# Zain-Jiang/Speech-Editing-Toolkit

Hardware: AMD Instinct MI355X
Metric: diffusion mel-frames/s (100-step p_sample, B=32/GPU, T=800) (higher is better)
Workload: dtype f32 (operands carried as 2 fp16 pieces, 3 MFMA products per term, fp32 accumulate: fp32-equivalent, see roofline.note)

## Files before the change

### include/set_amd.h

```cpp
#ifndef SET_AMD_H
#define SET_AMD_H

#include <stdint.h>

#ifdef __cplusplus
extern "C" {
#endif

#define SET_AMD_ABI_VERSION 2

#define SET_OK 0
#define SET_E_INVALID (-1)
#define SET_E_UNSUPPORTED (-2)
#define SET_E_LAUNCH (-3)

#define SET_ACT_NONE 0
#define SET_ACT_RELU 1
#define SET_ACT_GELU 2
#define SET_ACT_TANH 3
#define SET_ACT_SOFTPLUS 4
#define SET_ACT_MISH 5
#define SET_ACT_LRELU 6

#define SET_PRO_NONE 0
#define SET_PRO_LRELU 1
#define SET_PRO_DIV 2

#define SET_IMPL_NAIVE 1
#define SET_IMPL_MFMA 2
#define SET_IMPL_MFMA2 3

#define SET_IMPL_BF16 4
#define SET_IMPL_F16X2 5

#define SET_IMPL_FEWOUT 6

#define SET_DTYPE_F32 0
#define SET_DTYPE_BF16 1
#define SET_DTYPE_BF16_G16 2
#define SET_DTYPE_BF16_G16_X16 3

int set_abi_version(void);
const char *set_last_error(void);

typedef struct SetConv1dArgs {
    const float *in;
    const float *w;
    const float *bias;
    const float *res;
    const float *mask;
    const float *in_chan_add;
    float *out;
    int64_t in_bs, in_cs, out_bs, out_cs, res_bs, res_cs;
    int64_t w_base, w_sco, w_sci, w_stap;
    int32_t B, Cin, Cout, K, dil, pad;
    int32_t T_in, T_iter, T_out, out_stride, out_off;
    int32_t pro, act, accumulate, impl;
    float pro_param, act_param, alpha;
    float out_div;
} SetConv1dArgs;

int set_conv1d(const SetConv1dArgs *args, void *stream);

int64_t set_packed_conv_weight_size(int32_t Cout, int32_t Cin, int32_t K);
int set_pack_conv_weight(const float *w, float *wp, int32_t Cout, int32_t Cin, int32_t K,
                         int64_t w_base, int64_t w_sco, int64_t w_sci, int64_t w_stap, void *stream);

int64_t set_packed_conv_weight_x2_size(int32_t Cout, int32_t Cin, int32_t K);
int set_pack_conv_weight_x2(const float *w, void *wp, int32_t Cout, int32_t Cin, int32_t K, int64_t w_base, int64_t w_sco,
                            int64_t w_sci, int64_t w_stap, int32_t scale_exp, void *stream);
int64_t set_packed_conv_transpose_x2_size(int32_t Cout, int32_t Cin, int32_t k, int32_t u);
int set_pack_conv_transpose_x2(const float *w, void *wp, int32_t Cout, int32_t Cin, int32_t k, int32_t u, int32_t scale_exp,
                               void *stream);
int set_conv_transpose1d_x2(const float *in, const void *wp, const float *bias, float *out, int32_t B, int32_t Cin, int32_t Cout,
                            int32_t k, int32_t u, int32_t P, int32_t T_in, int32_t pro, float pro_param, void *stream);
int set_conv_x2_range_flag(int32_t *flag, int32_t reset);

typedef struct SetResblockPairArgs {
    const float *x;
    const void *w1;
    const float *b1;
    const void *w2;
    const float *b2;
    float *out;
    int64_t x_bs, x_cs, out_bs, out_cs;
    int32_t B, C, K, dil, T;
    int32_t accumulate;
    float slope, out_div;
} SetResblockPairArgs;
int64_t set_sizeof_resblock_pair_args(void);
int set_resblock_pair_x2_supported(int32_t C, int32_t K, int32_t dil, int32_t T);
int set_resblock_pair_x2(const SetResblockPairArgs *args, void *stream);

int64_t set_packed_conv_weight_v2_size(int32_t Cout, int32_t Cin, int32_t K);
int set_pack_conv_weight_v2(const float *w, float *wp, int32_t Cout, int32_t Cin, int32_t K, int32_t dil,
                            int64_t w_base, int64_t w_sco, int64_t w_sci, int64_t w_stap, void *stream);

int set_weight_norm_fold(const float *g, const float *v, float *w, int32_t n0, int64_t inner, void *stream);

int set_layernorm_ch(const float *x, const float *gamma, const float *beta, const float *mask, float *out,
                     int32_t B, int32_t C, int32_t T, float eps, void *stream);
int set_embedding_bct(const int64_t *idx, const float *table, float *out, int32_t B, int32_t T, int32_t C,
                      int32_t n_rows, float scale, int32_t accumulate, void *stream);
int set_embedding_bct_dev_scale(const int64_t *idx, const float *table, float *out, int32_t B, int32_t T, int32_t C,
                                int32_t n_rows, const float *scale_dev, int32_t accumulate, void *stream);
int set_abs_sum_mask(const float *x, float *mask, int32_t B, int32_t C, int32_t T, void *stream);
int set_index_mask(const int64_t *idx, float *mask, int64_t n, void *stream);
int set_expand_states(const float *enc, const int64_t *mel2ph, float *out, int32_t B, int32_t C,
                      int32_t T_txt, int32_t T, void *stream);
int set_add_chan_mask(const float *x, const float *add, const float *mask, float *out, int32_t B, int32_t C,
                      int32_t T, void *stream);
int set_masked_dur(const int64_t *mel2ph, const float *tmask, const int64_t *txt, int64_t *out, int32_t B,
                   int32_t T, int32_t T_txt, void *stream);
int set_pitch_coarse(const float *f0_in, const float *uv_in, const float *tmask, const int64_t *mel2ph_pad,
                     int32_t uv_from_logit, float *f0_denorm, int64_t *coarse, int64_t n, void *stream);
int set_transpose_btc_to_bct(const float *in, float *out, int32_t B, int32_t T, int32_t C, void *stream);
int set_transpose_bct_to_btc(const float *in, float *out, int32_t B, int32_t C, int32_t T, void *stream);
int set_sum_scale(const float *a, const float *b, const float *c, float *out, float div, int64_t n, void *stream);
int set_blend_mask(const float *a, const float *b, const float *m, float *out, int64_t n, int64_t inner, void *stream);
int set_mul_one_minus_mask(const float *x, const float *m, float *out, int64_t n, int64_t inner, void *stream);
int set_dur_total(const float *dur, const int64_t *txt, int64_t *total, int32_t B, int32_t T_txt, void *stream);
int set_length_regulate(const float *dur, const int64_t *txt, int64_t *mel2ph, int32_t B, int32_t T_txt,
                        int32_t T_out, void *stream);

int set_sinusoid_embed(const float *t, float *out, int32_t dim, int32_t n, void *stream);

int set_gate(const float *y, float *z, int32_t B, int32_t C, int32_t T, void *stream);
int set_res_skip(const float *x_in, const float *o, float *x_out, float *skip, int32_t B, int32_t C, int32_t T,
                 int32_t first, void *stream);

typedef struct SetDiffnetLayerArgs {
    const float *x_in;
    const float *condproj;
    const float *dstep;
    const float *w1p;
    const float *b_dil;
    const float *w2p;
    const float *b_out;
    float *x_out;
    float *skip;
    int64_t cp_bs, d_bs, d_cs;
    int32_t B, T, dil, first;
    uint64_t *dbg_clock;
} SetDiffnetLayerArgs;
int set_diffnet_layer(const SetDiffnetLayerArgs *args, void *stream);
int64_t set_diffnet_w1p_size(void);
int64_t set_diffnet_w2p_size(void);
int set_pack_diffnet_layer(const float *w_dil, const float *w_out, float *w1p, float *w2p, void *stream);
int set_pack_diffnet_layers(const float *w_dil, const float *w_out, int64_t wd_ls, int64_t wo_ls, float *w1p, float *w2p,
                            float *w1w, float *w2w, int32_t L, void *stream);

typedef struct SetDiffnetStackArgs {
    float *xa, *xb, *skip;
    const float *condproj;
    const float *dstep;
    const float *w1p_all;
    const float *w2p_all;
    const float *b_dil_all;
    const float *b_out_all;
    int32_t *sync_ws;
    int64_t cp_bs, cp_ls, d_bs, d_cs, d_ls;
    int32_t B, T, L, dilation_cycle_length;
    const float *w1w_all;
    const float *w2w_all;
    float *x_all;
    float *save_y;
    float *save_z;
    int32_t *err_flag;
    const float *w1s_all;
    const float *w2s_all;
    float *z_ws;
    const void *wx3_all;
    int32_t x3_mode;
} SetDiffnetStackArgs;
int set_diffnet_stack(const SetDiffnetStackArgs *args, void *stream);
int64_t set_sizeof_diffnet_stack_args(void);

int64_t set_diffnet_layer_x3_image_size(int32_t mode);
int set_pack_diffnet_layer_x3(const float *w_dil , const float *w_out , void *img, int32_t mode,
                              int32_t k1, int32_t k2, void *stream);
int set_diffnet_stack_variant(int B, int T, int dilation_cycle_length, int images);
int set_diffnet_stack_x3_winograd(int B, int T, int dilation_cycle_length, int images);
int64_t set_diffnet_w1w_size(void);
int set_pack_diffnet_layer_wino(const float *w_dil, const float *w_out, float *w1w, float *w2w, void *stream);

int set_posterior_step(const float *x0, const float *x_t, const float *eps, const float *coef4, int64_t coef_bs,
                       float *x_prev, int32_t B, int64_t per_batch, uint64_t seed, uint64_t offset, void *stream);
int set_q_sample(const float *x_start, const float *eps, const float *ab2, const float *nonpad, float *x_t,
                 int32_t B, int32_t M, int32_t T, void *stream);
int set_randn(float *out, int64_t n, uint64_t seed, uint64_t offset, void *stream);
int set_rng_seed_delta(const uint64_t *dev_word);
int set_stream_order(void *first, void *after, int32_t slot);
int set_stream_mark(void *stream, int32_t slot, int32_t dev);
int set_stream_mark_done(int32_t slot);
int set_stream_create_low_priority(void **out);

typedef struct SetDiffLoopArgs {
    int32_t B, T, M, L, steps, dilation_cycle_length;
    float *x;
    const float *noise;
    uint64_t seed;
    const float *condproj;
    const float *dstep;
    const float *coef4;
    const float *w_in_p;
    const float *b_in;
    const float *w1p_all;
    const float *w2p_all;
    const float *b_dil_all;
    const float *b_out_all;
    const float *w1w_all;
    const float *w2w_all;
    const float *w1s_all;
    const float *w2s_all;
    float *z_ws;
    const void *wx3_all;
    int32_t x3_mode;
    const void *w_skip_x2, *w_outp_x2, *w_in_x2;
    const float *w_skip_p;
    const float *b_skip;
    const float *w_outp_p;
    const float *b_outp;
    float *ws_x0, *ws_x1, *ws_skip, *ws_h;
    float *ws_x0pred;
    float *layer_span_ms;
    float *loop_ms;
    int32_t n_groups;
    int32_t persistent;
    int32_t *sync_ws;
    int32_t *err_flag;
    const float *cond;
    const void *img16_all;
    const float *b_cond_all;
    float *bf16_ws;
    int64_t bf16_ws_floats;
} SetDiffLoopArgs;
int set_diffusion_loop(const SetDiffLoopArgs *args, void *stream);

int set_conv1d_wgrad(const float *g, const float *x, const float *chan_add, float *dw, int32_t B, int32_t Cin,
                     int32_t Cout, int32_t K, int32_t dil, int32_t pad, int32_t T, int32_t T_in, int32_t pro,
                     float pro_param, int32_t impl, void *stream);

int64_t set_conv1d_wgrad_scratch_floats(int32_t B, int32_t Cin, int32_t Cout, int32_t K, int32_t T, int32_t dtype);
int set_conv1d_wgrad_det(const void *g, const void *x, const float *chan_add, float *dw, int32_t B, int32_t Cin,
                         int32_t Cout, int32_t K, int32_t dil, int32_t pad, int32_t T, int32_t T_in, int32_t pro,
                         float pro_param, int32_t dtype, float *scratch, int64_t scratch_floats, void *stream);
int64_t set_conv1d_wgrad_grouped_scratch_floats(int32_t groups, int32_t B, int32_t Cin, int32_t Cout, int32_t K, int32_t T);
int set_conv1d_wgrad_det_grouped(const void *g, const void *x, const float *chan_add, float *dw, int32_t groups, int64_t g_gs,
                                 int64_t x_gs, int64_t add_gs, int64_t dw_gs, int32_t B, int32_t Cin, int32_t Cout, int32_t K,
                                 int32_t dil, int32_t pad, int32_t T, int32_t T_in, int32_t dtype, float *scratch,
                                 int64_t scratch_floats, void *stream);

typedef struct SetDiffnetLayerBf16Args {
    const float *x_in;
    float *x_out;
    float *skip;
    const float *cond;
    const float *dstep;
    const void *img;
    const float *b_dil, *b_cond, *b_out;
    uint16_t *y16;
    uint16_t *z16;
    int64_t d_bs, d_cs;
    int32_t B, T, dil, first;
} SetDiffnetLayerBf16Args;
int64_t set_sizeof_diffnet_layer_bf16_args(void);
int64_t set_diffnet_layer_bf16_image_size(void);
int set_pack_diffnet_layer_bf16(const float *wdil , const float *wcond ,
                                const float *wout , void *img, void *stream);
int set_pack_diffnet_layers_bf16(const float *wdil, const float *wcond, const float *wout, int64_t sdil, int64_t scond, int64_t sout,
                                 void *img, int32_t L, void *stream);
int set_diffnet_layer_fwd_bf16(const SetDiffnetLayerBf16Args *args, void *stream);
typedef struct SetDiffnetLayersBf16Args {
    const float *x_in;
    float *x_out;
    float *skip;
    const float *cond;
    const float *dstep;
    const void *img;
    const float *b_dil, *b_cond, *b_out;
    float *scratch;
    int64_t scratch_floats;
    int64_t d_bs, d_cs, d_ls;
    int32_t B, T, l0, nl, dilation_cycle_length, first;
} SetDiffnetLayersBf16Args;
int64_t set_sizeof_diffnet_layers_bf16_args(void);
int64_t set_diffnet_layers_bf16_scratch_floats(int32_t B, int32_t T, int32_t l0, int32_t nl, int32_t dilation_cycle_length);
int32_t set_diffnet_layers_bf16_plan(int32_t B, int32_t T, int32_t L, int32_t dilation_cycle_length);
int set_diffnet_layers_fwd_bf16(const SetDiffnetLayersBf16Args *args, void *stream);
int set_debug_bf16_phase_buffer(uint64_t *buf);
int set_debug_split_phase_buffer(uint64_t *buf);
int set_debug_x3_phase_buffer(uint64_t *buf);
int set_debug_resblock_phase_buffer(uint64_t *buf);

typedef struct SetDiffnetLayerBf16BwdArgs {
    const float *dx_out;
    const float *dskip;
    const uint16_t *y16;
    const void *img;
    float *dx;
    uint16_t *dy16;
    uint16_t *do16;
    float *dcond;
    float *part_dbo;
    float *part_dby;
    float *part_dd;
    int32_t B, T, dil, dcond_first;
} SetDiffnetLayerBf16BwdArgs;
int64_t set_sizeof_diffnet_layer_bf16_bwd_args(void);
int32_t set_diffnet_layer_bwd_bf16_tiles(int32_t T, int32_t dil);
int set_diffnet_layer_bwd_bf16(const SetDiffnetLayerBf16BwdArgs *args, void *stream);
int set_diffnet_layer_bwd_reduce(const float *part_dbo, const float *part_dby, const float *part_dd, int32_t B, int32_t tiles,
                                 float *db_out, float *db_dil, float *db_cond, float *dd, int64_t dd_bs, void *stream);
int set_diffnet_layers_bwd_reduce(const float *part_dbo, const float *part_dby, const float *part_dd, int32_t B, int32_t tiles, int32_t L,
                                  float *db_out, int64_t s_out, float *db_dil, int64_t s_dil, float *db_cond, int64_t s_cond, float *dd,
                                  int64_t dd_bs, int64_t dd_ls, void *stream);
int set_partial_rows_sum(const float *part, float *out, int32_t groups, int32_t rows, int32_t cols, int32_t accumulate,
                         float scale, void *stream);

int set_step_proj_fwd(const float *h, const float *w, int64_t w_ls, const float *b, int64_t b_ls, float *out, int32_t L, int32_t C,
                      int32_t N, void *stream);
int64_t set_step_proj_bwd_scratch_floats(int32_t L, int32_t C, int32_t N);
int set_step_proj_bwd(const float *h, const float *g, const float *w, int64_t w_ls, float *dh, float *dw, int64_t dw_ls, float *db,
                      int64_t db_ls, float *scratch, int32_t L, int32_t C, int32_t N, void *stream);
int set_step_proj_bwd_dh(const float *g, const float *w, int64_t w_ls, float *dh, float *scratch, int32_t L, int32_t C, int32_t N,
                         void *stream);
// ... 144 lines not shown
```

### speech-editing-toolkit_amd/_lib.py

```python
import ctypes as C
import os
import shutil
import subprocess

_PKG = os.path.dirname(os.path.abspath(__file__))
_ROOT = os.path.dirname(_PKG)
CSRC = os.path.join(_PKG, "csrc")
INCLUDE = os.path.join(_ROOT, "include")
LIB_PATH = os.path.join(_PKG, "libset_amd.so")
_LIB_OVERRIDE = os.environ.get("SET_AMD_LIB")
SOURCES = ["conv1d.hip", "conv_x2.hip", "resblock_x2.hip", "glue.hip", "diffnet.hip", "diffnet_x3.hip", "train.hip", "attention.hip", "attention_fused.hip", "bf16.hip", "diffnet_bf16.hip", "stutter.hip"]
HIPCC_FLAGS = ["--offload-arch=gfx950", "-O3", "-std=c++17", "-fPIC", "-shared", "-ffp-contract=off"]

OK, E_INVALID, E_UNSUPPORTED, E_LAUNCH = 0, -1, -2, -3
ACT = dict(none=0, relu=1, gelu=2, tanh=3, softplus=4, mish=5, lrelu=6)
PRO = dict(none=0, lrelu=1, div=2)
IMPL_NAIVE, IMPL_MFMA, IMPL_MFMA2, IMPL_BF16, IMPL_F16X2, IMPL_FEWOUT = 1, 2, 3, 4, 5, 6
DTYPE_F32, DTYPE_BF16, DTYPE_BF16_G16, DTYPE_BF16_G16_X16 = 0, 1, 2, 3

c_f32p = C.POINTER(C.c_float)
c_i64p = C.POINTER(C.c_int64)


class SetConv1dArgs(C.Structure):
    _fields_ = [
        ("inp", C.c_void_p), ("w", C.c_void_p), ("bias", C.c_void_p), ("res", C.c_void_p),
        ("mask", C.c_void_p), ("in_chan_add", C.c_void_p), ("out", C.c_void_p),
        ("in_bs", C.c_int64), ("in_cs", C.c_int64), ("out_bs", C.c_int64), ("out_cs", C.c_int64),
        ("res_bs", C.c_int64), ("res_cs", C.c_int64),
        ("w_base", C.c_int64), ("w_sco", C.c_int64), ("w_sci", C.c_int64), ("w_stap", C.c_int64),
        ("B", C.c_int32), ("Cin", C.c_int32), ("Cout", C.c_int32), ("K", C.c_int32), ("dil", C.c_int32),
        ("pad", C.c_int32),
        ("T_in", C.c_int32), ("T_iter", C.c_int32), ("T_out", C.c_int32), ("out_stride", C.c_int32),
        ("out_off", C.c_int32),
        ("pro", C.c_int32), ("act", C.c_int32), ("accumulate", C.c_int32), ("impl", C.c_int32),
        ("pro_param", C.c_float), ("act_param", C.c_float), ("alpha", C.c_float), ("out_div", C.c_float),
    ]


class SetDiffnetLayerArgs(C.Structure):
    _fields_ = [
        ("x_in", C.c_void_p), ("condproj", C.c_void_p), ("dstep", C.c_void_p), ("w1p", C.c_void_p),
        ("b_dil", C.c_void_p), ("w2p", C.c_void_p), ("b_out", C.c_void_p), ("x_out", C.c_void_p),
        ("skip", C.c_void_p),
        ("cp_bs", C.c_int64), ("d_bs", C.c_int64), ("d_cs", C.c_int64),
        ("B", C.c_int32), ("T", C.c_int32), ("dil", C.c_int32), ("first", C.c_int32),
        ("dbg_clock", C.c_void_p),
    ]


class SetDiffLoopArgs(C.Structure):
    _fields_ = [
        ("B", C.c_int32), ("T", C.c_int32), ("M", C.c_int32), ("L", C.c_int32), ("steps", C.c_int32),
        ("dilation_cycle_length", C.c_int32),
        ("x", C.c_void_p), ("noise", C.c_void_p), ("seed", C.c_uint64),
        ("condproj", C.c_void_p), ("dstep", C.c_void_p), ("coef4", C.c_void_p),
        ("w_in_p", C.c_void_p), ("b_in", C.c_void_p),
        ("w1p_all", C.c_void_p), ("w2p_all", C.c_void_p), ("b_dil_all", C.c_void_p), ("b_out_all", C.c_void_p),
        ("w1w_all", C.c_void_p), ("w2w_all", C.c_void_p),
        ("w1s_all", C.c_void_p), ("w2s_all", C.c_void_p), ("z_ws", C.c_void_p), ("wx3_all", C.c_void_p),
        ("x3_mode", C.c_int32),
        ("w_skip_x2", C.c_void_p), ("w_outp_x2", C.c_void_p), ("w_in_x2", C.c_void_p),
        ("w_skip_p", C.c_void_p), ("b_skip", C.c_void_p), ("w_outp_p", C.c_void_p), ("b_outp", C.c_void_p),
        ("ws_x0", C.c_void_p), ("ws_x1", C.c_void_p), ("ws_skip", C.c_void_p), ("ws_h", C.c_void_p),
        ("ws_x0pred", C.c_void_p),
        ("layer_span_ms", C.POINTER(C.c_float)),
        ("loop_ms", C.POINTER(C.c_float)),
        ("n_groups", C.c_int32),
        ("persistent", C.c_int32),
        ("sync_ws", C.c_void_p),
        ("err_flag", C.c_void_p),
        ("cond", C.c_void_p), ("img16_all", C.c_void_p), ("b_cond_all", C.c_void_p),
        ("bf16_ws", C.c_void_p), ("bf16_ws_floats", C.c_int64),
    ]


class SetDiffnetStackArgs(C.Structure):
    _fields_ = [
        ("xa", C.c_void_p), ("xb", C.c_void_p), ("skip", C.c_void_p), ("condproj", C.c_void_p), ("dstep", C.c_void_p),
        ("w1p_all", C.c_void_p), ("w2p_all", C.c_void_p), ("b_dil_all", C.c_void_p), ("b_out_all", C.c_void_p),
        ("sync_ws", C.c_void_p),
        ("cp_bs", C.c_int64), ("cp_ls", C.c_int64), ("d_bs", C.c_int64), ("d_cs", C.c_int64), ("d_ls", C.c_int64),
        ("B", C.c_int32), ("T", C.c_int32), ("L", C.c_int32), ("dilation_cycle_length", C.c_int32),
        ("w1w_all", C.c_void_p), ("w2w_all", C.c_void_p),
        ("x_all", C.c_void_p), ("save_y", C.c_void_p), ("save_z", C.c_void_p),
        ("err_flag", C.c_void_p),
        ("w1s_all", C.c_void_p), ("w2s_all", C.c_void_p), ("z_ws", C.c_void_p), ("wx3_all", C.c_void_p),
        ("x3_mode", C.c_int32),
    ]


class SetDiffnetLayerBf16Args(C.Structure):
    _fields_ = [
        ("x_in", C.c_void_p), ("x_out", C.c_void_p), ("skip", C.c_void_p), ("cond", C.c_void_p), ("dstep", C.c_void_p),
        ("img", C.c_void_p), ("b_dil", C.c_void_p), ("b_cond", C.c_void_p), ("b_out", C.c_void_p),
        ("y16", C.c_void_p), ("z16", C.c_void_p),
        ("d_bs", C.c_int64), ("d_cs", C.c_int64),
        ("B", C.c_int32), ("T", C.c_int32), ("dil", C.c_int32), ("first", C.c_int32),
    ]


class SetDiffnetLayersBf16Args(C.Structure):
    _fields_ = [
        ("x_in", C.c_void_p), ("x_out", C.c_void_p), ("skip", C.c_void_p), ("cond", C.c_void_p), ("dstep", C.c_void_p),
        ("img", C.c_void_p), ("b_dil", C.c_void_p), ("b_cond", C.c_void_p), ("b_out", C.c_void_p),
        ("scratch", C.c_void_p), ("scratch_floats", C.c_int64),
        ("d_bs", C.c_int64), ("d_cs", C.c_int64), ("d_ls", C.c_int64),
        ("B", C.c_int32), ("T", C.c_int32), ("l0", C.c_int32), ("nl", C.c_int32), ("dilation_cycle_length", C.c_int32),
        ("first", C.c_int32),
    ]


class SetDiffnetLayerBf16BwdArgs(C.Structure):
    _fields_ = [
        ("dx_out", C.c_void_p), ("dskip", C.c_void_p), ("y16", C.c_void_p), ("img", C.c_void_p),
        ("dx", C.c_void_p), ("dy16", C.c_void_p), ("do16", C.c_void_p), ("dcond", C.c_void_p),
        ("part_dbo", C.c_void_p), ("part_dby", C.c_void_p), ("part_dd", C.c_void_p),
        ("B", C.c_int32), ("T", C.c_int32), ("dil", C.c_int32), ("dcond_first", C.c_int32),
    ]


class SetResblockPairArgs(C.Structure):
    _fields_ = [
        ("x", C.c_void_p), ("w1", C.c_void_p), ("b1", C.c_void_p), ("w2", C.c_void_p), ("b2", C.c_void_p), ("out", C.c_void_p),
        ("x_bs", C.c_int64), ("x_cs", C.c_int64), ("out_bs", C.c_int64), ("out_cs", C.c_int64),
        ("B", C.c_int32), ("C", C.c_int32), ("K", C.c_int32), ("dil", C.c_int32), ("T", C.c_int32),
        ("accumulate", C.c_int32),
        ("slope", C.c_float), ("out_div", C.c_float),
    ]


class SetPackBf16Desc(C.Structure):
    _fields_ = [
        ("w", C.c_void_p), ("wp", C.c_void_p),
        ("w_base", C.c_int64), ("w_sco", C.c_int64), ("w_sci", C.c_int64), ("w_stap", C.c_int64), ("start", C.c_int64),
        ("Cout", C.c_int32), ("Cin", C.c_int32), ("K", C.c_int32), ("CoutP", C.c_int32), ("CinP", C.c_int32), ("pad_", C.c_int32),
    ]


class SetPackF32Desc(C.Structure):
    _fields_ = [
        ("w", C.c_void_p), ("wp", C.c_void_p),
        ("w_base", C.c_int64), ("w_sco", C.c_int64), ("w_sci", C.c_int64), ("w_stap", C.c_int64), ("start", C.c_int64),
        ("Cout", C.c_int32), ("Cin", C.c_int32), ("K", C.c_int32), ("CinP", C.c_int32), ("kind", C.c_int32), ("RB", C.c_int32),
        ("ch_max", C.c_int32), ("pad_", C.c_int32),
    ]


class SetBmmArgs(C.Structure):
    _fields_ = [
        ("A", C.c_void_p), ("B", C.c_void_p), ("C", C.c_void_p),
        ("a_bo", C.c_int64), ("a_bi", C.c_int64), ("a_ms", C.c_int64), ("a_ks", C.c_int64),
        ("b_bo", C.c_int64), ("b_bi", C.c_int64), ("b_ks", C.c_int64), ("b_ns", C.c_int64),
        ("c_bo", C.c_int64), ("c_bi", C.c_int64), ("c_ms", C.c_int64), ("c_ns", C.c_int64),
        ("n_outer", C.c_int32), ("n_inner", C.c_int32), ("M", C.c_int32), ("N", C.c_int32), ("K", C.c_int32),
        ("alpha", C.c_float), ("accumulate", C.c_int32),
    ]


class SetAttnArgs(C.Structure):
    _fields_ = [
        ("q", C.c_void_p), ("k", C.c_void_p), ("v", C.c_void_p), ("o", C.c_void_p), ("lse", C.c_void_p), ("p", C.c_void_p),
        ("kpm", C.c_void_p),
        ("q_bs", C.c_int64), ("k_bs", C.c_int64), ("v_bs", C.c_int64), ("o_bs", C.c_int64),
        ("q_cs", C.c_int32), ("k_cs", C.c_int32), ("v_cs", C.c_int32), ("o_cs", C.c_int32),
        ("B", C.c_int32), ("heads", C.c_int32), ("head_dim", C.c_int32), ("Tq", C.c_int32), ("Tk", C.c_int32),
        ("scale", C.c_float), ("fill", C.c_float),
        ("bf16", C.c_int32),
    ]


class SetAttnBwdArgs(C.Structure):
    _fields_ = [
        ("fwd", SetAttnArgs),
        ("d_o", C.c_void_p), ("delta", C.c_void_p), ("dq", C.c_void_p), ("dk", C.c_void_p), ("dv", C.c_void_p),
        ("dq_bs", C.c_int64), ("dk_bs", C.c_int64), ("dv_bs", C.c_int64),
        ("dq_cs", C.c_int32), ("dk_cs", C.c_int32), ("dv_cs", C.c_int32),
    ]


_V, _I32, _I64, _U64, _F = C.c_void_p, C.c_int32, C.c_int64, C.c_uint64, C.c_float

SIGNATURES = {
    "set_abi_version": (C.c_int, []),
    "set_last_error": (C.c_char_p, []),
    "set_conv1d": (C.c_int, [C.POINTER(SetConv1dArgs), _V]),
    "set_packed_conv_weight_size": (_I64, [_I32, _I32, _I32]),
    "set_pack_conv_weight": (C.c_int, [_V, _V, _I32, _I32, _I32, _I64, _I64, _I64, _I64, _V]),
    "set_packed_conv_weight_v2_size": (_I64, [_I32, _I32, _I32]),
    "set_pack_conv_weight_v2": (C.c_int, [_V, _V, _I32, _I32, _I32, _I32, _I64, _I64, _I64, _I64, _V]),
    "set_weight_norm_fold": (C.c_int, [_V, _V, _V, _I32, _I64, _V]),
    "set_layernorm_ch": (C.c_int, [_V, _V, _V, _V, _V, _I32, _I32, _I32, _F, _V]),
    "set_embedding_bct": (C.c_int, [_V, _V, _V, _I32, _I32, _I32, _I32, _F, _I32, _V]),
    "set_embedding_bct_dev_scale": (C.c_int, [_V, _V, _V, _I32, _I32, _I32, _I32, _V, _I32, _V]),
    "set_abs_sum_mask": (C.c_int, [_V, _V, _I32, _I32, _I32, _V]),
    "set_index_mask": (C.c_int, [_V, _V, _I64, _V]),
    "set_expand_states": (C.c_int, [_V, _V, _V, _I32, _I32, _I32, _I32, _V]),
    "set_add_chan_mask": (C.c_int, [_V, _V, _V, _V, _I32, _I32, _I32, _V]),
    "set_masked_dur": (C.c_int, [_V, _V, _V, _V, _I32, _I32, _I32, _V]),
    "set_pitch_coarse": (C.c_int, [_V, _V, _V, _V, _I32, _V, _V, _I64, _V]),
    "set_transpose_btc_to_bct": (C.c_int, [_V, _V, _I32, _I32, _I32, _V]),
    "set_transpose_bct_to_btc": (C.c_int, [_V, _V, _I32, _I32, _I32, _V]),
    "set_sum_scale": (C.c_int, [_V, _V, _V, _V, _F, _I64, _V]),
    "set_blend_mask": (C.c_int, [_V, _V, _V, _V, _I64, _I64, _V]),
    "set_mul_one_minus_mask": (C.c_int, [_V, _V, _V, _I64, _I64, _V]),
    "set_dur_total": (C.c_int, [_V, _V, _V, _I32, _I32, _V]),
    "set_length_regulate": (C.c_int, [_V, _V, _V, _I32, _I32, _I32, _V]),
    "set_sinusoid_embed": (C.c_int, [_V, _V, _I32, _I32, _V]),
    "set_gate": (C.c_int, [_V, _V, _I32, _I32, _I32, _V]),
    "set_res_skip": (C.c_int, [_V, _V, _V, _V, _I32, _I32, _I32, _I32, _V]),
    "set_diffnet_layer": (C.c_int, [C.POINTER(SetDiffnetLayerArgs), _V]),
    "set_diffnet_w1p_size": (_I64, []),
    "set_diffnet_w2p_size": (_I64, []),
    "set_pack_diffnet_layer": (C.c_int, [_V, _V, _V, _V, _V]),
    "set_pack_diffnet_layers": (C.c_int, [_V, _V, _I64, _I64, _V, _V, _V, _V, _I32, _V]),
    "set_diffnet_stack_variant": (C.c_int, [C.c_int, C.c_int, C.c_int, C.c_int]),
    "set_diffnet_stack_x3_winograd": (C.c_int, [C.c_int, C.c_int, C.c_int, C.c_int]),
    "set_packed_conv_weight_x2_size": (C.c_int64, [_I32, _I32, _I32]),
    "set_pack_conv_weight_x2": (C.c_int, [_V, _V, _I32, _I32, _I32, _I64, _I64, _I64, _I64, _I32, _V]),
    "set_conv_x2_range_flag": (C.c_int, [C.POINTER(C.c_int32), _I32]),
    "set_sizeof_resblock_pair_args": (_I64, []),
    "set_resblock_pair_x2_supported": (C.c_int, [_I32, _I32, _I32, _I32]),
    "set_resblock_pair_x2": (C.c_int, [C.POINTER(SetResblockPairArgs), _V]),
    "set_packed_conv_transpose_x2_size": (C.c_int64, [_I32, _I32, _I32, _I32]),
    "set_pack_conv_transpose_x2": (C.c_int, [_V, _V, _I32, _I32, _I32, _I32, _I32, _V]),
    "set_conv_transpose1d_x2": (C.c_int, [_V, _V, _V, _V, _I32, _I32, _I32, _I32, _I32, _I32, _I32, _I32, _F, _V]),
    "set_diffnet_layer_x3_image_size": (C.c_int64, [_I32]),
    "set_pack_diffnet_layer_x3": (C.c_int, [_V, _V, _V, _I32, _I32, _I32, _V]),
    "set_diffnet_w1w_size": (_I64, []),
    "set_pack_diffnet_layer_wino": (C.c_int, [_V, _V, _V, _V, _V]),
    "set_diffnet_stack": (C.c_int, [C.POINTER(SetDiffnetStackArgs), _V]),
    "set_sizeof_diffnet_stack_args": (_I64, []),
    "set_posterior_step": (C.c_int, [_V, _V, _V, _V, _I64, _V, _I32, _I64, _U64, _U64, _V]),
    "set_q_sample": (C.c_int, [_V, _V, _V, _V, _V, _I32, _I32, _I32, _V]),
    "set_randn": (C.c_int, [_V, _I64, _U64, _U64, _V]),
    "set_rng_seed_delta": (C.c_int, [_V]),
    "set_stream_order": (C.c_int, [_V, _V, _I32]),
    "set_stream_mark": (C.c_int, [_V, _I32, _I32]),
    "set_stream_mark_done": (C.c_int, [_I32]),
    "set_stream_create_low_priority": (C.c_int, [C.POINTER(C.c_void_p)]),
    "set_diffusion_loop": (C.c_int, [C.POINTER(SetDiffLoopArgs), _V]),
# ... 193 lines not shown
```

### speech-editing-toolkit_amd/csrc/diffnet.hip

```cpp
#include <stdlib.h>

#include "common.h"
#include "boundary_x2.h"

namespace {

constexpr int DC = 256;
constexpr int NT = 64;
constexpr int KS1 = 3 * DC / 2;
constexpr int KS2 = DC / 2;

__device__ __forceinline__ int urow16(int r) { return (r & 3) + 8 * (r >> 2); }

__device__ __forceinline__ int layer_row(int w, int rb, int i) {
    return (rb < 2 ? 64 * w + 32 * rb : DC + 64 * w + 32 * (rb - 2)) + i;
}

__device__ __forceinline__ float fast_sigmoid(float x) { return __builtin_amdgcn_rcpf(1.0f + __expf(-x)); }
__device__ __forceinline__ float fast_tanh(float x) { return 1.0f - 2.0f * __builtin_amdgcn_rcpf(1.0f + __expf(2.0f * x)); }

struct LayerTile {
    const float *xin;
    float *xout;
    float *skp;
// ... 812 lines not shown
#ifdef SET_WINO_PHASES
    if (tid == 0)
        for (int k = 0; k < 9; ++k) atomicAdd(a.sync_ws + 4 + ntiles + k, (int)(ph[k] >> 10));
#endif
    if (tid == 0) {
        atomicAdd(a.sync_ws + 2, (int)(wait_ticks >> 10));
        atomicAdd(a.sync_ws + 3, (int)(fence_ticks >> 10));
    }
}

__global__ void __launch_bounds__(256) pack_diffnet_layer_kernel(const float *w_dil, const float *w_out, float *w1p,
                                                                 float *w2p, int64_t wd_ls = 0, int64_t wo_ls = 0) {
    const int64_t idx = (int64_t)blockIdx.x * 256 + threadIdx.x;
    const int64_t n1 = (int64_t)4 * KS1 * 64 * 4, n2 = (int64_t)4 * KS2 * 64 * 4;
    w_dil += (int64_t)blockIdx.y * wd_ls;
    w_out += (int64_t)blockIdx.y * wo_ls;
    w1p += (int64_t)blockIdx.y * n1;
    w2p += (int64_t)blockIdx.y * n2;
    if (idx < n1) {
        const int rb = (int)(idx & 3), lane = (int)((idx >> 2) & 63);
        const int ks = (int)((idx >> 8) % KS1), w = (int)((idx >> 8) / KS1);
        const int tap = ks >> 7, cp = ks & 127;
        const int row = layer_row(w, rb, lane & 31), c = 2 * cp + (lane >> 5);
        w1p[idx] = w_dil[((int64_t)row * DC + c) * 3 + tap];
    } else if (idx < n1 + n2) {
        const int64_t j = idx - n1;
        const int rb = (int)(j & 3), lane = (int)((j >> 2) & 63);
        const int ks = (int)((j >> 8) % KS2), w = (int)((j >> 8) / KS2);
        const int row = layer_row(w, rb, lane & 31), c = 2 * ks + (lane >> 5);
        w2p[j] = w_out[(int64_t)row * DC + c];
    }
}

__global__ void __launch_bounds__(256) pack_diffnet_wino_kernel(const float *w_dil, const float *w_out, float *w1w,
                                                                float *w2w, int64_t wd_ls = 0, int64_t wo_ls = 0) {
    const int64_t idx = (int64_t)blockIdx.x * 256 + threadIdx.x;
    const int64_t n1 = (int64_t)8 * WN_KS * 64 * 8, n2 = (int64_t)8 * WN_KS * 64 * 2;
    w_dil += (int64_t)blockIdx.y * wd_ls;
    w_out += (int64_t)blockIdx.y * wo_ls;
    w1w += (int64_t)blockIdx.y * n1;
    w2w += (int64_t)blockIdx.y * n2;
    if (idx < n1) {
        const int e = (int)(idx & 7), lane = (int)((idx >> 3) & 63);
        const int ks = (int)((idx >> 9) % WN_KS), w = (int)((idx >> 9) / WN_KS);
        const int rf = e >> 2, p = e & 3;
        const int row = rf * DC + 32 * w + (lane & 31), c = 2 * ks + (lane >> 5);
        const float *g = w_dil + ((int64_t)row * DC + c) * 3;
        const double g0 = g[0], g1 = g[1], g2 = g[2];
        const double v = p == 0 ? g0 : (p == 1 ? 0.5 * (g0 + g1 + g2) : (p == 2 ? 0.5 * (g0 - g1 + g2) : g2));
        w1w[idx] = (float)v;
    } else if (idx < n1 + n2) {
        const int64_t j = idx - n1;
        const int rb = (int)(j & 1), lane = (int)((j >> 1) & 63);
        const int ks = (int)((j >> 7) % WN_KS), w = (int)((j >> 7) / WN_KS);
        const int row = rb * DC + 32 * w + (lane & 31), c = 2 * ks + (lane >> 5);
        w2w[j] = w_out[(int64_t)row * DC + c];
    }
}

}

extern "C" int64_t set_diffnet_w1w_size(void) { return (int64_t)512 * 256 * 4; }
extern "C" int set_pack_diffnet_layer_wino(const float *w_dil, const float *w_out, float *w1w, float *w2w, void *stream) {
    SET_REQUIRE(w_dil && w_out && w1w && w2w, "set_pack_diffnet_layer_wino");
    const int64_t total = set_diffnet_w1w_size() + (int64_t)512 * 256;
    hipLaunchKernelGGL(pack_diffnet_wino_kernel, dim3(set_blocks(total, 256)), dim3(256), 0, (hipStream_t)stream, w_dil,
                       w_out, w1w, w2w);
    return set_check_launch("set_pack_diffnet_layer_wino");
}

extern "C" int64_t set_diffnet_w1p_size(void) { return (int64_t)512 * 768; }
extern "C" int64_t set_diffnet_w2p_size(void) { return (int64_t)512 * 256; }

extern "C" int set_pack_diffnet_layers(const float *w_dil, const float *w_out, int64_t wd_ls, int64_t wo_ls, float *w1p, float *w2p,
                                       float *w1w, float *w2w, int32_t L, void *stream) {
    SET_REQUIRE(w_dil && w_out && w1p && w2p && L > 0 && L <= 65535 && (w1w == nullptr) == (w2w == nullptr), "set_pack_diffnet_layers");
    SET_REQUIRE((int64_t)8 * WN_KS * 64 * 8 == set_diffnet_w1w_size() && (int64_t)8 * WN_KS * 64 * 2 == (int64_t)512 * 256 &&
                    (int64_t)4 * KS1 * 64 * 4 == set_diffnet_w1p_size() && (int64_t)4 * KS2 * 64 * 4 == set_diffnet_w2p_size(),
                "set_pack_diffnet_layers(image sizes)");
    const int64_t total = set_diffnet_w1p_size() + set_diffnet_w2p_size();
    hipLaunchKernelGGL(pack_diffnet_layer_kernel, dim3(set_blocks(total, 256), L), dim3(256), 0, (hipStream_t)stream, w_dil, w_out, w1p,
                       w2p, wd_ls, wo_ls);
    int rc = set_check_launch("set_pack_diffnet_layers");
    if (rc != SET_OK || w1w == nullptr) return rc;
    const int64_t totw = set_diffnet_w1w_size() + (int64_t)512 * 256;
    hipLaunchKernelGGL(pack_diffnet_wino_kernel, dim3(set_blocks(totw, 256), L), dim3(256), 0, (hipStream_t)stream, w_dil, w_out, w1w,
                       w2w, wd_ls, wo_ls);
    return set_check_launch("set_pack_diffnet_layers(wino)");
}
extern "C" int set_pack_diffnet_layer(const float *w_dil, const float *w_out, float *w1p, float *w2p, void *stream) {
    SET_REQUIRE(w_dil && w_out && w1p && w2p, "set_pack_diffnet_layer");
    const int64_t total = set_diffnet_w1p_size() + set_diffnet_w2p_size();
    hipLaunchKernelGGL(pack_diffnet_layer_kernel, dim3(set_blocks(total, 256)), dim3(256), 0, (hipStream_t)stream,
                       w_dil, w_out, w1p, w2p);
    return set_check_launch("set_pack_diffnet_layer");
}

extern "C" int set_diffnet_layer(const SetDiffnetLayerArgs *args, void *stream) {
    SET_REQUIRE(args != nullptr, "set_diffnet_layer");
    const SetDiffnetLayerArgs &a = *args;
    SET_REQUIRE(a.x_in && a.condproj && a.dstep && a.w1p && a.b_dil && a.w2p && a.b_out && a.x_out && a.skip,
                "set_diffnet_layer");
    SET_REQUIRE(a.B > 0 && a.T > 0 && a.dil >= 1, "set_diffnet_layer");
    SET_REQUIRE(a.x_in != a.x_out, "set_diffnet_layer(x_in must not alias x_out)");
    if (a.dil > 8) return set_fail(SET_E_UNSUPPORTED, "set_diffnet_layer", "dilation > 8 (LDS tile > 80 KiB)");
    const size_t lds = (size_t)DC * (NT + 2 * a.dil) * sizeof(float);
    static SetDeviceOnce lds_once;
    if (int rc = set_lds_optin(lds_once, 96 * 1024, "set_diffnet_layer(attr)", diffnet_layer_kernel)) return rc;
    dim3 grid((a.T + NT - 1) / NT, a.B);
    hipLaunchKernelGGL(diffnet_layer_kernel, grid, dim3(256), lds, (hipStream_t)stream, a);
    return set_check_launch("set_diffnet_layer");
}

extern "C" int set_debug_split_phase_buffer(uint64_t *buf) {
    SET_HIP(hipMemcpyToSymbol(HIP_SYMBOL(g_split_phase_buf), &buf, sizeof(buf)), "set_debug_split_phase_buffer");
    return SET_OK;
}

extern "C" int64_t set_sizeof_diffnet_stack_args(void) { return (int64_t)sizeof(SetDiffnetStackArgs); }

static bool split_f32_pinned() {
    const char *e = getenv("SET_AMD_SPLIT_F32");
    return e && atoi(e) != 0;
}
static int x3_mode_of_images(int images) { return (images & 4) ? 3 : ((images & 8) ? 2 : 0); }

static int stack_variant(int B, int T, int dcl, bool have_wino, bool have_split, int x3_mode, int n_cu) {
    const bool have_x3 = x3_mode == 2 || x3_mode == 3;
    const int64_t tiles64 = (int64_t)B * ((T + 63) / 64);
    const int64_t split_blocks = 4 * (int64_t)B * ((T + 31) / 32);
    const bool split_one_per_cu = have_x3 && !split_f32_pinned();
    const bool split_fits = have_split && dcl <= 4 && split_blocks <= (split_one_per_cu ? 1 : 2) * (int64_t)n_cu;
    const bool split_pays = split_blocks <= (int64_t)(have_x3 ? 1 : 2) * n_cu;
    int split_env = 1;
    if (const char *e = getenv("SET_AMD_SPLIT")) split_env = atoi(e);
    if (split_fits && (split_env == 2 || (split_env == 1 && !getenv("SET_AMD_WINO") && split_pays))) return 3;
    int x3_env = 1;
    if (const char *e = getenv("SET_AMD_X3")) x3_env = atoi(e);
    if (have_x3 && dcl <= 4 && (x3_env == 2 || (x3_env == 1 && !getenv("SET_AMD_WINO") && tiles64 >= 8)))
        return x3_mode == 3 ? 4 : 5;
    int ncb = tiles64 < 3 * n_cu ? 1 : 2;
    if (const char *e = getenv("SET_AMD_STACK_NCB")) ncb = atoi(e) == 2 ? 2 : 1;
    const bool wino_ok = have_wino && (1 << (dcl - 1)) <= WN_MAXD;
    bool wino = wino_ok && 25 * tiles64 >= 17 * n_cu;
    if (const char *e = getenv("SET_AMD_WINO")) wino = wino_ok && (atoi(e) == 2 || (wino && atoi(e) != 0));
    return wino ? 2 : (ncb == 1 ? 1 : 0);
}
extern "C" int set_diffnet_stack_variant(int B, int T, int dilation_cycle_length, int images) {
    int n_cu = 256;
    (void)set_cu_count(&n_cu);
    return stack_variant(B, T, dilation_cycle_length, (images & 1) != 0, (images & 2) != 0, x3_mode_of_images(images), n_cu);
}

int set_launch_diffnet_stack_x3(const SetDiffnetStackArgs &a, int n_cu, int fault_tile, hipStream_t s);
int set_x3_winograd_selected(int x3_mode, int B, int T, int dilation_cycle_length, int n_cu);
extern "C" int set_diffnet_stack_x3_winograd(int B, int T, int dilation_cycle_length, int images) {
    int n_cu = 256;
    (void)set_cu_count(&n_cu);
    const int x3_mode = x3_mode_of_images(images);
    if (stack_variant(B, T, dilation_cycle_length, (images & 1) != 0, (images & 2) != 0, x3_mode, n_cu) != 5) return 0;
    return set_x3_winograd_selected(x3_mode, B, T, dilation_cycle_length, n_cu);
}
int set_launch_diffnet_stack_split_x2(const SetDiffnetStackArgs &a, int fault_tile, hipStream_t s);

extern "C" int set_diffnet_stack(const SetDiffnetStackArgs *args, void *stream) {
    SET_REQUIRE(args != nullptr, "set_diffnet_stack");
    const SetDiffnetStackArgs &a = *args;
    SET_REQUIRE(a.xa && a.xb && a.skip && a.condproj && a.dstep && a.w1p_all && a.w2p_all && a.b_dil_all &&
                    a.b_out_all && a.sync_ws,
                "set_diffnet_stack");
    SET_REQUIRE(a.B > 0 && a.T > 0 && a.L > 0 && a.dilation_cycle_length >= 1 && a.dilation_cycle_length <= 4,
                "set_diffnet_stack");
    hipStream_t s = (hipStream_t)stream;
    static SetDeviceOnce lds_once;
    if (int rc = set_lds_optin(lds_once, 150 * 1024, "set_diffnet_stack(attr)", diffnet_stack_kernel<1, 8, 2>, diffnet_stack_kernel<2, 4, 2>,
                               diffnet_stack_wino_kernel<true>, diffnet_stack_wino_kernel<false>, diffnet_stack_split_kernel))
        return rc;
    int n_cu = 0;
    SET_HIP(set_cu_count(&n_cu), "set_diffnet_stack");
    const bool plain = !a.x_all && !a.save_y && !a.save_z;
    const int variant = stack_variant(a.B, a.T, a.dilation_cycle_length, a.w1w_all && a.w2w_all,
                                      a.w1s_all && a.w2s_all && a.z_ws && plain, (a.wx3_all && plain) ? a.x3_mode : 0, n_cu);
    int fault_tile = -1;
    if (const char *e = getenv("SET_AMD_FAULT_TILE")) fault_tile = atoi(e);
    if (variant >= 4) return set_launch_diffnet_stack_x3(a, n_cu, fault_tile, s);
    if (variant == 3 && a.wx3_all && a.x3_mode == 2 && !split_f32_pinned())
        return set_launch_diffnet_stack_split_x2(a, fault_tile, s);
    if (variant == 3) {
        const int tiles = (a.T + 31) / 32, nt = a.B * tiles;
        SET_HIP(set_zero_async(a.sync_ws, (size_t)(4 + 2 * nt) * sizeof(int32_t), s), "set_diffnet_stack(memset)");
        hipLaunchKernelGGL(diffnet_stack_split_kernel, dim3(4 * nt), dim3(256), (size_t)SP_LDS_FLOATS * sizeof(float), s, a,
                           tiles, nt, fault_tile);
        return set_check_launch("set_diffnet_stack");
    }
    const bool wino = variant == 2;
    const int ncb = variant == 1 ? 1 : 2;
    const int ntt = 32 * ncb;
    int tiles_per_utt = (a.T + ntt - 1) / ntt;
    int ntiles = a.B * tiles_per_utt;
    bool concat = wino && a.dilation_cycle_length == 1 && a.T % 2 == 0 && a.T >= WN_NT &&
                  (int64_t)a.cp_bs * 4 < (1ll << 31) && a.d_bs == 0 && !a.save_y && !a.save_z;
    if (concat) {
        ntiles = (int)(((int64_t)a.B * a.T + WN_NT - 1) / WN_NT);
        tiles_per_utt = ntiles;
    }
    const int64_t ntasks64 = (int64_t)ntiles * a.L;
    SET_REQUIRE(ntasks64 < (1ll << 30), "set_diffnet_stack(task count)");
    const int max_dil = 1 << (a.dilation_cycle_length - 1);
    const int task_slot = DC * (ntt + 2 * max_dil);
    const size_t lds = (size_t)(task_slot + 4) * sizeof(float);
    SET_HIP(set_zero_async(a.sync_ws, (size_t)(4 + ntiles + (wino ? 12 : 0)) * sizeof(int32_t), s),
            "set_diffnet_stack(memset)");
    const int wps = wino ? 1 : 2;
    int grid = wps * n_cu;
    if (grid > ntiles * 4 / 5) grid = ntiles * 4 / 5;
    if (grid < n_cu) grid = n_cu < ntiles ? n_cu : ntiles;
    if (const char *e = getenv("SET_AMD_STACK_GRID")) grid = atoi(e) > 0 ? atoi(e) : grid;
    if ((int64_t)grid > ntasks64) grid = (int)ntasks64;
    if (grid < 1) grid = 1;
    if (wino) {
        if (a.dilation_cycle_length == 1)
            hipLaunchKernelGGL(diffnet_stack_wino_kernel<true>, dim3(grid), dim3(512),
                               (size_t)(WN_ZS_OFF + DC * WN_NT + 4) * sizeof(float), s, a, tiles_per_utt, ntiles,
                               (int)ntasks64, concat ? 1 : 0, fault_tile);
        else
            hipLaunchKernelGGL(diffnet_stack_wino_kernel<false>, dim3(grid), dim3(512),
                               (size_t)(WN_ZS_OFF + DC * WN_NT + 4) * sizeof(float), s, a, tiles_per_utt, ntiles,
                               (int)ntasks64, 0, fault_tile);
    } else if (ncb == 1)
        hipLaunchKernelGGL((diffnet_stack_kernel<1, 8, 2>), dim3(grid), dim3(256), lds, s, a, tiles_per_utt, ntiles,
                           (int)ntasks64, task_slot);
    else
        hipLaunchKernelGGL((diffnet_stack_kernel<2, 4, 2>), dim3(grid), dim3(256), lds, s, a, tiles_per_utt, ntiles,
                           (int)ntasks64, task_slot);
    return set_check_launch("set_diffnet_stack");
}

namespace {
__global__ void __launch_bounds__(256) gate_kernel(const float *y, float *z, int B, int C, int T) {
    const int64_t i = (int64_t)blockIdx.x * 256 + threadIdx.x;
    if (i >= (int64_t)B * C * T) return;
    const int64_t ct = i % ((int64_t)C * T);
    const int64_t b = i / ((int64_t)C * T);
    const float *yb = y + b * 2 * C * T;
    z[i] = dev_sigmoid(yb[ct]) * tanhf(yb[(int64_t)C * T + ct]);
}
__global__ void __launch_bounds__(256) res_skip_kernel(const float *x_in, const float *o, float *x_out, float *skip,
                                                       int B, int C, int T, int first) {
    const int64_t i = (int64_t)blockIdx.x * 256 + threadIdx.x;
    if (i >= (int64_t)B * C * T) return;
    const int64_t ct = i % ((int64_t)C * T);
    const int64_t b = i / ((int64_t)C * T);
    const float *ob = o + b * 2 * C * T;
    x_out[i] = (x_in[i] + ob[ct]) / 1.41421356237309504880f;
    const float s = ob[(int64_t)C * T + ct];
    skip[i] = first ? s : skip[i] + s;
}
__global__ void __launch_bounds__(256) sinusoid_kernel(const float *t, float *out, int dim, int n) {
    const int64_t i = (int64_t)blockIdx.x * 256 + threadIdx.x;
    if (i >= (int64_t)dim * n) return;
    const int j = (int)(i / n), k = (int)(i % n);
    const int half = dim / 2;
    const int jj = j < half ? j : j - half;
    const float e = (float)(9.210340371976184 / (double)(half - 1));
    const float freq = expf((float)jj * -e);
    const float ang = t[k] * freq;
    out[i] = j < half ? sinf(ang) : cosf(ang);
}


__global__ void __launch_bounds__(256) randn_kernel(float *out, int64_t n, uint64_t seed, uint64_t offset, const uint64_t *seed_delta) {
    const int64_t q = (int64_t)blockIdx.x * 256 + threadIdx.x;
    if (q * 4 >= n) return;
    if (seed_delta) seed += *seed_delta;
    float z[4];
    randn4(seed, offset + (uint64_t)q, z);
#pragma unroll
    for (int k = 0; k < 4; ++k)
        if (q * 4 + k < n) out[q * 4 + k] = z[k];
}

__global__ void __launch_bounds__(256) posterior_kernel(const float *x0, const float *x_t, const float *eps,
                                                        const float *coef4, int64_t coef_bs, float *x_prev,
                                                        int64_t per_batch, int64_t n, uint64_t seed,
                                                        uint64_t offset, const uint64_t *seed_delta) {
    const int64_t q = (int64_t)blockIdx.x * 256 + threadIdx.x;
    if (q * 4 >= n) return;
    if (seed_delta) seed += *seed_delta;
    float z[4];
    if (!eps) randn4(seed, offset + (uint64_t)q, z);
#pragma unroll
    for (int k = 0; k < 4; ++k) {
        const int64_t i = q * 4 + k;
        if (i >= n) break;
        const float *cf = coef4 + (i / per_batch) * coef_bs;
        const float mean = cf[0] * x0[i] + cf[1] * x_t[i];
        const float e = eps ? eps[i] : z[k];
        x_prev[i] = mean + cf[3] * expf(0.5f * cf[2]) * e;
    }
}

__global__ void __launch_bounds__(256) q_sample_kernel(const float *x_start, const float *eps, const float *ab2,
                                                       const float *nonpad, float *x_t, int B, int M, int T) {
    const int64_t i = (int64_t)blockIdx.x * 256 + threadIdx.x;
    if (i >= (int64_t)B * M * T) return;
    const int t = (int)(i % T);
    const int b = (int)(i / ((int64_t)M * T));
    float v = ab2[2 * b] * x_start[i] + ab2[2 * b + 1] * eps[i];
    if (nonpad) v *= nonpad[(int64_t)b * T + t];
    x_t[i] = v;
}

__global__ void __launch_bounds__(64) selftest_mfma_kernel(float *max_err) {
    constexpr int K = 8;
    const int lane = threadIdx.x;
    auto Af = [](int i, int k) { return 0.25f * (float)((i * 7 + k * 3) % 11) - 1.0f; };
    auto Bf = [](int k, int j) { return 0.125f * (float)((k * 5 + j * 13) % 17) - 0.75f; };
    f32x16 acc = {0};
    for (int k0 = 0; k0 < K; k0 += 2) {
        const int k = k0 + (lane >> 5);
        acc = mfma32(Af(lane & 31, k), Bf(k, lane & 31), acc);
    }
    float err = 0.0f;
    for (int r = 0; r < 16; ++r) {
        const int row = mfma32_row(r, lane), col = lane & 31;
        float ref = 0.0f;
        for (int k = 0; k < K; ++k) ref = fmaf(Af(row, k), Bf(k, col), ref);
        err = fmaxf(err, fabsf(ref - acc[r]));
    }
    for (int off = 32; off > 0; off >>= 1) err = fmaxf(err, __shfl_xor(err, off));
    if (lane == 0) *max_err = err;
}
}

extern "C" int set_gate(const float *y, float *z, int32_t B, int32_t C, int32_t T, void *stream) {
    SET_REQUIRE(y && z && B > 0 && C > 0 && T > 0, "set_gate");
    hipLaunchKernelGGL(gate_kernel, dim3(set_blocks((int64_t)B * C * T, 256)), dim3(256), 0, (hipStream_t)stream, y, z,
                       B, C, T);
    return set_check_launch("set_gate");
}
extern "C" int set_res_skip(const float *x_in, const float *o, float *x_out, float *skip, int32_t B, int32_t C,
                            int32_t T, int32_t first, void *stream) {
    SET_REQUIRE(x_in && o && x_out && skip && B > 0 && C > 0 && T > 0, "set_res_skip");
    hipLaunchKernelGGL(res_skip_kernel, dim3(set_blocks((int64_t)B * C * T, 256)), dim3(256), 0, (hipStream_t)stream,
                       x_in, o, x_out, skip, B, C, T, first);
    return set_check_launch("set_res_skip");
}
extern "C" int set_sinusoid_embed(const float *t, float *out, int32_t dim, int32_t n, void *stream) {
    SET_REQUIRE(t && out && dim >= 4 && (dim % 2) == 0 && n > 0, "set_sinusoid_embed");
    hipLaunchKernelGGL(sinusoid_kernel, dim3(set_blocks((int64_t)dim * n, 256)), dim3(256), 0, (hipStream_t)stream, t,
                       out, dim, n);
    return set_check_launch("set_sinusoid_embed");
}
static const uint64_t *g_seed_delta = nullptr;
const uint64_t *set_seed_delta_ptr() { return g_seed_delta; }
extern "C" int set_rng_seed_delta(const uint64_t *dev_word) {
    g_seed_delta = dev_word;
    return SET_OK;
}

extern "C" int set_randn(float *out, int64_t n, uint64_t seed, uint64_t offset, void *stream) {
    SET_REQUIRE(out && n > 0, "set_randn");
    hipLaunchKernelGGL(randn_kernel, dim3(set_blocks((n + 3) / 4, 256)), dim3(256), 0, (hipStream_t)stream, out, n,
                       seed, offset, g_seed_delta);
    return set_check_launch("set_randn");
}
extern "C" int set_posterior_step(const float *x0, const float *x_t, const float *eps, const float *coef4,
                                  int64_t coef_bs, float *x_prev, int32_t B, int64_t per_batch, uint64_t seed,
                                  uint64_t offset, void *stream) {
    SET_REQUIRE(x0 && x_t && coef4 && x_prev && B > 0 && per_batch > 0, "set_posterior_step");
    const int64_t n = (int64_t)B * per_batch;
    hipLaunchKernelGGL(posterior_kernel, dim3(set_blocks((n + 3) / 4, 256)), dim3(256), 0, (hipStream_t)stream, x0,
                       x_t, eps, coef4, coef_bs, x_prev, per_batch, n, seed, offset, g_seed_delta);
    return set_check_launch("set_posterior_step");
}
extern "C" int set_q_sample(const float *x_start, const float *eps, const float *ab2, const float *nonpad, float *x_t,
                            int32_t B, int32_t M, int32_t T, void *stream) {
    SET_REQUIRE(x_start && eps && ab2 && x_t && B > 0 && M > 0 && T > 0, "set_q_sample");
    hipLaunchKernelGGL(q_sample_kernel, dim3(set_blocks((int64_t)B * M * T, 256)), dim3(256), 0, (hipStream_t)stream,
                       x_start, eps, ab2, nonpad, x_t, B, M, T);
    return set_check_launch("set_q_sample");
}
extern "C" int set_selftest_mfma(float *max_err_host, void *stream) {
    SET_REQUIRE(max_err_host != nullptr, "set_selftest_mfma");
    float *d = nullptr;
    SET_HIP(hipMalloc(&d, sizeof(float)), "set_selftest_mfma");
    hipLaunchKernelGGL(selftest_mfma_kernel, dim3(1), dim3(64), 0, (hipStream_t)stream, d);
    int rc = set_check_launch("set_selftest_mfma");
    if (rc == SET_OK) {
        hipError_t e = hipMemcpyAsync(max_err_host, d, sizeof(float), hipMemcpyDeviceToHost, (hipStream_t)stream);
        if (e == hipSuccess) e = hipStreamSynchronize((hipStream_t)stream);
        if (e != hipSuccess) rc = set_fail(SET_E_LAUNCH, "set_selftest_mfma", hipGetErrorString(e));
    }
    (void)hipFree(d);
    return rc;
}

struct BoundaryArgs {
    const float *skip;
    float *x;
    const float *eps;
    const float *coef4;
    const float *w_skip_p, *b_skip, *w_outp_p, *b_outp, *w_in_p, *b_in;
    float *xin_next;
    float inv_div;
    float div;
    uint64_t seed, quad_offset;
    int T, M, MP;
};
constexpr int BD_LD = 64;

__global__ void __launch_bounds__(256, 2) diffnet_boundary_kernel(BoundaryArgs a) {
    extern __shared__ __attribute__((aligned(16))) float smem[];
    const int tid = threadIdx.x, lane = tid & 63;
    const int w = __builtin_amdgcn_readfirstlane(tid >> 6);
    const int half = lane >> 5, l31 = lane & 31;
    const int b = blockIdx.y, t0 = blockIdx.x * 64, T = a.T, M = a.M;
    {
        const rsrc_t rs = make_rsrc(a.skip + (int64_t)b * DC * T);
        const unsigned vo = 4u * (unsigned)min(t0 + lane, T - 1);
        const bool tv = t0 + lane < T;
        for (int r0 = 0; r0 < 64; r0 += 16) {
            float v[16];
#pragma unroll
            for (int u = 0; u < 16; ++u) v[u] = buf_load(rs, vo, 4u * (unsigned)(64 * w + r0 + u) * (unsigned)T);
#pragma unroll
            for (int u = 0; u < 16; ++u) smem[(64 * w + r0 + u) * BD_LD + lane] = tv ? v[u] / a.div : 0.0f;
        }
    }
    __syncthreads();
    f32x16 acc[2][1][2];
#pragma unroll
    for (int i = 0; i < 2; ++i) {
        acc[i][0][0] = (f32x16){0};
        acc[i][0][1] = (f32x16){0};
        const float *wp = a.w_skip_p + (int64_t)(2 * w + i) * (DC / 2) * 64 + lane;
        const float *bp = smem + half * BD_LD + l31;
        gemm_groups<1, 2, 8>(acc[i], wp, bp, 2 * BD_LD, (DC / 2) / 8, [&](int) {
            wp += 8 * 64;
            bp += 8 * 2 * BD_LD;
        });
    }
    __syncthreads();
#pragma unroll
    for (int i = 0; i < 2; ++i)
#pragma unroll
        for (int r = 0; r < 16; ++r) {
            const int row = 32 * (2 * w + i) + mfma32_row(r, lane);
            const float bias = a.b_skip[row];
#pragma unroll
            for (int cb = 0; cb < 2; ++cb) smem[row * BD_LD + 32 * cb + l31] = fmaxf(acc[i][0][cb][r] + bias, 0.0f);
        }
    __syncthreads();
    const int rbn = (M + 31) / 32;
    f32x16 xo[1][2];
    xo[0][0] = (f32x16){0};
    xo[0][1] = (f32x16){0};
    if (w < rbn) {
        const float *wp = a.w_outp_p + (int64_t)w * (DC / 2) * 64 + lane;
        const float *bp = smem + half * BD_LD + l31;
        gemm_groups<1, 2, 8>(xo, wp, bp, 2 * BD_LD, (DC / 2) / 8, [&](int) {
            wp += 8 * 64;
            bp += 8 * 2 * BD_LD;
        });
    }
    __syncthreads();
    if (w < rbn) {
#pragma unroll
        for (int r = 0; r < 16; ++r) {
            const int row = 32 * w + mfma32_row(r, lane);
            const float bias = a.b_outp[min(row, M - 1)];
#pragma unroll
            for (int cb = 0; cb < 2; ++cb) smem[row * BD_LD + 32 * cb + l31] = row < M ? xo[0][cb][r] + bias : 0.0f;
        }
    }
    __syncthreads();
    {
        const float c1 = a.coef4[0], c2 = a.coef4[1], sig = a.coef4[3] * expf(0.5f * a.coef4[2]);
        float *xb = a.x + (int64_t)b * M * T;
        const float *eb = a.eps ? a.eps + (int64_t)b * M * T : nullptr;
        for (int qi = tid; qi < a.MP * 16; qi += 256) {
            const int m = qi >> 4, tq = qi & 15, t = t0 + 4 * tq;
            float *cell = smem + m * BD_LD + 4 * tq;
            if (m < M && t < T) {
                const int64_t i = (int64_t)m * T + t;
                const f32x4 xt = *reinterpret_cast<const f32x4 *>(xb + i);
                float z[4];
                if (eb) {
                    const f32x4 e4 = *reinterpret_cast<const f32x4 *>(eb + i);
                    z[0] = e4[0]; z[1] = e4[1]; z[2] = e4[2]; z[3] = e4[3];
                } else {
                    randn4(a.seed, a.quad_offset + (uint64_t)(((int64_t)b * M * T + i) >> 2), z);
                }
                f32x4 o;
#pragma unroll
                for (int k = 0; k < 4; ++k) {
                    const float mean = c1 * cell[k] + c2 * xt[k];
                    o[k] = mean + sig * z[k];
                }
                *reinterpret_cast<f32x4 *>(xb + i) = o;
                *reinterpret_cast<f32x4 *>(cell) = o;
            } else {
                *reinterpret_cast<f32x4 *>(cell) = (f32x4){0.0f, 0.0f, 0.0f, 0.0f};
            }
        }
    }
    if (!a.xin_next) return;
    __syncthreads();
#pragma unroll
    for (int i = 0; i < 2; ++i) {
        acc[i][0][0] = (f32x16){0};
        acc[i][0][1] = (f32x16){0};
        const float *wp = a.w_in_p + (int64_t)(2 * w + i) * (a.MP / 2) * 64 + lane;
        const float *bp = smem + half * BD_LD + l31;
        gemm_groups<1, 2, 4>(acc[i], wp, bp, 2 * BD_LD, (a.MP / 2) / 4, [&](int) {
            wp += 4 * 64;
            bp += 4 * 2 * BD_LD;
        });
    }
    const rsrc_t ro = make_rsrc(a.xin_next + (int64_t)b * DC * T);
    float bin[2][16];
#pragma unroll
    for (int i = 0; i < 2; ++i)
#pragma unroll
        for (int r = 0; r < 16; ++r) bin[i][r] = (a.b_in + 32 * (2 * w + i) + urow16(r))[4 * half];
#pragma unroll
    for (int cb = 0; cb < 2; ++cb) {
        if (t0 + 32 * cb + l31 < T) {
            const unsigned so = 4u * (unsigned)(4 * half * T + t0 + 32 * cb + l31);
#pragma unroll
            for (int i = 0; i < 2; ++i)
#pragma unroll
                for (int r = 0; r < 16; ++r) {
                    const int ur = 32 * (2 * w + i) + urow16(r);
                    buf_store(fmaxf(acc[i][0][cb][r] + bin[i][r], 0.0f), ro, so, 4u * (unsigned)ur * (unsigned)T);
                }
        }
    }
}

struct BoundaryX2Args {
    BoundaryArgs g;
    const unsigned short *w_skip_x2, *w_outp_x2, *w_in_x2;
    int32_t *err_flag;
};

__global__ void __launch_bounds__(256, 2) diffnet_boundary_x2_kernel(BoundaryX2Args ax) {
    const BoundaryArgs &a = ax.g;
    extern __shared__ __attribute__((aligned(16))) unsigned char bl[];
    const int tid = threadIdx.x, lane = tid & 63;
    const int w = __builtin_amdgcn_readfirstlane(tid >> 6);
    const int half = lane >> 5, l31 = lane & 31;
    const int b = blockIdx.y, t0 = blockIdx.x * 64, T = a.T, M = a.M;
    const unsigned lane16 = 16u * (unsigned)lane;
    const unsigned T4 = 4u * (unsigned)T;
    float amax = 0.0f;
    {
        const int f = lane, cg = w;
        const rsrc_t rs = make_rsrc(a.skip + (int64_t)b * DC * T);
        const unsigned vo = 4u * (unsigned)min(t0 + f, T - 1);
        const bool tv = t0 + f < T;
        for (int c0 = 0; c0 < 64; c0 += 16) {
            float v[16];
#pragma unroll
            for (int u = 0; u < 16; ++u) v[u] = buf_load(rs, vo, (unsigned)(64 * cg + c0 + u) * T4);
#pragma unroll
            for (int q8 = 0; q8 < 2; ++q8) {
                bx_u32x4 u0, u1;
#pragma unroll
                for (int e = 0; e < 4; ++e) {
                    unsigned short p0[2], p1[2];
#pragma unroll
                    for (int k = 0; k < 2; ++k) {
                        const float sv = v[8 * q8 + 2 * e + k] / a.div;
                        const float x = tv ? sv : 0.0f;
                        amax = fmaxf(amax, fabsf(x));
                        bx_split(x, p0[k], p1[k]);
                    }
                    u0[e] = (unsigned)p0[0] | ((unsigned)p0[1] << 16);
                    u1[e] = (unsigned)p1[0] | ((unsigned)p1[1] << 16);
                }
                *reinterpret_cast<bx_u32x4 *>(bl + f * BX_XR + (64 * cg + c0 + 8 * q8) * 2) = u0;
                *reinterpret_cast<bx_u32x4 *>(bl + BX_PIECE + f * BX_XR + (64 * cg + c0 + 8 * q8) * 2) = u1;
            }
        }
    }
    __syncthreads();
    auto bfrag256 = [&](int ks, int cb) { return (unsigned)((cb * 32 + l31) * BX_XR + (ks * 16 + half * 8) * 2); };
    {
        const rsrc_t rw = make_rsrc(ax.w_skip_x2);
        const float inv = reinterpret_cast<const float *>(ax.w_skip_x2 + (DC / 32) * (DC / 16) * 1024)[1];
        f32x16 acc[2][2];
#pragma unroll
        for (int i = 0; i < 2; ++i)
#pragma unroll
            for (int cb = 0; cb < 2; ++cb) acc[i][cb] = (f32x16){0};
        bx_gemm<2>(acc, rw, lane16, 2 * w, DC / 16, DC / 16, bl, BX_PIECE, bfrag256);
        __syncthreads();
#pragma unroll
        for (int i = 0; i < 2; ++i)
#pragma unroll
            for (int cb = 0; cb < 2; ++cb)
#pragma unroll
                for (int g = 0; g < 4; ++g) {
                    unsigned short p0[4], p1[4];
#pragma unroll
                    for (int e = 0; e < 4; ++e) {
                        const int row = 32 * (2 * w + i) + 8 * g + 4 * half + e;
                        const float h = fmaxf(acc[i][cb][4 * g + e] * inv + a.b_skip[row], 0.0f);
                        amax = fmaxf(amax, h);
                        bx_split(h, p0[e], p1[e]);
                    }
                    const unsigned off = (unsigned)((cb * 32 + l31) * BX_XR + (32 * (2 * w + i) + 8 * g + 4 * half) * 2);
                    bx_u32x2 u;
                    u[0] = (unsigned)p0[0] | ((unsigned)p0[1] << 16); u[1] = (unsigned)p0[2] | ((unsigned)p0[3] << 16);
                    *reinterpret_cast<bx_u32x2 *>(bl + off) = u;
                    u[0] = (unsigned)p1[0] | ((unsigned)p1[1] << 16); u[1] = (unsigned)p1[2] | ((unsigned)p1[3] << 16);
                    *reinterpret_cast<bx_u32x2 *>(bl + BX_PIECE + off) = u;
                }
    }
    __syncthreads();
    float *xs = reinterpret_cast<float *>(bl);
    {
        const int rbn = (M + 31) / 32;
        f32x16 xo[1][2];
        xo[0][0] = (f32x16){0};
        xo[0][1] = (f32x16){0};
        const float inv = reinterpret_cast<const float *>(ax.w_outp_x2 + ((M + 31) / 32) * (DC / 16) * 1024)[1];
        if (w < rbn) bx_gemm<1>(xo, make_rsrc(ax.w_outp_x2), lane16, w, DC / 16, DC / 16, bl, BX_PIECE, bfrag256);
        __syncthreads();
        if (w < 3) {
#pragma unroll
            for (int r = 0; r < 16; ++r) {
                const int row = 32 * w + mfma32_row(r, lane);
                const float bias = a.b_outp[min(row, M - 1)];
#pragma unroll
                for (int cb = 0; cb < 2; ++cb) xs[row * 64 + 32 * cb + l31] = (w < rbn && row < M) ? xo[0][cb][r] * inv + bias : 0.0f;
            }
        }
    }
    __syncthreads();
    {
        const float c1 = a.coef4[0], c2 = a.coef4[1], sig = a.coef4[3] * expf(0.5f * a.coef4[2]);
        float *xb = a.x + (int64_t)b * M * T;
        const float *eb = a.eps ? a.eps + (int64_t)b * M * T : nullptr;
        for (int qi = tid; qi < 96 * 16; qi += 256) {
            const int m = qi >> 4, tq = qi & 15, t = t0 + 4 * tq;
            float *cell = xs + m * 64 + 4 * tq;
            if (m < M && t < T) {
                const int64_t i = (int64_t)m * T + t;
                const f32x4 xt = *reinterpret_cast<const f32x4 *>(xb + i);
                float z[4];
                if (eb) {
                    const f32x4 e4 = *reinterpret_cast<const f32x4 *>(eb + i);
                    z[0] = e4[0]; z[1] = e4[1]; z[2] = e4[2]; z[3] = e4[3];
                } else {
                    randn4(a.seed, a.quad_offset + (uint64_t)(((int64_t)b * M * T + i) >> 2), z);
                }
                f32x4 o;
#pragma unroll
                for (int k = 0; k < 4; ++k) {
                    const float mean = c1 * cell[k] + c2 * xt[k];
                    o[k] = mean + sig * z[k];
                }
                *reinterpret_cast<f32x4 *>(xb + i) = o;
                *reinterpret_cast<f32x4 *>(cell) = o;
            } else {
                *reinterpret_cast<f32x4 *>(cell) = (f32x4){0.0f, 0.0f, 0.0f, 0.0f};
            }
        }
    }
    if (!a.xin_next) {
        if (!(amax < 32768.0f) && ax.err_flag) __hip_atomic_store(ax.err_flag, 2, __ATOMIC_RELAXED, __HIP_MEMORY_SCOPE_AGENT);
        return;
    }
    __syncthreads();
    unsigned char *xp = bl + BX_PIECE;
    constexpr unsigned XP_PIECE = 64 * BX_PR;
    {
        const int f = lane, cg = w;
#pragma unroll
        for (int q8 = 0; q8 < 3; ++q8) {
            bx_u32x4 u0, u1;
#pragma unroll
            for (int e = 0; e < 4; ++e) {
                unsigned short p0[2], p1[2];
#pragma unroll
                for (int k = 0; k < 2; ++k) {
                    const float x = xs[(24 * cg + 8 * q8 + 2 * e + k) * 64 + f];
                    amax = fmaxf(amax, fabsf(x));
                    bx_split(x, p0[k], p1[k]);
                }
                u0[e] = (unsigned)p0[0] | ((unsigned)p0[1] << 16);
                u1[e] = (unsigned)p1[0] | ((unsigned)p1[1] << 16);
            }
            *reinterpret_cast<bx_u32x4 *>(xp + f * BX_PR + (24 * cg + 8 * q8) * 2) = u0;
            *reinterpret_cast<bx_u32x4 *>(xp + XP_PIECE + f * BX_PR + (24 * cg + 8 * q8) * 2) = u1;
        }
    }
    if (!(amax < 32768.0f) && ax.err_flag) __hip_atomic_store(ax.err_flag, 2, __ATOMIC_RELAXED, __HIP_MEMORY_SCOPE_AGENT);
    __syncthreads();
    {
        const int ngin = ((M + 31) / 32) * 2;
        const float inv = reinterpret_cast<const float *>(ax.w_in_x2 + (DC / 32) * ngin * 1024)[1];
        f32x16 acc[2][2];
#pragma unroll
        for (int i = 0; i < 2; ++i)
#pragma unroll
            for (int cb = 0; cb < 2; ++cb) acc[i][cb] = (f32x16){0};
        bx_gemm<2>(acc, make_rsrc(ax.w_in_x2), lane16, 2 * w, ngin, ngin, xp, XP_PIECE,
                   [&](int ks, int cb) { return (unsigned)((cb * 32 + l31) * BX_PR + (ks * 16 + half * 8) * 2); });
        const rsrc_t ro = make_rsrc(a.xin_next + (int64_t)b * DC * T);
        float bin[2][16];
#pragma unroll
        for (int i = 0; i < 2; ++i)
#pragma unroll
            for (int r = 0; r < 16; ++r) bin[i][r] = (a.b_in + 32 * (2 * w + i) + urow16(r))[4 * half];
#pragma unroll
        for (int cb = 0; cb < 2; ++cb) {
            if (t0 + 32 * cb + l31 < T) {
                const unsigned so = 4u * (unsigned)(4 * half * T + t0 + 32 * cb + l31);
#pragma unroll
                for (int i = 0; i < 2; ++i)
#pragma unroll
                    for (int r = 0; r < 16; ++r) {
                        const int ur = 32 * (2 * w + i) + urow16(r);
                        buf_store(fmaxf(acc[i][cb][r] * inv + bin[i][r], 0.0f), ro, so, 4u * (unsigned)ur * (unsigned)T);
                    }
            }
        }
    }
}

static bool boundary_fusable(const SetDiffLoopArgs &a) {
    if (const char *e = getenv("SET_AMD_FUSED_BOUNDARY"))
        if (atoi(e) == 0) return false;
    return a.T % 4 == 0 && a.M <= 96 && a.M >= 2 && ((a.M + 15) / 16 * 16 / 2) % 8 == 0;
}

static int launch_boundary(const SetDiffLoopArgs &a, int Bg, const float *skip, float *x, const float *eps, int sid,
                           uint64_t quad_offset, float *xin_next, bool x2, hipStream_t s) {
    static SetDeviceOnce lds_once;
    if (int rc = set_lds_optin(lds_once, 80 * 1024, "boundary(attr)", diffnet_boundary_kernel, diffnet_boundary_x2_kernel)) return rc;
    BoundaryArgs g = {};
    g.skip = skip; g.x = x; g.eps = eps; g.coef4 = a.coef4 + 4 * sid;
    g.w_skip_p = a.w_skip_p; g.b_skip = a.b_skip; g.w_outp_p = a.w_outp_p; g.b_outp = a.b_outp;
    g.w_in_p = a.w_in_p; g.b_in = a.b_in; g.xin_next = xin_next;
    g.div = sqrtf((float)a.L); g.seed = a.seed; g.quad_offset = quad_offset;
    g.T = a.T; g.M = a.M; g.MP = (a.M + 15) / 16 * 16;
    if (x2) {
        BoundaryX2Args gx = {};
        gx.g = g;
        gx.w_skip_x2 = reinterpret_cast<const unsigned short *>(a.w_skip_x2);
        gx.w_outp_x2 = reinterpret_cast<const unsigned short *>(a.w_outp_x2);
        gx.w_in_x2 = reinterpret_cast<const unsigned short *>(a.w_in_x2);
        gx.err_flag = a.err_flag;
        hipLaunchKernelGGL(diffnet_boundary_x2_kernel, dim3((a.T + 63) / 64, Bg), dim3(256), (size_t)2 * BX_PIECE, s, gx);
    } else {
        hipLaunchKernelGGL(diffnet_boundary_kernel, dim3((a.T + 63) / 64, Bg), dim3(256), (size_t)DC * BD_LD * sizeof(float), s, g);
    }
    return set_check_launch("set_diffusion_loop(boundary)");
}

static SetConv1dArgs conv1x1_args(const float *in, const float *wp, const float *bias, float *out, int B, int Cin,
                                  int Cout, int T) {
    SetConv1dArgs c = {};
    c.in = in; c.w = wp; c.bias = bias; c.out = out;
    c.in_bs = (int64_t)Cin * T; c.in_cs = T; c.out_bs = (int64_t)Cout * T; c.out_cs = T;
    c.B = B; c.Cin = Cin; c.Cout = Cout; c.K = 1; c.dil = 1; c.pad = 0;
    c.T_in = T; c.T_iter = T; c.T_out = T; c.out_stride = 1; c.out_off = 0;
    c.alpha = 1.0f; c.impl = SET_IMPL_MFMA;
    return c;
}

static hipStream_t g_aux_streams[8] = {nullptr};
static int aux_stream(int i, hipStream_t *out) {
    if (!g_aux_streams[i]) SET_HIP(hipStreamCreateWithFlags(&g_aux_streams[i], hipStreamNonBlocking), "aux stream");
    *out = g_aux_streams[i];
    return SET_OK;
}

static int diffusion_chain(const SetDiffLoopArgs &a, int g, int b0, int Bg, hipStream_t s, hipEvent_t *ev) {
    const int T = a.T, M = a.M, L = a.L;
    const int64_t per_batch = (int64_t)M * T;
    float *x = a.x + (int64_t)b0 * per_batch;
    float *ws_x0 = a.ws_x0 + (int64_t)b0 * DC * T, *ws_x1 = a.ws_x1 + (int64_t)b0 * DC * T;
    float *ws_skip = a.ws_skip + (int64_t)b0 * DC * T, *ws_h = a.ws_h + (int64_t)b0 * DC * T;
    float *ws_x0pred = a.ws_x0pred + (int64_t)b0 * per_batch;
    const float *condproj = a.condproj ? a.condproj + (int64_t)b0 * L * 512 * T : nullptr;
    const int tiles_per_utt = (T + NT - 1) / NT;
    int32_t *sync_ws = a.sync_ws ? a.sync_ws + 16 * (int64_t)g + 2 * (int64_t)b0 * ((T + 31) / 32) : nullptr;
    const uint64_t quads_before = (uint64_t)((int64_t)b0 * per_batch / 4);
    const uint64_t quads_total = (uint64_t)(((int64_t)a.B * per_batch + 3) / 4);
    int rc = SET_OK;
    const bool fused_boundary = boundary_fusable(a);
    const bool bf16_loop = a.img16_all != nullptr;
    int n_cu = 0;
    SET_HIP(set_cu_count(&n_cu), "set_diffusion_loop");
    bool boundary_x2 = false;
    if (a.persistent && !bf16_loop && fused_boundary && a.w_skip_x2 && a.w_outp_x2 && a.w_in_x2 && a.wx3_all && a.x3_mode == 2 &&
        a.M <= 96) {
        const int v = stack_variant(Bg, T, a.dilation_cycle_length, a.w1w_all && a.w2w_all, a.w1s_all && a.w2s_all && a.z_ws,
                                    a.x3_mode, n_cu);
        boundary_x2 = v == 5 || (v == 3 && !split_f32_pinned());
    }
    if (bf16_loop && fused_boundary && a.w_skip_x2 && a.w_outp_x2 && a.w_in_x2 && a.M <= 96) boundary_x2 = true;
    if (const char *e = getenv("SET_AMD_BOUNDARY_X2")) boundary_x2 = boundary_x2 && atoi(e) != 0;
    for (int k = 0; k < a.steps && rc == SET_OK; ++k) {
        const int sid = a.steps - 1 - k;
        if (!fused_boundary || k == 0) {
            SetConv1dArgs cin = conv1x1_args(x, a.w_in_p, a.b_in, ws_x0, Bg, M, DC, T);
            cin.act = SET_ACT_RELU;
            rc = set_conv1d(&cin, s);
            if (rc != SET_OK) break;
        }
        float *cur = ws_x0, *nxt = ws_x1;
        if (ev) (void)hipEventRecord(ev[2 * k], s);
        if (a.persistent && !bf16_loop) {
            SetDiffnetStackArgs sa = {};
            sa.xa = ws_x0; sa.xb = ws_x1; sa.skip = ws_skip;
            sa.condproj = condproj; sa.cp_bs = (int64_t)L * 512 * T; sa.cp_ls = (int64_t)512 * T;
            sa.dstep = a.dstep + sid; sa.d_bs = 0; sa.d_cs = a.steps; sa.d_ls = (int64_t)DC * a.steps;
            sa.w1p_all = a.w1p_all; sa.w2p_all = a.w2p_all; sa.b_dil_all = a.b_dil_all; sa.b_out_all = a.b_out_all;
            sa.w1w_all = a.w1w_all; sa.w2w_all = a.w2w_all;
            sa.w1s_all = a.w1s_all; sa.w2s_all = a.w2s_all; sa.wx3_all = a.wx3_all; sa.x3_mode = a.x3_mode;
            sa.z_ws = a.z_ws ? a.z_ws + (int64_t)b0 * DC * 32 * ((T + 31) / 32) : nullptr;
            sa.err_flag = a.err_flag;
            sa.sync_ws = sync_ws;
            sa.B = Bg; sa.T = T; sa.L = L; sa.dilation_cycle_length = a.dilation_cycle_length;
            rc = set_diffnet_stack(&sa, s);
        }
        int fuse = 1;
        if (bf16_loop && a.bf16_ws && a.dilation_cycle_length <= 2) {
            fuse = set_diffnet_layers_bf16_plan(Bg, T, L, a.dilation_cycle_length);
            if (const char *e = getenv("SET_AMD_BF16_FUSE")) fuse = atoi(e) < 1 ? 1 : (atoi(e) > 16 ? 16 : atoi(e));
            if (fuse > 1 && a.bf16_ws_floats < set_diffnet_layers_bf16_scratch_floats(a.B, T, 0, fuse, a.dilation_cycle_length)) fuse = 1;
        }
        for (int l = 0; l < L && rc == SET_OK && bf16_loop && fuse > 1; l += fuse) {
            SetDiffnetLayersBf16Args fa = {};
            fa.x_in = cur; fa.x_out = nxt; fa.skip = ws_skip;
            fa.cond = a.cond + (int64_t)b0 * 192 * T;
            fa.dstep = a.dstep + sid; fa.d_bs = 0; fa.d_cs = a.steps; fa.d_ls = (int64_t)DC * a.steps;
            fa.img = reinterpret_cast<const uint16_t *>(a.img16_all) + (int64_t)l * set_diffnet_layer_bf16_image_size();
            fa.b_dil = a.b_dil_all + (int64_t)l * 512; fa.b_cond = a.b_cond_all + (int64_t)l * 512; fa.b_out = a.b_out_all + (int64_t)l * 512;
            const int64_t per_utt = set_diffnet_layers_bf16_scratch_floats(1, T, 0, fuse, a.dilation_cycle_length);
            fa.scratch = a.bf16_ws + (int64_t)b0 * per_utt; fa.scratch_floats = (int64_t)Bg * per_utt;
            fa.B = Bg; fa.T = T; fa.l0 = l; fa.nl = L - l < fuse ? L - l : fuse; fa.dilation_cycle_length = a.dilation_cycle_length;
            fa.first = (l == 0);
            rc = set_diffnet_layers_fwd_bf16(&fa, s);
            float *tmp = cur; cur = nxt; nxt = tmp;
        }
        for (int l = 0; l < L && rc == SET_OK && bf16_loop && fuse == 1; ++l) {
            SetDiffnetLayerBf16Args la = {};
            la.x_in = cur; la.x_out = nxt; la.skip = ws_skip;
            la.cond = a.cond + (int64_t)b0 * 192 * T;
            la.dstep = a.dstep + (int64_t)l * DC * a.steps + sid;
            la.d_bs = 0; la.d_cs = a.steps;
            la.img = reinterpret_cast<const uint16_t *>(a.img16_all) + (int64_t)l * set_diffnet_layer_bf16_image_size();
            la.b_dil = a.b_dil_all + (int64_t)l * 512; la.b_cond = a.b_cond_all + (int64_t)l * 512;
            la.b_out = a.b_out_all + (int64_t)l * 512;
            la.B = Bg; la.T = T; la.dil = 1 << (l % a.dilation_cycle_length); la.first = (l == 0);
            rc = set_diffnet_layer_fwd_bf16(&la, s);
            float *tmp = cur; cur = nxt; nxt = tmp;
        }
        for (int l = 0; l < L && rc == SET_OK && !a.persistent && !bf16_loop; ++l) {
            SetDiffnetLayerArgs la = {};
            la.x_in = cur; la.x_out = nxt; la.skip = ws_skip;
            la.condproj = condproj + (int64_t)l * 512 * T;
            la.cp_bs = (int64_t)L * 512 * T;
            la.dstep = a.dstep + (int64_t)l * DC * a.steps + sid;
            la.d_bs = 0; la.d_cs = a.steps;
            la.w1p = a.w1p_all + (int64_t)l * (512 * 768); la.b_dil = a.b_dil_all + (int64_t)l * 512;
            la.w2p = a.w2p_all + (int64_t)l * (512 * 256); la.b_out = a.b_out_all + (int64_t)l * 512;
            la.B = Bg; la.T = T; la.dil = 1 << (l % a.dilation_cycle_length); la.first = (l == 0);
            rc = set_diffnet_layer(&la, s);
            float *tmp = cur; cur = nxt; nxt = tmp;
        }
        if (ev) (void)hipEventRecord(ev[2 * k + 1], s);
        if (rc != SET_OK) break;
        const float *eps = a.noise ? a.noise + (int64_t)k * a.B * per_batch + (int64_t)b0 * per_batch : nullptr;
        if (fused_boundary) {
            rc = launch_boundary(a, Bg, ws_skip, x, eps, sid, (uint64_t)(k + 1) * quads_total + quads_before,
                                 k + 1 < a.steps ? ws_x0 : nullptr, boundary_x2, s);
            continue;
        }
        SetConv1dArgs cs = conv1x1_args(ws_skip, a.w_skip_p, a.b_skip, ws_h, Bg, DC, DC, T);
        cs.pro = SET_PRO_DIV; cs.pro_param = sqrtf((float)L); cs.act = SET_ACT_RELU;
        rc = set_conv1d(&cs, s);
        if (rc != SET_OK) break;
        SetConv1dArgs co = conv1x1_args(ws_h, a.w_outp_p, a.b_outp, ws_x0pred, Bg, DC, M, T);
        rc = set_conv1d(&co, s);
        if (rc != SET_OK) break;
        rc = set_posterior_step(ws_x0pred, x, eps, a.coef4 + 4 * sid, 0, x, Bg, per_batch, a.seed,
                                (uint64_t)(k + 1) * quads_total + quads_before, s);
    }
    return rc;
}

extern "C" int set_diffusion_loop(const SetDiffLoopArgs *args, void *stream) {
    SET_REQUIRE(args != nullptr, "set_diffusion_loop");
    const SetDiffLoopArgs &a = *args;
    SET_REQUIRE(a.B > 0 && a.T > 0 && a.M > 0 && a.L > 0 && a.steps > 0 && a.dilation_cycle_length >= 1,
                "set_diffusion_loop");
    SET_REQUIRE(a.x && a.dstep && a.coef4 && a.w_in_p && a.b_in && a.b_dil_all && a.b_out_all && a.w_skip_p && a.b_skip &&
                    a.w_outp_p && a.b_outp, "set_diffusion_loop");
    if (a.img16_all) {
        SET_REQUIRE(a.cond && a.b_cond_all, "set_diffusion_loop(bf16 loop needs cond and b_cond_all)");
    } else {
        SET_REQUIRE(a.condproj && a.w1p_all && a.w2p_all, "set_diffusion_loop");
        SET_REQUIRE(!a.persistent || a.sync_ws, "set_diffusion_loop(persistent needs sync_ws)");
    }
    SET_REQUIRE(a.ws_x0 && a.ws_x1 && a.ws_skip && a.ws_h && a.ws_x0pred, "set_diffusion_loop");
    hipStream_t s = (hipStream_t)stream;
    const int64_t per_batch = (int64_t)a.M * a.T;
    int G = a.n_groups < 1 ? 1 : (a.n_groups > 8 ? 8 : a.n_groups);
    if (G > a.B) G = a.B;
    if (per_batch % 4 != 0) G = 1;
    const bool timing = a.layer_span_ms != nullptr;
    hipEvent_t *ev = nullptr;
    if (timing) {
        ev = new hipEvent_t[(size_t)2 * a.steps * G];
        for (int i = 0; i < 2 * a.steps * G; ++i) SET_HIP(hipEventCreate(&ev[i]), "set_diffusion_loop(event)");
    }
    hipEvent_t loop_ev[2] = {nullptr, nullptr};
    if (a.loop_ms) {
        SET_HIP(hipEventCreate(&loop_ev[0]), "set_diffusion_loop(event)");
        SET_HIP(hipEventCreate(&loop_ev[1]), "set_diffusion_loop(event)");
        (void)hipEventRecord(loop_ev[0], s);
    }
    int rc = SET_OK;
    if (G == 1) {
        rc = diffusion_chain(a, 0, 0, a.B, s, ev);
    } else {
        hipEvent_t fork = nullptr, join[8] = {nullptr};
        SET_HIP(hipEventCreateWithFlags(&fork, hipEventDisableTiming), "set_diffusion_loop(fork)");
        SET_HIP(hipEventRecord(fork, s), "set_diffusion_loop(fork)");
        for (int g = 0; g < G && rc == SET_OK; ++g) {
            const int b0 = (int)((int64_t)a.B * g / G), b1 = (int)((int64_t)a.B * (g + 1) / G);
            hipStream_t sg;
            rc = aux_stream(g, &sg);
            if (rc != SET_OK) break;
            SET_HIP(hipStreamWaitEvent(sg, fork, 0), "set_diffusion_loop(fork wait)");
            rc = diffusion_chain(a, g, b0, b1 - b0, sg, ev ? ev + (size_t)2 * a.steps * g : nullptr);
            SET_HIP(hipEventCreateWithFlags(&join[g], hipEventDisableTiming), "set_diffusion_loop(join)");
            SET_HIP(hipEventRecord(join[g], sg), "set_diffusion_loop(join)");
            SET_HIP(hipStreamWaitEvent(s, join[g], 0), "set_diffusion_loop(join wait)");
        }
        (void)hipEventDestroy(fork);
        for (int g = 0; g < G; ++g)
            if (join[g]) (void)hipEventDestroy(join[g]);
    }
    if (a.loop_ms) (void)hipEventRecord(loop_ev[1], s);
    if (timing || a.loop_ms) {
        if (rc == SET_OK) {
            hipError_t e = hipStreamSynchronize(s);
            if (e != hipSuccess) rc = set_fail(SET_E_LAUNCH, "set_diffusion_loop(sync)", hipGetErrorString(e));
        }
        if (rc == SET_OK && timing) {
            for (int k = 0; k < a.steps; ++k) {
                float acc_ms = 0.0f;
                for (int g = 0; g < G; ++g) {
                    float ms = 0.0f;
                    (void)hipEventElapsedTime(&ms, ev[(size_t)2 * a.steps * g + 2 * k], ev[(size_t)2 * a.steps * g + 2 * k + 1]);
                    acc_ms += ms;
                }
                a.layer_span_ms[k] = acc_ms / (float)G;
            }
        }
        if (rc == SET_OK && a.loop_ms) (void)hipEventElapsedTime(a.loop_ms, loop_ev[0], loop_ev[1]);
    }
    if (ev) {
        for (int i = 0; i < 2 * a.steps * G; ++i) (void)hipEventDestroy(ev[i]);
        delete[] ev;
    }
    if (loop_ev[0]) { (void)hipEventDestroy(loop_ev[0]); (void)hipEventDestroy(loop_ev[1]); }
    return rc;
}

extern "C" int64_t set_sizeof_conv1d_args(void) { return (int64_t)sizeof(SetConv1dArgs); }
extern "C" int64_t set_sizeof_diffnet_layer_args(void) { return (int64_t)sizeof(SetDiffnetLayerArgs); }
extern "C" int64_t set_sizeof_diff_loop_args(void) { return (int64_t)sizeof(SetDiffLoopArgs); }
```

### speech-editing-toolkit_amd/csrc/diffnet_x3.hip

```cpp
#include <stdio.h>
#include <stdlib.h>

#include "common.h"

typedef __bf16 bf16x8_t __attribute__((ext_vector_type(8)));
typedef unsigned u32x4_t __attribute__((ext_vector_type(4)));
typedef unsigned u32x2_t __attribute__((ext_vector_type(2)));

__device__ uint64_t *g_x3_phase_buf = nullptr;
#ifndef SET_X3_PROBE
#define SET_X3_PROBE 0
#endif

namespace {

constexpr int XC = 256;
constexpr int X_MAXD = 8;
constexpr int XR = XC * 2 + 16;
constexpr int X_KS1 = 48;
constexpr int X_KS2 = 16;
constexpr float RSQRT2 = 0.70710678118654752440f;

__device__ __forceinline__ unsigned short f2bf(float x) { return __builtin_bit_cast(unsigned short, (__bf16)x); }
__device__ __forceinline__ float bf2f(unsigned short u) { return __builtin_bit_cast(float, (unsigned)u << 16); }
__device__ __forceinline__ void split3(float a, unsigned short &p0, unsigned short &p1, unsigned short &p2) {
    p0 = f2bf(a);
    const float r1 = a - bf2f(p0);
    p1 = f2bf(r1);
    p2 = f2bf(r1 - bf2f(p1));
}
typedef _Float16 f16x8_t __attribute__((ext_vector_type(8)));
__device__ __forceinline__ unsigned short f2h(float x) { return __builtin_bit_cast(unsigned short, (_Float16)x); }
__device__ __forceinline__ float h2f(unsigned short u) { return (float)__builtin_bit_cast(_Float16, u); }

struct SplitBf16x3 {
    static constexpr int NP = 3, NPROD = 6, MODE = 3, PF = 2, PF2 = 1;
    static __device__ __forceinline__ constexpr int qa(int t) { return t == 0 ? 2 : (t == 1 || t == 3) ? 1 : 0; }
    static __device__ __forceinline__ constexpr int qb(int t) { return t == 2 ? 2 : (t == 1 || t == 4) ? 1 : 0; }
    static __device__ __forceinline__ void split(float a, unsigned short (&p)[3]) { split3(a, p[0], p[1], p[2]); }
    static __device__ __forceinline__ f32x16 mma(u32x4_t a, u32x4_t b, f32x16 c) {
        return __builtin_amdgcn_mfma_f32_32x32x16_bf16(__builtin_bit_cast(bf16x8_t, a), __builtin_bit_cast(bf16x8_t, b), c, 0, 0, 0);
    }
};
struct SplitF16x2 {
    static constexpr int NP = 2, NPROD = 3, MODE = 2, PF = 4, PF2 = 2;
    static __device__ __forceinline__ constexpr int qa(int t) { return t == 0 ? 1 : 0; }
    static __device__ __forceinline__ constexpr int qb(int t) { return t == 1 ? 1 : 0; }
    static __device__ __forceinline__ void split(float a, unsigned short (&p)[2]) {
        p[0] = f2h(a);
        p[1] = f2h(a - h2f(p[0]));
    }
    static __device__ __forceinline__ void split2(float a, float b, unsigned (&p)[2]) { split2_f16(a, b, p[0], p[1]); }
    static __device__ __forceinline__ f32x16 mma(u32x4_t a, u32x4_t b, f32x16 c) {
        return __builtin_amdgcn_mfma_f32_32x32x16_f16(__builtin_bit_cast(f16x8_t, a), __builtin_bit_cast(f16x8_t, b), c, 0, 0, 0);
    }
};
template <typename S> constexpr int64_t x_n1() { return 8LL * X_KS1 * 2 * S::NP * 512; }
template <typename S> constexpr int64_t x_n2() { return 8LL * X_KS2 * 2 * S::NP * 512; }
constexpr int X_KSV = 32;
template <typename S> constexpr int64_t x_nv() { return S::MODE == 2 ? 8LL * X_KSV * 4 * S::NP * 512 + 8 : 0; }
template <typename S> constexpr int64_t x_nimg() { return x_n1<S>() + x_n2<S>() + 8 + x_nv<S>(); }
__device__ __forceinline__ u32x4_t buf_load_u4(rsrc_t r, unsigned voff, unsigned soff) {
    return __builtin_amdgcn_raw_buffer_load_b128(r, (int)voff, (int)soff, 0);
}
__device__ __forceinline__ float fsig(float x) { return __builtin_amdgcn_rcpf(1.0f + __expf(-x)); }
__device__ __forceinline__ float ftanh(float x) { return 1.0f - 2.0f * __builtin_amdgcn_rcpf(1.0f + __expf(2.0f * x)); }
__device__ __forceinline__ int urow(int r) { return (r & 3) + 8 * (r >> 2); }
constexpr int X_NT = 2;
__device__ __forceinline__ float buf_load_nt(rsrc_t r, unsigned voff, unsigned soff) {
    return __builtin_bit_cast(float, __builtin_amdgcn_raw_buffer_load_b32(r, (int)voff, (int)soff, X_NT));
}

template <typename S>
__global__ void __launch_bounds__(256) pack_layer_x3_kernel(const float *wdil, const float *wout, unsigned short *img, float s1, float s2) {
    const int64_t idx = (int64_t)blockIdx.x * 256 + threadIdx.x;
    constexpr int64_t n1 = x_n1<S>() / S::NP, n2 = x_n2<S>() / S::NP;
    constexpr int64_t nv = x_nv<S>() > 0 ? (x_nv<S>() - 8) / S::NP : 0;
    if (idx == 0) {
        float *tail = reinterpret_cast<float *>(img + x_n1<S>() + x_n2<S>());
        tail[0] = s1; tail[1] = 1.0f / s1; tail[2] = s2; tail[3] = 1.0f / s2;
        if (nv > 0) {
            float *tw = reinterpret_cast<float *>(img + x_nimg<S>() - 8);
            tw[0] = 0.5f * s1; tw[1] = 1.0f / (0.5f * s1); tw[2] = 0.0f; tw[3] = 0.0f;
        }
    }
    if (idx >= n1 + n2 + nv) return;
    if (idx >= n1 + n2) {
        int64_t r = idx - n1 - n2;
        const int e = r & 7; r >>= 3;
        const int l = r & 63; r >>= 6;
        const int mb = r & 3; r >>= 2;
        const int ks = (int)(r % X_KSV), w = (int)(r / X_KSV);
        const int row = (mb >= 2 ? XC : 0) + 32 * w + 16 * (mb & 1) + (l & 15), k = 8 * (l >> 4) + e;
        const int plane = ks >> 3, c = 32 * (ks & 7) + k;
        const float *g = wdil + ((int64_t)row * XC + c) * 3;
        const double g0 = g[0], g1 = g[1], gg2 = g[2];
        const double u = plane == 0 ? 0.5 * (g0 + g1 + gg2) : (plane == 1 ? 0.5 * (g0 - g1 + gg2) : (plane == 2 ? g0 : -gg2));
        unsigned short p[S::NP];
        S::split((0.5f * s1) * (float)u, p);
        unsigned short *base = img + x_n1<S>() + x_n2<S>() + 8 + ((((int64_t)w * X_KSV + ks) * 4 + mb) * S::NP) * 512 + l * 8 + e;
#pragma unroll
        for (int q = 0; q < S::NP; ++q) base[q * 512] = p[q];
        return;
    }
    const bool g2 = idx >= n1;
    int64_t r = g2 ? idx - n1 : idx;
    const int e = r & 7; r >>= 3;
    const int l = r & 63; r >>= 6;
    const int rb = r & 1; r >>= 1;
    const int nks = g2 ? X_KS2 : X_KS1;
    const int ks = (int)(r % nks), w = (int)(r / nks);
    const int row = (rb ? XC : 0) + 32 * w + (l & 31), k = 8 * (l >> 5) + e;
    const float v = g2 ? s2 * wout[(int64_t)row * XC + 16 * ks + k] : s1 * wdil[((int64_t)row * XC + 16 * (ks % 16) + k) * 3 + ks / 16];
    unsigned short p[S::NP];
    S::split(v, p);
    unsigned short *base = img + (g2 ? x_n1<S>() : 0) + ((((int64_t)w * nks + ks) * 2 + rb) * S::NP) * 512 + l * 8 + e;
#pragma unroll
    for (int q = 0; q < S::NP; ++q) base[q * 512] = p[q];
}

template <typename S, int NKS, int NU, int NCB, int PF, typename BF>
__device__ __forceinline__ void gemm_x3(f32x16 (&acc)[NU][2][NCB], rsrc_t img, unsigned lane16, unsigned abase, unsigned ustride,
                                        const unsigned char *lds, unsigned piece_bytes, BF bfrag) {
    constexpr int NP = S::NP;
    static_assert(NKS % PF == 0, "k-steps must be a multiple of the prefetch distance");
    u32x4_t A[PF][NU][2][NP];
#pragma unroll
    for (int p = 0; p < PF; ++p)
#pragma unroll
        for (int u = 0; u < NU; ++u)
#pragma unroll
            for (int rb = 0; rb < 2; ++rb)
#pragma unroll
                for (int q = 0; q < NP; ++q)
                    A[p][u][rb][q] = buf_load_u4(img, lane16, abase + (unsigned)u * ustride + (unsigned)(((p * 2 + rb) * NP + q) * 1024));
    for (int kb = 0; kb < NKS; kb += PF) {
#pragma unroll
        for (int p = 0; p < PF; ++p) {
            const int ks = kb + p;
            u32x4_t Bv[NCB][NP];
#pragma unroll
            for (int cb = 0; cb < NCB; ++cb) {
                const unsigned bo = bfrag(ks, cb);
#pragma unroll
                for (int q = 0; q < NP; ++q) Bv[cb][q] = *reinterpret_cast<const u32x4_t *>(lds + q * piece_bytes + bo);
            }
            __builtin_amdgcn_sched_barrier(0);
            __builtin_amdgcn_s_setprio(1);
#pragma unroll
            for (int t = 0; t < S::NPROD; ++t)
#pragma unroll
                for (int u = 0; u < NU; ++u)
#pragma unroll
                    for (int rb = 0; rb < 2; ++rb)
#pragma unroll
                        for (int cb = 0; cb < NCB; ++cb)
                            acc[u][rb][cb] = S::mma(A[p][u][rb][S::qa(t)], Bv[cb][S::qb(t)], acc[u][rb][cb]);
            __builtin_amdgcn_s_setprio(0);
            const int kn = min(ks + PF, NKS - 1);
#pragma unroll
            for (int u = 0; u < NU; ++u)
#pragma unroll
                for (int rb = 0; rb < 2; ++rb)
#pragma unroll
                    for (int q = 0; q < NP; ++q)
                        A[p][u][rb][q] = buf_load_u4(img, lane16, abase + (unsigned)u * ustride + (unsigned)(((kn * 2 + rb) * NP + q) * 1024));
            __builtin_amdgcn_sched_barrier(0);
        }
    }
}

template <typename S, int NCB>
constexpr size_t x3_lds_bytes(int max_dil) {
    return (size_t)S::NP * (size_t)(NCB * (32 + 2 * max_dil) * XR) + NCB * XC * sizeof(float) + 16;
}

struct X3Tile {
    const float *xin;
    float *xout, *skp;
    const float *cp;
    const float *dstep;
    int64_t cp_bs, d_bs, d_cs;
    const unsigned short *img;
    const float *b_dil, *b_out;
    int32_t *err_flag;
    int T, dil, first;
    int q0, nbu, Q;
};

struct X3Col {
    int b, t0;
    bool ok;
};
__device__ __forceinline__ X3Col x3_col(const X3Tile &a, int cb) {
    const int q = a.q0 + cb, qc = min(q, a.Q - 1);
    X3Col c;
    c.b = qc / a.nbu;
    c.t0 = (qc - c.b * a.nbu) * 32;
    c.ok = q < a.Q;
    return c;
}

template <int NP>
__device__ __forceinline__ void pack8(const unsigned short (&p)[8][NP], u32x4_t (&u)[NP]) {
#pragma unroll
    for (int q = 0; q < NP; ++q)
#pragma unroll
        for (int e = 0; e < 4; ++e) u[q][e] = (unsigned)p[2 * e][q] | ((unsigned)p[2 * e + 1][q] << 16);
}

template <int NU, int NCB>
__device__ __forceinline__ void x3_init(const X3Tile &a, f32x16 (&acc)[NU][2][NCB]) {
    const int lane = threadIdx.x & 63;
    const int w = __builtin_amdgcn_readfirstlane(threadIdx.x >> 6);
    const int half = lane >> 5, l31 = lane & 31;
    const int T = a.T;
    const unsigned T4 = 4u * (unsigned)T;
#pragma unroll
    for (int cb = 0; cb < NCB; ++cb) {
        const X3Col c = x3_col(a, cb);
        const rsrc_t rcp = make_rsrc(a.cp + (int64_t)c.b * a.cp_bs);
        const unsigned vo4 = 4u * (unsigned)(4 * half * T + min(c.t0 + l31, T - 1));
#pragma unroll
        for (int u = 0; u < NU; ++u)
#pragma unroll
            for (int rb = 0; rb < 2; ++rb) {
                const float *bd = a.b_dil + (rb ? XC : 0) + 32 * (NU * w + u);
#pragma unroll
                for (int r = 0; r < 16; ++r) {
                    const unsigned ur = (unsigned)((rb ? XC : 0) + 32 * (NU * w + u) + urow(r));
                    const float blo = bd[urow(r)], bhi = bd[urow(r) + 4];
                    acc[u][rb][cb][r] = (half ? bhi : blo) + buf_load_nt(rcp, vo4, ur * T4);
                }
            }
    }
}

template <typename S, int NU, int NCB>
__device__ __forceinline__ void x3_main(const X3Tile &a, f32x16 (&acc)[NU][2][NCB], unsigned char *lds, unsigned piece_bytes, uint64_t *dbg,
                                        uint64_t &tprev) {
#define X3_PHASE(p)                                           \
    if (dbg) {                                                \
        const uint64_t tn = __builtin_amdgcn_s_memtime();     \
        dbg[p] += tn - tprev;                                 \
        tprev = tn;                                           \
    }
    X3_PHASE(0)
    constexpr int NP = S::NP;
    constexpr int NW = 8 / NU, NT = 64 * NW;
    const int tid = threadIdx.x, lane = tid & 63;
    const int w = __builtin_amdgcn_readfirstlane(tid >> 6);
    const int half = lane >> 5, l31 = lane & 31;
    const int T = a.T, d = a.dil;
    const int RB = 32 + 2 * d;
    float *dsh = reinterpret_cast<float *>(lds + NP * piece_bytes);
    const unsigned T4 = 4u * (unsigned)T;
    const rsrc_t rw = make_rsrc(a.img);
    const unsigned lane16 = 16u * (unsigned)lane;
    auto row0 = [&](int u, int rb) { return (rb ? XC : 0) + 32 * (NU * w + u); };
    const float *sc = reinterpret_cast<const float *>(a.img + x_n1<S>() + x_n2<S>());
    const float s1 = sc[0], is1 = sc[1], s2 = sc[2], is2 = sc[3];
    bool tv[NCB];
    unsigned vo4[NCB];
    int64_t ub[NCB];
#pragma unroll
    for (int cb = 0; cb < NCB; ++cb) {
        const X3Col c = x3_col(a, cb);
        const int t = c.t0 + l31;
        tv[cb] = c.ok && t < T;
        vo4[cb] = 4u * (unsigned)(4 * half * T + min(t, T - 1));
        ub[cb] = (int64_t)c.b * XC * T;
    }

    {
        constexpr int NCG = (NW / NCB) * 2, CHG = XC / NCG, CPT = CHG < 32 ? CHG : 32, NPASS = CHG / CPT;
        const int cbs = w % NCB, fr = lane & 31, cg = (w / NCB) * 2 + (lane >> 5);
        const X3Col c = x3_col(a, cbs);
        const rsrc_t rx = make_rsrc(a.xin + (int64_t)c.b * XC * T);
#pragma unroll
        for (int i0 = 0; i0 < XC * NCB; i0 += NT) {
            const int idx = i0 + tid;
            if (NT <= XC * NCB || idx < XC * NCB) {
                const X3Col cd = x3_col(a, idx >> 8);
                dsh[idx] = a.dstep[(int64_t)cd.b * a.d_bs + (int64_t)(idx & 255) * a.d_cs];
            }
        }
        float amax = 0.0f;
        auto put = [&](int jj, int ch0, const float (&v)[CPT], bool valid) {
#pragma unroll
            for (int q8 = 0; q8 < CPT / 8; ++q8) {
                unsigned short p[8][NP];
                const f32x4 d0 = *reinterpret_cast<const f32x4 *>(dsh + XC * cbs + ch0 + 8 * q8);
                const f32x4 d1 = *reinterpret_cast<const f32x4 *>(dsh + XC * cbs + ch0 + 8 * q8 + 4);
#pragma unroll
                for (int e = 0; e < 8; ++e) {
                    const int ch = 8 * q8 + e;
                    const float xs = v[ch] + (e < 4 ? d0[e & 3] : d1[e & 3]);
                    const float xv = valid ? xs : 0.0f;
                    if constexpr (S::MODE == 2) amax = fmaxf(amax, fabsf(xv));
                    S::split(xv, p[e]);
                }
                u32x4_t u[NP];
                pack8<NP>(p, u);
#pragma unroll
                for (int q = 0; q < NP; ++q)
                    *reinterpret_cast<u32x4_t *>(lds + q * piece_bytes + (cbs * RB + jj) * XR + (ch0 + 8 * q8) * 2) = u[q];
            }
        };
        const int t = c.t0 - d + fr, th = c.t0 - d + 32 + fr;
        const bool tvx = c.ok && t >= 0 && t < T, has_h = fr < 2 * d, tvh = c.ok && th >= 0 && th < T;
#pragma unroll
        for (int ps = 0; ps < NPASS; ++ps) {
            const int ch0 = CHG * cg + CPT * ps;
            const unsigned cgo = (unsigned)ch0 * T4;
            const unsigned vox = 4u * (unsigned)min(max(t, 0), T - 1) + cgo, voh = 4u * (unsigned)min(max(th, 0), T - 1) + cgo;
            float vx[CPT], vh[CPT];
#pragma unroll
            for (int k = 0; k < CPT; ++k) vx[k] = buf_load(rx, vox, (unsigned)k * T4);
            if (has_h) {
#pragma unroll
                for (int k = 0; k < CPT; ++k) vh[k] = buf_load(rx, voh, (unsigned)k * T4);
            }
            if (ps == 0) __syncthreads();
            put(fr, ch0, vx, tvx);
            if (has_h) put(32 + fr, ch0, vh, tvh);
        }
        if constexpr (S::MODE == 2) {
            if (!(amax < 32768.0f) && a.err_flag) __hip_atomic_store(a.err_flag, 2, __ATOMIC_RELAXED, __HIP_MEMORY_SCOPE_AGENT);
        }
    }
    if constexpr (NU != 1) x3_init<NU, NCB>(a, acc);
#pragma unroll
    for (int u = 0; u < NU; ++u)
#pragma unroll
        for (int rb = 0; rb < 2; ++rb)
#pragma unroll
            for (int cb = 0; cb < NCB; ++cb)
#pragma unroll
                for (int r = 0; r < 16; ++r) acc[u][rb][cb][r] *= s1;
    __syncthreads();
    X3_PHASE(1)

    gemm_x3<S, X_KS1, NU, NCB, (NU == 1 ? S::PF : S::PF2)>(
        acc, rw, lane16, (unsigned)(NU * w * X_KS1 * 2 * NP * 1024), (unsigned)(X_KS1 * 2 * NP * 1024), lds, piece_bytes, [&](int ks, int cb) {
            return (unsigned)((cb * RB + l31 + (ks >> 4) * d) * XR + ((ks & 15) * 16 + half * 8) * 2);
        });
    X3_PHASE(2)

    float xres[NU][NCB][16];
    auto load_xres = [&]() {
#pragma unroll
        for (int cb = 0; cb < NCB; ++cb) {
            const rsrc_t rx = make_rsrc(a.xin + ub[cb]);
#pragma unroll
            for (int u = 0; u < NU; ++u)
#pragma unroll
                for (int r = 0; r < 16; ++r) xres[u][cb][r] = buf_load(rx, vo4[cb], (unsigned)(row0(u, 0) + urow(r)) * T4);
        }
    };
    if constexpr (NU == 1) load_xres();
    __syncthreads();
    X3_PHASE(8)
#pragma unroll
    for (int u = 0; u < NU; ++u)
#pragma unroll
        for (int cb = 0; cb < NCB; ++cb)
#pragma unroll
            for (int g = 0; g < 4; ++g) {
                unsigned short p[4][NP];
#pragma unroll
                for (int e = 0; e < 4; ++e) {
                    const int r = 4 * g + e;
                    const float zz = fsig(acc[u][0][cb][r] * is1) * ftanh(acc[u][1][cb][r] * is1);
                    const float z = tv[cb] ? zz : 0.0f;
                    S::split(z, p[e]);
                }
                const unsigned off = (unsigned)((cb * 32 + l31) * XR + (32 * (NU * w + u) + 8 * g + 4 * half) * 2);
#pragma unroll
                for (int q = 0; q < NP; ++q) {
                    u32x2_t uu;
                    uu[0] = (unsigned)p[0][q] | ((unsigned)p[1][q] << 16);
                    uu[1] = (unsigned)p[2][q] | ((unsigned)p[3][q] << 16);
                    *reinterpret_cast<u32x2_t *>(lds + q * piece_bytes + off) = uu;
                }
            }
    X3_PHASE(9)
    if constexpr (NU != 1) load_xres();
#pragma unroll
    for (int u = 0; u < NU; ++u)
#pragma unroll
        for (int rb = 0; rb < 2; ++rb) {
            const float *bo = a.b_out + row0(u, rb);
#pragma unroll
            for (int r = 0; r < 16; ++r) {
                const float blo = bo[urow(r)], bhi = bo[urow(r) + 4];
                const float bias = half ? bhi : blo;
#pragma unroll
                for (int cb = 0; cb < NCB; ++cb) acc[u][rb][cb][r] = (rb == 0 ? bias + xres[u][cb][r] : bias) * s2;
            }
        }
    float sk[NU][NCB][16];
    auto load_sk = [&]() {
#pragma unroll
        for (int cb = 0; cb < NCB; ++cb) {
            const rsrc_t rsk = make_rsrc(a.skp + ub[cb]);
#pragma unroll
            for (int u = 0; u < NU; ++u)
#pragma unroll
                for (int r = 0; r < 16; ++r) sk[u][cb][r] = buf_load_nt(rsk, vo4[cb], (unsigned)(32 * (NU * w + u) + urow(r)) * T4);
        }
    };
    if constexpr (NU == 1) load_sk();
    X3_PHASE(10)
    __syncthreads();
    X3_PHASE(3)

    gemm_x3<S, X_KS2, NU, NCB, (NU == 1 ? S::PF : S::PF2)>(
        acc, rw, lane16, (unsigned)(x_n1<S>() * 2 + NU * w * X_KS2 * 2 * NP * 1024), (unsigned)(X_KS2 * 2 * NP * 1024), lds, piece_bytes,
        [&](int ks, int cb) { return (unsigned)((cb * 32 + l31) * XR + (ks * 16 + half * 8) * 2); });
    X3_PHASE(4)

#pragma unroll
    for (int cb = 0; cb < NCB; ++cb) {
        if (tv[cb]) {
            const rsrc_t rxo = make_rsrc(a.xout + ub[cb]);
#pragma unroll
            for (int u = 0; u < NU; ++u)
#pragma unroll
                for (int r = 0; r < 16; ++r)
                    buf_store_agent((acc[u][0][cb][r] * is2) * RSQRT2, rxo, vo4[cb], (unsigned)(row0(u, 0) + urow(r)) * T4);
        }
    }
    const bool first = a.first != 0;
    if constexpr (NU != 1) {
        if (!first) load_sk();
    }
#pragma unroll
    for (int cb = 0; cb < NCB; ++cb) {
        if (tv[cb]) {
            const rsrc_t rsk = make_rsrc(a.skp + ub[cb]);
#pragma unroll
            for (int u = 0; u < NU; ++u)
#pragma unroll
                for (int r = 0; r < 16; ++r)
                    buf_store_agent(first ? acc[u][1][cb][r] * is2 : acc[u][1][cb][r] * is2 + sk[u][cb][r], rsk, vo4[cb],
                                    (unsigned)(32 * (NU * w + u) + urow(r)) * T4);
        }
    }
}
#undef X3_PHASE

template <typename S, int NU, int NCB>
__global__ void __launch_bounds__(512 / NU, NU) diffnet_stack_x3_kernel(SetDiffnetStackArgs a, int tiles_per_utt, int ntiles, int ntasks,
                                                                        unsigned piece_bytes, int fault_tile) {
    extern __shared__ __attribute__((aligned(16))) unsigned char lds[];
    int *s_task = reinterpret_cast<int *>(lds + S::NP * piece_bytes + NCB * XC * sizeof(float));
    int *counter = a.sync_ws, *abort_flag = a.sync_ws + 1, *done = a.sync_ws + 4;
    const int tid = threadIdx.x;
    uint64_t *dbg = (SET_X3_PROBE && blockIdx.x == 0 && tid == 0) ? g_x3_phase_buf : nullptr;
    uint64_t tprev = dbg ? __builtin_amdgcn_s_memtime() : 0;
    if (tid == 0) s_task[0] = atomicAdd(counter, 1);
    __syncthreads();
    int n = __builtin_amdgcn_readfirstlane(s_task[0]);
    int i_done = -1, l_done = 0;
    while (n < ntasks) {
        const int l = n / ntiles, i = n - l * ntiles, j = i;
        X3Tile lt;
        lt.xin = (l & 1) ? a.xb : a.xa;
        lt.xout = (l & 1) ? a.xa : a.xb;
        lt.skp = a.skip;
        lt.cp = a.condproj + (int64_t)l * a.cp_ls; lt.cp_bs = a.cp_bs;
        lt.dstep = a.dstep + (int64_t)l * a.d_ls; lt.d_bs = a.d_bs; lt.d_cs = a.d_cs;
        lt.img = reinterpret_cast<const unsigned short *>(a.wx3_all) + (int64_t)l * x_nimg<S>();
        lt.b_dil = a.b_dil_all + (int64_t)l * 512;
        lt.b_out = a.b_out_all + (int64_t)l * 512;
        lt.err_flag = a.err_flag;
        lt.T = a.T; lt.dil = 1 << (l % a.dilation_cycle_length); lt.first = (l == 0);
        lt.nbu = (a.T + 31) / 32; lt.Q = a.B * lt.nbu; lt.q0 = i * NCB;
        f32x16 acc[NU][2][NCB];
        if constexpr (NU == 1) x3_init<NU, NCB>(lt, acc);
        __builtin_amdgcn_sched_barrier(0);
        const int *f0 = done + i, *fl = done + (j > 0 ? i - 1 : i), *fr = done + (j < tiles_per_utt - 1 ? i + 1 : i);
        int peek = l, claimed = 0;
        if (tid == 0) {
            if (l > 0) peek = min(ld_agent(f0), min(ld_agent(fl), ld_agent(fr)));
            claimed = atomicAdd(counter, 1);
        }
        if (dbg) { const uint64_t tn = __builtin_amdgcn_s_memtime(); dbg[11] += tn - tprev; tprev = tn; }
        asm volatile("s_waitcnt vmcnt(0)" ::: "memory");
        if (dbg) { const uint64_t tn = __builtin_amdgcn_s_memtime(); dbg[12] += tn - tprev; tprev = tn; }
        if (tid == 0) {
            if (peek >= l) __builtin_amdgcn_fence(__ATOMIC_ACQUIRE, "agent");
            s_task[0] = claimed;
            s_task[1] = peek >= l ? 1 : 2;
        }
        __syncthreads();
        if (tid == 0 && i_done >= 0 && !(l_done == 0 && i_done == fault_tile))
            __hip_atomic_store(done + i_done, l_done + 1, __ATOMIC_RELAXED, __HIP_MEMORY_SCOPE_AGENT);
        i_done = -1;
        if (__builtin_amdgcn_readfirstlane(s_task[1]) == 2) {
            if (tid == 0) {
                int ok = 1;
                unsigned spins = 0;
                for (;;) {
                    const int v0 = ld_agent(f0), v1 = ld_agent(fl), v2 = ld_agent(fr);
                    if (min(v0, min(v1, v2)) >= l) break;
                    __builtin_amdgcn_s_sleep(8);
                    if (++spins > STACK_SPIN_LIMIT || ld_agent(abort_flag) != 0) {
                        __hip_atomic_store(abort_flag, 1, __ATOMIC_RELAXED, __HIP_MEMORY_SCOPE_AGENT);
                        if (a.err_flag) __hip_atomic_store(a.err_flag, 1, __ATOMIC_RELAXED, __HIP_MEMORY_SCOPE_AGENT);
                        ok = 0;
                        break;
                    }
                }
                __builtin_amdgcn_fence(__ATOMIC_ACQUIRE, "agent");
                s_task[2] = ok;
            }
            __syncthreads();
            if (__builtin_amdgcn_readfirstlane(s_task[2]) == 0) break;
        }
        const int n_next = __builtin_amdgcn_readfirstlane(s_task[0]);
        x3_main<S, NU, NCB>(lt, acc, lds, piece_bytes, dbg, tprev);
        i_done = i;
        l_done = l;
        n = n_next;
        if (dbg) {
            const uint64_t tn = __builtin_amdgcn_s_memtime();
            dbg[5] += tn - tprev;
            dbg[7] += 1;
            tprev = tn;
        }
    }
    asm volatile("s_waitcnt vmcnt(0)" ::: "memory");
    __syncthreads();
    if (tid == 0 && i_done >= 0 && !(l_done == 0 && i_done == fault_tile))
        __hip_atomic_store(done + i_done, l_done + 1, __ATOMIC_RELAXED, __HIP_MEMORY_SCOPE_AGENT);
}

template <typename S, int NU, int NCB>
int launch_x3(const SetDiffnetStackArgs &a, int n_cu, int fault_tile, hipStream_t s) {
    static SetDeviceOnce lds_once;
    if (int rc = set_lds_optin(lds_once, 160 * 1024, "set_diffnet_stack(x3 attr)", diffnet_stack_x3_kernel<S, NU, NCB>)) return rc;
    const int Q = a.B * ((a.T + 31) / 32);
    const int ntiles = (Q + NCB - 1) / NCB, tiles_per_utt = ntiles;
    const int64_t ntasks64 = (int64_t)ntiles * a.L;
    SET_REQUIRE(ntasks64 < (1ll << 30), "set_diffnet_stack(task count)");
    SET_REQUIRE((int64_t)2 * XC * a.T * 4 < ((int64_t)1 << 31), "set_diffnet_stack(split-operand kernel: T too large)");
    const int max_dil = 1 << (a.dilation_cycle_length - 1);
    const unsigned piece_bytes = (unsigned)(NCB * (32 + 2 * max_dil) * XR);
    const size_t ldsz = x3_lds_bytes<S, NCB>(max_dil);
    SET_HIP(set_zero_async(a.sync_ws, (size_t)(4 + ntiles) * sizeof(int32_t), s), "set_diffnet_stack(memset)");
    int grid = NU * n_cu;
    if (grid > ntiles * 4 / 5) grid = ntiles * 4 / 5;
    if (const char *e = getenv("SET_AMD_STACK_GRID")) grid = atoi(e) > 0 ? atoi(e) : grid;
    if ((int64_t)grid > ntasks64) grid = (int)ntasks64;
    if (grid < 1) grid = 1;
    hipLaunchKernelGGL((diffnet_stack_x3_kernel<S, NU, NCB>), dim3(grid), dim3(512 / NU), ldsz, s, a, tiles_per_utt, ntiles, (int)ntasks64,
                       piece_bytes, fault_tile);
    return set_check_launch("set_diffnet_stack");
}

typedef unsigned u32x2w_t __attribute__((ext_vector_type(2)));
typedef float f32x2 __attribute__((ext_vector_type(2)));
__device__ __forceinline__ f32x2 buf_load2(rsrc_t r, unsigned voff, unsigned soff) {
    return __builtin_bit_cast(f32x2, __builtin_amdgcn_raw_buffer_load_b64(r, (int)voff, (int)soff, 0));
}
__device__ __forceinline__ f32x2 buf_load2_nt(rsrc_t r, unsigned voff, unsigned soff) {
    return __builtin_bit_cast(f32x2, __builtin_amdgcn_raw_buffer_load_b64(r, (int)voff, (int)soff, X_NT));
}

constexpr int XRV = XC * 2 + 32;
template <int NB> constexpr unsigned xv_piece() { return 16 * NB * XRV; }
template <int NB> constexpr unsigned xv_plane() { return 2 * xv_piece<NB>(); }
template <int NB> constexpr unsigned xv_zpiece() { return 32 * NB * XR; }
template <int NB> constexpr unsigned xv_tile() { return 2 * xv_plane<NB>() > 2 * xv_zpiece<NB>() ? 2 * xv_plane<NB>() : 2 * xv_zpiece<NB>(); }
constexpr int XV_PF = 2;
constexpr int XV_PF2 = 2;
constexpr int X3V_FLAG_UNIT = 8;

__device__ __forceinline__ f32x4 mma16(u32x4_t a, u32x4_t b, f32x4 c) {
    return __builtin_amdgcn_mfma_f32_16x16x32_f16(__builtin_bit_cast(f16x8_t, a), __builtin_bit_cast(f16x8_t, b), c, 0, 0, 0);
}
__device__ __forceinline__ float row_prev(float v) {
    return __builtin_bit_cast(float, __builtin_amdgcn_update_dpp(0, __builtin_bit_cast(int, v), 0x111, 0xf, 0xf, false));
}
__device__ __forceinline__ float row_next(float v) {
    return __builtin_bit_cast(float, __builtin_amdgcn_update_dpp(0, __builtin_bit_cast(int, v), 0x101, 0xf, 0xf, false));
}

template <int NB>
__device__ __forceinline__ void x3v_init(const X3Tile &a, f32x4 (&PQ)[2][4][NB]) {
    typedef SplitF16x2 S;
    int tid = threadIdx.x;
    asm volatile("" : "+v"(tid));
    const int lane = tid & 63;
    const int w = __builtin_amdgcn_readfirstlane(tid >> 6);
    const int l15 = lane & 15, kg = lane >> 4;
    const int T = a.T;
    const unsigned T4 = 4u * (unsigned)T;
    const float hs = 0.5f * reinterpret_cast<const float *>(a.img + x_nimg<S>() - 8)[0];
    f32x4 bias[4];
#pragma unroll
    for (int mb = 0; mb < 4; ++mb) bias[mb] = *reinterpret_cast<const f32x4 *>(a.b_dil + (mb >= 2 ? XC : 0) + 32 * w + 16 * (mb & 1) + 4 * kg);
#pragma unroll
    for (int nb = 0; nb < NB; ++nb) {
        const X3Col c = x3_col(a, nb);
        const rsrc_t rcp = make_rsrc(a.cp + (int64_t)c.b * a.cp_bs);
        const unsigned vo = 4u * (unsigned)(4 * kg * T + min(c.t0 + 2 * l15, T - 2));
#pragma unroll
        for (int mb = 0; mb < 4; ++mb) {
            const unsigned row0 = (unsigned)((mb >= 2 ? XC : 0) + 32 * w + 16 * (mb & 1));
#pragma unroll
            for (int i = 0; i < 4; ++i) {
                const f32x2 v = buf_load2_nt(rcp, vo, (row0 + (unsigned)i) * T4);
                const float e = bias[mb][i] + v[0], o = bias[mb][i] + v[1];
                PQ[0][mb][nb][i] = hs * (e + o);
                PQ[1][mb][nb][i] = hs * (e - o);
            }
        }
    }
}

template <int NB, int PH>
__device__ __forceinline__ void x3v_stage_load(const X3Tile &a, int w, int lane, f32x2 (&x12)[NB][8], float (&xh)[NB][8]) {
    const int l15 = lane & 15, cs = lane >> 4;
    const int ch0 = 32 * w + 8 * cs;
    const int T = a.T;
    const unsigned T4 = 4u * (unsigned)T;
    const bool edge = l15 == 0 || l15 == 15;
#pragma unroll
    for (int nb = 0; nb < NB; ++nb) {
        const X3Col c = x3_col(a, nb);
        const rsrc_t rx = make_rsrc(a.xin + (int64_t)c.b * XC * T);
        const int t = c.t0 + 2 * l15;
        const unsigned vox = 4u * (unsigned)min(t, T - 2) + (unsigned)ch0 * T4;
#pragma unroll
        for (int k = 0; k < 8; ++k) x12[nb][k] = buf_load2(rx, vox, (unsigned)k * T4);
        if (PH == 1) {
            const int th = l15 == 0 ? c.t0 - 1 : c.t0 + 32;
            const unsigned voh = 4u * (unsigned)min(max(th, 0), T - 1) + (unsigned)ch0 * T4;
            if (edge) {
#pragma unroll
                for (int k = 0; k < 8; ++k) xh[nb][k] = buf_load(rx, voh, (unsigned)k * T4);
            }
        }
    }
}
template <int NB, int PH>
__device__ __forceinline__ float x3v_stage_store(const X3Tile &a, unsigned char *lds, const float *dsh, int w, int lane, const f32x2 (&x12)[NB][8],
                                                 const float (&xh)[NB][8]) {
    typedef SplitF16x2 S;
    const int l15 = lane & 15, cs = lane >> 4;
    const int ch0 = 32 * w + 8 * cs;
    const int T = a.T;
    const bool edge = l15 == 0 || l15 == 15;
    float amax = 0.0f;
#pragma unroll
    for (int nb = 0; nb < NB; ++nb) {
        const X3Col c = x3_col(a, nb);
        const int t = c.t0 + 2 * l15, th = l15 == 0 ? c.t0 - 1 : c.t0 + 32;
        const bool v12 = c.ok && t < T, vh = c.ok && edge && th >= 0 && th < T;
        const f32x4 dA = *reinterpret_cast<const f32x4 *>(dsh + nb * XC + ch0);
        const f32x4 dB = *reinterpret_cast<const f32x4 *>(dsh + nb * XC + ch0 + 4);
        u32x4_t u[2][2];
#pragma unroll
        for (int e2 = 0; e2 < 4; ++e2) {
            float V[2][2];
#pragma unroll
            for (int h = 0; h < 2; ++h) {
                const int e = 2 * e2 + h;
                const float ds = e < 4 ? dA[e & 3] : dB[e & 3];
                const float d1 = v12 ? x12[nb][e][0] + ds : 0.0f, d2 = v12 ? x12[nb][e][1] + ds : 0.0f;
                if (PH == 0) {
                    V[0][h] = d1 + d2;
                    V[1][h] = d2 - d1;
                } else {
                    float d0 = row_prev(d2), d3 = row_next(d1);
                    const float hv = vh ? xh[nb][e] + ds : 0.0f;
                    d0 = l15 == 0 ? hv : d0;
                    d3 = l15 == 15 ? hv : d3;
                    V[0][h] = d0 - d2;
                    V[1][h] = d1 - d3;
                }
            }
#pragma unroll
            for (int j = 0; j < 2; ++j) {
                amax = fmaxf(fmaxf(amax, fabsf(V[j][0])), fabsf(V[j][1]));
                unsigned pw[2];
                S::split2(V[j][0], V[j][1], pw);
                u[j][0][e2] = pw[0];
                u[j][1][e2] = pw[1];
            }
        }
#pragma unroll
        for (int j = 0; j < 2; ++j)
#pragma unroll
            for (int q = 0; q < 2; ++q) *reinterpret_cast<u32x4_t *>(lds + j * xv_plane<NB>() + q * xv_piece<NB>() + (16 * nb + l15) * XRV + ch0 * 2) = u[j][q];
    }
    return amax;
}

template <int NB, int PFV>
__device__ __forceinline__ void x3v_plane(f32x4 (&acc)[4][NB], u32x4_t (&A)[PFV][4][2], rsrc_t img, unsigned lane16, unsigned abase, int seg,
                                          const unsigned char *bplane, unsigned boff) {
    typedef SplitF16x2 S;
    const int ks_last = 16 * (seg >> 1) + 15;
    for (int kb = 0; kb < 8; kb += PFV) {
#pragma unroll
        for (int p = 0; p < PFV; ++p) {
            const int kc = kb + p, ks = 8 * seg + kc;
            u32x4_t Bv[NB][2];
#pragma unroll
            for (int nb = 0; nb < NB; ++nb)
#pragma unroll
                for (int q = 0; q < 2; ++q) Bv[nb][q] = *reinterpret_cast<const u32x4_t *>(bplane + q * xv_piece<NB>() + boff + (unsigned)(nb * 16 * XRV) + (unsigned)kc * 64u);
            __builtin_amdgcn_sched_barrier(0);
            __builtin_amdgcn_s_setprio(1);
#pragma unroll
            for (int t = 0; t < S::NPROD; ++t)
#pragma unroll
                for (int mb = 0; mb < 4; ++mb)
#pragma unroll
                    for (int nb = 0; nb < NB; ++nb) acc[mb][nb] = mma16(A[p][mb][S::qa(t)], Bv[nb][S::qb(t)], acc[mb][nb]);
            __builtin_amdgcn_s_setprio(0);
            const int kn = min(ks + PFV, ks_last);
#pragma unroll
            for (int mb = 0; mb < 4; ++mb)
#pragma unroll
                for (int q = 0; q < 2; ++q) A[p][mb][q] = buf_load_u4(img, lane16, abase + (unsigned)(((kn * 4 + mb) * 2 + q) * 1024));
            __builtin_amdgcn_sched_barrier(0);
        }
    }
}

template <int NB>
__device__ __forceinline__ void x3v_main(const X3Tile &a, f32x4 (&PQ)[2][4][NB], unsigned char *lds, uint64_t *dbg, uint64_t &tprev, uint64_t (&ts)[32]) {
#if SET_X3_PROBE == 2
#define X3V_PHASE(p)                                  \
    {                                                 \
        __builtin_amdgcn_sched_barrier(0);            \
        ts[8 + (p)] = __builtin_amdgcn_s_memtime();   \
        __builtin_amdgcn_sched_barrier(0);            \
    }
#else
#define X3V_PHASE(p)                                          \
    if (dbg) {                                                \
        const uint64_t tn = __builtin_amdgcn_s_memtime();     \
        dbg[p] += tn - tprev;                                 \
        tprev = tn;                                           \
    }
#endif
#if SET_X3_PROBE == 2
#define X3V_TS(p) X3V_PHASE(p)
#else
#define X3V_TS(p)
#endif
    X3V_PHASE(0)
    typedef SplitF16x2 S;
    constexpr int PFV = XV_PF;
    int tid = threadIdx.x;
    asm volatile("" : "+v"(tid));
    const int lane = tid & 63;
    const int w = __builtin_amdgcn_readfirstlane(tid >> 6);
    const int l15 = lane & 15, kg = lane >> 4;
    const int half = lane >> 5, l31 = lane & 31;
    const int T = a.T;
    const unsigned T4 = 4u * (unsigned)T;
    const unsigned lane16 = 16u * (unsigned)lane;
    float *dsh = reinterpret_cast<float *>(lds + xv_tile<NB>());
    const rsrc_t rw = make_rsrc(a.img);
    const float *sc = reinterpret_cast<const float *>(a.img + x_n1<S>() + x_n2<S>());
    const float s2 = sc[2], is2 = sc[3];
    const float is1w = reinterpret_cast<const float *>(a.img + x_nimg<S>() - 8)[1];
    const float cg2 = is1w * -1.4426950408889634f, cf2 = is1w * 2.8853900817779268f;
    const unsigned abase = (unsigned)((x_n1<S>() + x_n2<S>() + 8) * 2) + (unsigned)(w * X_KSV * 4 * 2 * 1024);
    const unsigned boff = (unsigned)(l15 * XRV + kg * 16);
    u32x4_t A[PFV][4][2];
    f32x2 x12[NB][8];
    float xh[NB][8];
    x3v_stage_load<NB, 0>(a, w, lane, x12, xh);
    float amax = x3v_stage_store<NB, 0>(a, lds, dsh, w, lane, x12, xh);
#pragma unroll
    for (int p = 0; p < PFV; ++p)
#pragma unroll
        for (int mb = 0; mb < 4; ++mb)
#pragma unroll
            for (int q = 0; q < 2; ++q) A[p][mb][q] = buf_load_u4(rw, lane16, abase + (unsigned)(((p * 4 + mb) * 2 + q) * 1024));
    X3V_TS(12)
    __syncthreads();
    X3V_PHASE(1)
    x3v_plane<NB, PFV>(PQ[0], A, rw, lane16, abase, 0, lds, boff);
    x3v_plane<NB, PFV>(PQ[1], A, rw, lane16, abase, 1, lds + xv_plane<NB>(), boff);
    X3V_PHASE(2)
    x3v_stage_load<NB, 1>(a, w, lane, x12, xh);
    __builtin_amdgcn_sched_barrier(0);
#pragma unroll
    for (int mb = 0; mb < 4; ++mb)
#pragma unroll
        for (int nb = 0; nb < NB; ++nb)
#pragma unroll
            for (int i = 0; i < 4; ++i) {
                const float pp = PQ[0][mb][nb][i], qq = PQ[1][mb][nb][i];
                PQ[0][mb][nb][i] = pp + qq;
                PQ[1][mb][nb][i] = pp - qq;
            }
    __syncthreads();
    X3V_TS(13)
    amax = fmaxf(amax, x3v_stage_store<NB, 1>(a, lds, dsh, w, lane, x12, xh));
    if (!(amax < 32768.0f) && a.err_flag) __hip_atomic_store(a.err_flag, 2, __ATOMIC_RELAXED, __HIP_MEMORY_SCOPE_AGENT);
#pragma unroll
    for (int p = 0; p < PFV; ++p)
#pragma unroll
        for (int mb = 0; mb < 4; ++mb)
#pragma unroll
            for (int q = 0; q < 2; ++q) A[p][mb][q] = buf_load_u4(rw, lane16, abase + (unsigned)((((16 + p) * 4 + mb) * 2 + q) * 1024));
    X3V_TS(14)
    __syncthreads();
    X3V_PHASE(3)
    x3v_plane<NB, PFV>(PQ[0], A, rw, lane16, abase, 2, lds, boff);
    x3v_plane<NB, PFV>(PQ[1], A, rw, lane16, abase, 3, lds + xv_plane<NB>(), boff);
    X3V_PHASE(4)
    bool tv[NB];
    unsigned vo4[NB];
    int64_t ub[NB];
#pragma unroll
    for (int cb = 0; cb < NB; ++cb) {
        const X3Col c = x3_col(a, cb);
        const int t = c.t0 + l31;
        tv[cb] = c.ok && t < T;
        vo4[cb] = 4u * (unsigned)(4 * half * T + min(t, T - 1));
        ub[cb] = (int64_t)c.b * XC * T;
    }
    float xres[NB][16];
#pragma unroll
    for (int cb = 0; cb < NB; ++cb) {
        const rsrc_t rx = make_rsrc(a.xin + ub[cb]);
#pragma unroll
        for (int r = 0; r < 16; ++r) xres[cb][r] = buf_load(rx, vo4[cb], (unsigned)(32 * w + urow(r)) * T4);
    }
    __syncthreads();
    X3V_TS(15)
#pragma unroll
    for (int nb = 0; nb < NB; ++nb) {
        const X3Col c = x3_col(a, nb);
        const bool tvp = c.ok && c.t0 + 2 * l15 < T;
#pragma unroll
        for (int eo = 0; eo < 2; ++eo)
#pragma unroll
            for (int m = 0; m < 2; ++m) {
                float zz[4];
#pragma unroll
                for (int i = 0; i < 4; ++i) {
                    const float u = __builtin_amdgcn_exp2f(PQ[eo][m][nb][i] * cg2);
                    const float v = __builtin_amdgcn_exp2f(fminf(PQ[eo][m + 2][nb][i] * cf2, 64.0f));
                    const float g = (v - 1.0f) * __builtin_amdgcn_rcpf((1.0f + u) * (1.0f + v));
                    zz[i] = tvp ? g : 0.0f;
                }
                unsigned plo[2], phi[2];
                S::split2(zz[0], zz[1], plo);
                S::split2(zz[2], zz[3], phi);
                const unsigned off = (unsigned)((32 * nb + 2 * l15 + eo) * XR + (32 * w + 16 * m + 4 * kg) * 2);
#pragma unroll
                for (int q = 0; q < 2; ++q) {
                    u32x2w_t uu;
                    uu[0] = plo[q];
                    uu[1] = phi[q];
                    *reinterpret_cast<u32x2w_t *>(lds + q * xv_zpiece<NB>() + off) = uu;
                }
            }
    }
    f32x16 acc[1][2][NB];
#pragma unroll
    for (int rb = 0; rb < 2; ++rb) {
        const float *bo = a.b_out + (rb ? XC : 0) + 32 * w;
#pragma unroll
        for (int r = 0; r < 16; ++r) {
            const float blo = bo[urow(r)], bhi = bo[urow(r) + 4];
            const float bias = half ? bhi : blo;
#pragma unroll
            for (int cb = 0; cb < NB; ++cb) acc[0][rb][cb][r] = (rb == 0 ? bias + xres[cb][r] : bias) * s2;
        }
    }
    X3V_TS(16)
    __syncthreads();
    X3V_PHASE(8)
    gemm_x3<S, X_KS2, 1, NB, XV_PF2>(acc, rw, lane16, (unsigned)(x_n1<S>() * 2 + w * X_KS2 * 2 * 2 * 1024), (unsigned)(X_KS2 * 2 * 2 * 1024), lds,
                                     xv_zpiece<NB>(), [&](int ks, int cb) { return (unsigned)((cb * 32 + l31) * XR + (ks * 16 + half * 8) * 2); });
    X3V_PHASE(9)
    const bool first = a.first != 0;
    float sk[NB][16];
    if (!first) {
#pragma unroll
        for (int cb = 0; cb < NB; ++cb) {
            const rsrc_t rsk = make_rsrc(a.skp + ub[cb]);
#pragma unroll
            for (int r = 0; r < 16; ++r) sk[cb][r] = buf_load_nt(rsk, vo4[cb], (unsigned)(32 * w + urow(r)) * T4);
        }
    }
#pragma unroll
    for (int cb = 0; cb < NB; ++cb) {
        if (tv[cb]) {
            const rsrc_t rxo = make_rsrc(a.xout + ub[cb]);
#pragma unroll
            for (int r = 0; r < 16; ++r) buf_store_agent((acc[0][0][cb][r] * is2) * RSQRT2, rxo, vo4[cb], (unsigned)(32 * w + urow(r)) * T4);
        }
    }
    X3V_TS(17)
#pragma unroll
    for (int cb = 0; cb < NB; ++cb) {
        if (tv[cb]) {
            const rsrc_t rsk = make_rsrc(a.skp + ub[cb]);
#pragma unroll
            for (int r = 0; r < 16; ++r)
                buf_store_agent(first ? acc[0][1][cb][r] * is2 : acc[0][1][cb][r] * is2 + sk[cb][r], rsk, vo4[cb], (unsigned)(32 * w + urow(r)) * T4);
        }
    }
    X3V_PHASE(10)
}
#undef X3V_PHASE
#undef X3V_TS

#if SET_X3_PROBE == 2
#ifndef X3V_TL_TASK
#define X3V_TL_TASK 10
#endif
#define X3V_KTS(p)                                \
    {                                             \
        __builtin_amdgcn_sched_barrier(0);        \
        ts[p] = __builtin_amdgcn_s_memtime();     \
        __builtin_amdgcn_sched_barrier(0);        \
    }
#else
#define X3V_KTS(p)
#endif
template <int NB>
__global__ void __launch_bounds__(512, 1) diffnet_stack_x3v_kernel(SetDiffnetStackArgs a, int ntiles, int ntasks, int fault_tile) {
    typedef SplitF16x2 S;
    extern __shared__ __attribute__((aligned(16))) unsigned char lds[];
    int *s_task = reinterpret_cast<int *>(lds + xv_tile<NB>() + NB * XC * sizeof(float));
    int *counter = a.sync_ws, *abort_flag = a.sync_ws + 1, *done = a.sync_ws + 4;
    const int tid = threadIdx.x;
    uint64_t *dbg = (SET_X3_PROBE == 1 && blockIdx.x == 0 && tid == 0) ? g_x3_phase_buf : nullptr;
    uint64_t tprev = dbg ? __builtin_amdgcn_s_memtime() : 0;
    if (tid == 0) s_task[0] = atomicAdd(counter, 1);
    __syncthreads();
    int n = __builtin_amdgcn_readfirstlane(s_task[0]);
    int i_done = -1, l_done = 0;
    uint64_t ts[32] = {};
    int n_mine = 0;
    (void)n_mine;
    while (n < ntasks) {
        const int l = n / ntiles, i = n - l * ntiles;
        X3Tile lt;
        lt.xin = (l & 1) ? a.xb : a.xa;
        lt.xout = (l & 1) ? a.xa : a.xb;
        lt.skp = a.skip;
        lt.cp = a.condproj + (int64_t)l * a.cp_ls; lt.cp_bs = a.cp_bs;
        lt.dstep = a.dstep + (int64_t)l * a.d_ls; lt.d_bs = a.d_bs; lt.d_cs = a.d_cs;
        lt.img = reinterpret_cast<const unsigned short *>(a.wx3_all) + (int64_t)l * x_nimg<S>();
        lt.b_dil = a.b_dil_all + (int64_t)l * 512;
        lt.b_out = a.b_out_all + (int64_t)l * 512;
        lt.err_flag = a.err_flag;
        lt.T = a.T; lt.dil = 1; lt.first = (l == 0);
        lt.nbu = (a.T + 31) / 32; lt.Q = a.B * lt.nbu; lt.q0 = i * NB;
        f32x4 PQ[2][4][NB];
        X3V_KTS(0)
        if (i_done >= 0) {
            asm volatile("s_waitcnt vmcnt(0)" ::: "memory");
            if ((tid & 63) == 0 && !(l_done == 0 && i_done == fault_tile))
                (void)__hip_atomic_fetch_add(done + i_done, 1, __ATOMIC_RELAXED, __HIP_MEMORY_SCOPE_AGENT);
            i_done = -1;
        }
        __builtin_amdgcn_sched_barrier(0);
        float dsv[(NB * XC + 511) / 512];
#pragma unroll
        for (int j = 0; j < (NB * XC + 511) / 512; ++j) {
            const int idx = min(tid + 512 * j, NB * XC - 1);
            dsv[j] = lt.dstep[(int64_t)x3_col(lt, idx >> 8).b * lt.d_bs + (int64_t)(idx & (XC - 1)) * lt.d_cs];
        }
        x3v_init<NB>(lt, PQ);
        __builtin_amdgcn_sched_barrier(0);
        const int *f0 = done + i, *fl = done + (i > 0 ? i - 1 : i), *fr = done + (i < ntiles - 1 ? i + 1 : i);
        int peek = l, claimed = 0;
        if (tid == 0) {
            if (l > 0) peek = min(ld_agent(f0), min(ld_agent(fl), ld_agent(fr))) / X3V_FLAG_UNIT;
            claimed = atomicAdd(counter, 1);
        }
        X3V_KTS(1)
        asm volatile("s_waitcnt vmcnt(0)" ::: "memory");
        X3V_KTS(2)
        {
            float *dsh = reinterpret_cast<float *>(lds + xv_tile<NB>());
#pragma unroll
            for (int j = 0; j < (NB * XC + 511) / 512; ++j)
                if (tid + 512 * j < NB * XC) dsh[tid + 512 * j] = dsv[j];
        }
        if (tid == 0) {
            if (peek >= l) __builtin_amdgcn_fence(__ATOMIC_ACQUIRE, "agent");
            s_task[0] = claimed;
            s_task[1] = peek >= l ? 1 : 2;
        }
        __syncthreads();
        X3V_KTS(3)
        if (__builtin_amdgcn_readfirstlane(s_task[1]) == 2) {
            if (tid == 0) {
                int ok = 1;
                unsigned spins = 0;
                for (;;) {
                    const int v0 = ld_agent(f0), v1 = ld_agent(fl), v2 = ld_agent(fr);
                    if (min(v0, min(v1, v2)) >= l * X3V_FLAG_UNIT) break;
                    __builtin_amdgcn_s_sleep(8);
                    if (++spins > STACK_SPIN_LIMIT || ld_agent(abort_flag) != 0) {
                        __hip_atomic_store(abort_flag, 1, __ATOMIC_RELAXED, __HIP_MEMORY_SCOPE_AGENT);
                        if (a.err_flag) __hip_atomic_store(a.err_flag, 1, __ATOMIC_RELAXED, __HIP_MEMORY_SCOPE_AGENT);
                        ok = 0;
                        break;
                    }
                }
                __builtin_amdgcn_fence(__ATOMIC_ACQUIRE, "agent");
                s_task[2] = ok;
            }
            __syncthreads();
            if (__builtin_amdgcn_readfirstlane(s_task[2]) == 0) break;
        }
        const int n_next = __builtin_amdgcn_readfirstlane(s_task[0]);
        X3V_KTS(4)
        x3v_main<NB>(lt, PQ, lds, dbg, tprev, ts);
#if SET_X3_PROBE == 2
        if (++n_mine == X3V_TL_TASK && (tid == 0 || tid == 448) && g_x3_phase_buf) {
            const rsrc_t rt = make_rsrc(g_x3_phase_buf);
            const unsigned row = (unsigned)(2 * blockIdx.x + (tid ? 1 : 0)) * 128u;
#pragma unroll
            for (int k = 0; k < 32; ++k) __builtin_amdgcn_raw_buffer_store_b32((unsigned)(ts[k] - ts[0]), rt, (int)(row + 4 * k), 0, 0);
            __builtin_amdgcn_raw_buffer_store_b32((unsigned)n, rt, (int)(row + 20), 0, 0);
            __builtin_amdgcn_raw_buffer_store_b32((unsigned)s_task[1], rt, (int)(row + 24), 0, 0);
            __builtin_amdgcn_raw_buffer_store_b32((unsigned)ts[0], rt, (int)(row + 28), 0, 0);
        } else if (n_mine == X3V_TL_TASK + 1 && (tid == 0 || tid == 448) && g_x3_phase_buf) {
            __builtin_amdgcn_raw_buffer_store_b32((unsigned)ts[0], make_rsrc(g_x3_phase_buf), (int)((unsigned)(2 * blockIdx.x + (tid ? 1 : 0)) * 128u + 124u), 0, 0);
        }
#endif
        i_done = i;
        l_done = l;
        n = n_next;
        if (dbg) {
            const uint64_t tn = __builtin_amdgcn_s_memtime();
            dbg[5] += tn - tprev;
            dbg[7] += 1;
            tprev = tn;
        }
    }
    asm volatile("s_waitcnt vmcnt(0)" ::: "memory");
    if ((tid & 63) == 0 && i_done >= 0 && !(l_done == 0 && i_done == fault_tile))
        (void)__hip_atomic_fetch_add(done + i_done, 1, __ATOMIC_RELAXED, __HIP_MEMORY_SCOPE_AGENT);
}

template <int NB>
int launch_x3v(const SetDiffnetStackArgs &a, int n_cu, int fault_tile, hipStream_t s) {
    static SetDeviceOnce lds_once;
    if (int rc = set_lds_optin(lds_once, 160 * 1024, "set_diffnet_stack(x3v attr)", diffnet_stack_x3v_kernel<NB>)) return rc;
    const int Q = a.B * ((a.T + 31) / 32);
    const int ntiles = (Q + NB - 1) / NB;
    const int64_t ntasks64 = (int64_t)ntiles * a.L;
    SET_REQUIRE(ntasks64 < (1ll << 30), "set_diffnet_stack(task count)");
    SET_REQUIRE((int64_t)2 * XC * a.T * 4 < ((int64_t)1 << 31), "set_diffnet_stack(split-operand kernel: T too large)");
    SET_REQUIRE(a.dilation_cycle_length == 1 && a.T % 2 == 0, "set_diffnet_stack(x3v: dilation 1 and even T only)");
    const size_t ldsz = (size_t)xv_tile<NB>() + NB * XC * sizeof(float) + 16;
    SET_HIP(set_zero_async(a.sync_ws, (size_t)(4 + ntiles) * sizeof(int32_t), s), "set_diffnet_stack(memset)");
    int grid = n_cu;
    if (NB == 2 && grid > ntiles * 4 / 5) grid = ntiles * 4 / 5;
    if (const char *e = getenv("SET_AMD_STACK_GRID")) grid = atoi(e) > 0 ? atoi(e) : grid;
    if ((int64_t)grid > ntasks64) grid = (int)ntasks64;
    if (grid < 1) grid = 1;
    hipLaunchKernelGGL(diffnet_stack_x3v_kernel<NB>, dim3(grid), dim3(512), ldsz, s, a, ntiles, (int)ntasks64, fault_tile);
    return set_check_launch("set_diffnet_stack");
}


constexpr int SX_PF = 8;

__device__ __forceinline__ float buf_load_sc1(rsrc_t r, unsigned voff, unsigned soff) {
    return __builtin_bit_cast(float, __builtin_amdgcn_raw_buffer_load_b32(r, (int)voff, (int)soff, 16));
}
__device__ __forceinline__ u32x4_t buf_load_u4_sc1(rsrc_t r, unsigned voff, unsigned soff) {
    return __builtin_amdgcn_raw_buffer_load_b128(r, (int)voff, (int)soff, 16);
}

__device__ __forceinline__ bool sx_wait(const int *f0, const int *f1, const int *f2, int want, int *abort_flag, int *err_flag, bool fence = true) {
    unsigned spins = 0;
    for (;;) {
        const int v0 = ld_agent(f0), v1 = ld_agent(f1), v2 = ld_agent(f2);
        if (min(v0, min(v1, v2)) >= want) break;
        __builtin_amdgcn_s_sleep(1);
        if (++spins > SPLIT_SPIN_LIMIT || ld_agent(abort_flag) != 0) {
            __hip_atomic_store(abort_flag, 1, __ATOMIC_RELAXED, __HIP_MEMORY_SCOPE_AGENT);
            if (err_flag) __hip_atomic_store(err_flag, 1, __ATOMIC_RELAXED, __HIP_MEMORY_SCOPE_AGENT);
            return false;
        }
    }
    if (fence) __builtin_amdgcn_fence(__ATOMIC_ACQUIRE, "agent");
    return true;
}

template <int NKS, typename BF>
__device__ __forceinline__ void sx_gemm(f32x16 &acc, u32x4_t (&A)[SX_PF][2], rsrc_t img, unsigned lane16, unsigned abase,
                                        const unsigned char *lds, unsigned piece_bytes, BF bfrag) {
    unsigned bo = bfrag(0);
    u32x4_t b0 = *reinterpret_cast<const u32x4_t *>(lds + bo);
    u32x4_t b1 = *reinterpret_cast<const u32x4_t *>(lds + piece_bytes + bo);
#pragma unroll 1
    for (int kb = 0; kb < NKS; kb += SX_PF) {
#pragma unroll
        for (int p = 0; p < SX_PF; ++p) {
            const int ks = kb + p;
            const unsigned bn = bfrag(min(ks + 1, NKS - 1));
            const u32x4_t nb0 = *reinterpret_cast<const u32x4_t *>(lds + bn);
            const u32x4_t nb1 = *reinterpret_cast<const u32x4_t *>(lds + piece_bytes + bn);
            acc = SplitF16x2::mma(A[p][1], b0, acc);
            acc = SplitF16x2::mma(A[p][0], b1, acc);
            acc = SplitF16x2::mma(A[p][0], b0, acc);
            const int kn = min(ks + SX_PF, NKS - 1);
            A[p][0] = buf_load_u4(img, lane16, abase + (unsigned)(kn * 4 * 1024));
            A[p][1] = buf_load_u4(img, lane16, abase + (unsigned)((kn * 4 + 1) * 1024));
            b0 = nb0;
            b1 = nb1;
            __builtin_amdgcn_sched_barrier(0);
        }
    }
}
__device__ __forceinline__ void sx_preload(u32x4_t (&A)[SX_PF][2], rsrc_t img, unsigned lane16, unsigned abase) {
#pragma unroll
    for (int p = 0; p < SX_PF; ++p) {
        A[p][0] = buf_load_u4(img, lane16, abase + (unsigned)(p * 4 * 1024));
        A[p][1] = buf_load_u4(img, lane16, abase + (unsigned)((p * 4 + 1) * 1024));
    }
}

__global__ void __launch_bounds__(256, 1) diffnet_stack_split_x2_kernel(SetDiffnetStackArgs a, int tiles_per_utt, int ntiles,
                                                                         unsigned piece_bytes, int fault_tile, int nofence) {
    typedef SplitF16x2 S;
    extern __shared__ __attribute__((aligned(16))) unsigned char lds[];
    float *gs = reinterpret_cast<float *>(lds + 2 * piece_bytes);
    float *dsh = gs + 64 * 32;
    int *s_ok = reinterpret_cast<int *>(dsh + XC);
    int *abort_flag = a.sync_ws + 1, *ready = a.sync_ws + 4, *zcnt = a.sync_ws + 4 + ntiles;
    const int tid = threadIdx.x, lane = tid & 63, half = lane >> 5, l31 = lane & 31;
    const int j = __builtin_amdgcn_readfirstlane(tid >> 6);
    if ((int)blockIdx.x >= 4 * ntiles) {
        const int hp = blockIdx.x & 3;
        for (int l = 1; l < a.L; ++l) {
            unsigned spins = 0;
            while (l >= 2 && ld_agent(ready) < 4 * (l - 1)) {
                __builtin_amdgcn_s_sleep(8);
                if (++spins > SPLIT_SPIN_LIMIT || ld_agent(abort_flag) != 0) return;
            }
            const unsigned char *img = reinterpret_cast<const unsigned char *>(a.wx3_all) + (int64_t)l * x_nimg<S>() * 2;
            const rsrc_t r1 = make_rsrc(img + (size_t)(2 * hp) * X_KS1 * 4 * 1024);
            const rsrc_t r2 = make_rsrc(img + x_n1<S>() * 2 + (size_t)(2 * hp) * X_KS2 * 4 * 1024);
            for (unsigned off = 16u * tid; off < 2u * X_KS1 * 4 * 1024; off += 8u * 4096u) {
#pragma unroll
                for (unsigned q = 0; q < 8; ++q) {
                    const u32x4_t v = buf_load_u4(r1, off + q * 4096u, 0u);
                    asm volatile("" ::"v"(v));
                }
            }
            for (unsigned off = 16u * tid; off < 2u * X_KS2 * 4 * 1024; off += 8u * 4096u) {
#pragma unroll
                for (unsigned q = 0; q < 8; ++q) {
                    const u32x4_t v = buf_load_u4(r2, off + q * 4096u, 0u);
                    asm volatile("" ::"v"(v));
                }
            }
        }
        return;
    }
    const int i = blockIdx.x >> 2, h = blockIdx.x & 3;
    const int b = i / tiles_per_utt, jt = i - b * tiles_per_utt;
    const int T = a.T, t0 = jt * 32;
    const int il = jt > 0 ? i - 1 : i, ir = jt < tiles_per_utt - 1 ? i + 1 : i;
    const unsigned T4 = 4u * (unsigned)T;
    const int w8 = 2 * h + (j & 1), rb = j >> 1;
    const int ch0 = 32 * w8;
    const int tq = t0 + l31;
    const bool tv = tq < T;
    const unsigned vo4 = 4u * (unsigned)(4 * half * T + min(tq, T - 1));
    const unsigned lane16 = 16u * (unsigned)lane;
    unsigned short *zt = reinterpret_cast<unsigned short *>(a.z_ws) + (int64_t)i * (2 * 32 * XC);
    const rsrc_t rz = make_rsrc(zt);
    const rsrc_t rsk = make_rsrc(a.skip + (int64_t)b * XC * T);
    uint64_t *dbg = (SET_X3_PROBE && blockIdx.x == 5 && tid == 0) ? g_x3_phase_buf : nullptr;
    uint64_t tprev = dbg ? __builtin_amdgcn_s_memtime() : 0;
#define SX_PHASE(p)                                           \
    if (dbg) {                                                \
        const uint64_t tn = __builtin_amdgcn_s_memtime();     \
        dbg[p] += tn - tprev;                                 \
        tprev = tn;                                           \
    }
    for (int l = 0; l < a.L; ++l) {
        const int d = 1 << (l % a.dilation_cycle_length);
        const unsigned short *img = reinterpret_cast<const unsigned short *>(a.wx3_all) + (int64_t)l * x_nimg<S>();
        const rsrc_t rw = make_rsrc(img);
        const float *sc = reinterpret_cast<const float *>(img + x_n1<S>() + x_n2<S>());
        const float s1 = sc[0], is1 = sc[1], s2 = sc[2], is2 = sc[3];
        const rsrc_t rxin = make_rsrc(((l & 1) ? a.xb : a.xa) + (int64_t)b * XC * T);
        const rsrc_t rxout = make_rsrc(((l & 1) ? a.xa : a.xb) + (int64_t)b * XC * T);
        const rsrc_t rcp = make_rsrc(a.condproj + (int64_t)l * a.cp_ls + (int64_t)b * a.cp_bs);
        const float *dstep = a.dstep + (int64_t)l * a.d_ls + (int64_t)b * a.d_bs;
        const float *bd = a.b_dil_all + (int64_t)l * 512 + rb * XC + ch0, *bo = a.b_out_all + (int64_t)l * 512 + rb * XC + ch0;
        u32x4_t A[SX_PF][2];
        const unsigned ab1 = (unsigned)(((w8 * X_KS1) * 2 + rb) * 2 * 1024);
        sx_preload(A, rw, lane16, ab1);
        f32x16 acc;
#pragma unroll
        for (int r = 0; r < 16; ++r) {
            const float blo = bd[urow(r)], bhi = bd[urow(r) + 4];
            acc[r] = (half ? bhi : blo) + buf_load(rcp, vo4, (unsigned)(rb * XC + ch0 + urow(r)) * T4);
        }
        if (tid == 0) *s_ok = (l == 0 || sx_wait(ready + i, ready + il, ready + ir, 4 * l, abort_flag, a.err_flag, !nofence)) ? 1 : 0;
        __syncthreads();
        if (__builtin_amdgcn_readfirstlane(*s_ok) == 0) return;
        SX_PHASE(0)
        {
            const int f = tid & 31, cg = tid >> 5;
            dsh[tid] = dstep[(int64_t)tid * a.d_cs];
            float amax = 0.0f;
            auto put = [&](int row, const float (&v)[32], bool valid) {
#pragma unroll
                for (int q8 = 0; q8 < 4; ++q8) {
                    unsigned short p[8][2];
                    const f32x4 d0 = *reinterpret_cast<const f32x4 *>(dsh + 32 * cg + 8 * q8);
                    const f32x4 d1 = *reinterpret_cast<const f32x4 *>(dsh + 32 * cg + 8 * q8 + 4);
#pragma unroll
                    for (int e = 0; e < 8; ++e) {
                        const float xs = v[8 * q8 + e] + (e < 4 ? d0[e & 3] : d1[e & 3]);
                        const float xv = valid ? xs : 0.0f;
                        amax = fmaxf(amax, fabsf(xv));
                        S::split(xv, p[e]);
                    }
                    u32x4_t u[2];
                    pack8<2>(p, u);
                    *reinterpret_cast<u32x4_t *>(lds + row * XR + (32 * cg + 8 * q8) * 2) = u[0];
                    *reinterpret_cast<u32x4_t *>(lds + piece_bytes + row * XR + (32 * cg + 8 * q8) * 2) = u[1];
                }
            };
            const int t = t0 - d + f, th = t0 - d + 32 + f;
            const bool tvx = t >= 0 && t < T, has_h = f < 2 * d, tvh = th >= 0 && th < T;
            const unsigned vox = 4u * (unsigned)min(max(t, 0), T - 1), voh = 4u * (unsigned)min(max(th, 0), T - 1);
            float vx[32], vh[32];
            if (nofence) {
#pragma unroll
                for (int k = 0; k < 32; ++k) vx[k] = buf_load_sc1(rxin, vox, (unsigned)(32 * cg + k) * T4);
                if (has_h) {
#pragma unroll
                    for (int k = 0; k < 32; ++k) vh[k] = buf_load_sc1(rxin, voh, (unsigned)(32 * cg + k) * T4);
                }
            } else {
#pragma unroll
                for (int k = 0; k < 32; ++k) vx[k] = buf_load(rxin, vox, (unsigned)(32 * cg + k) * T4);
                if (has_h) {
#pragma unroll
                    for (int k = 0; k < 32; ++k) vh[k] = buf_load(rxin, voh, (unsigned)(32 * cg + k) * T4);
                }
            }
            __syncthreads();
            put(f, vx, tvx);
            if (has_h) put(32 + f, vh, tvh);
            if (!(amax < 32768.0f) && a.err_flag) __hip_atomic_store(a.err_flag, 2, __ATOMIC_RELAXED, __HIP_MEMORY_SCOPE_AGENT);
        }
#pragma unroll
        for (int r = 0; r < 16; ++r) acc[r] *= s1;
        __syncthreads();
        SX_PHASE(1)
        sx_gemm<X_KS1>(acc, A, rw, lane16, ab1, lds, piece_bytes, [&](int ks) {
            return (unsigned)((l31 + (ks >> 4) * d) * XR + ((ks & 15) * 16 + half * 8) * 2);
        });
        SX_PHASE(2)
        if (rb == 1) {
#pragma unroll
            for (int r = 0; r < 16; ++r) gs[(32 * (j & 1) + urow(r) + 4 * half) * 32 + l31] = ftanh(acc[r] * is1);
        }
        __syncthreads();
        if (rb == 0) {
#pragma unroll
            for (int g = 0; g < 4; ++g) {
                unsigned short p[4][2];
#pragma unroll
                for (int e = 0; e < 4; ++e) {
                    const int r = 4 * g + e;
                    const float zz = fsig(acc[r] * is1) * gs[(32 * (j & 1) + urow(r) + 4 * half) * 32 + l31];
                    S::split(tv ? zz : 0.0f, p[e]);
                }
                const unsigned off = (unsigned)(l31 * (XC * 2) + (ch0 + 8 * g + 4 * half) * 2);
#pragma unroll
                for (int q = 0; q < 2; ++q) {
                    u32x2_t u;
                    u[0] = (unsigned)p[0][q] | ((unsigned)p[1][q] << 16);
                    u[1] = (unsigned)p[2][q] | ((unsigned)p[3][q] << 16);
                    __builtin_amdgcn_raw_buffer_store_b64(u, rz, (int)(off + (unsigned)q * (32u * XC * 2u)), 0, 16);
                }
            }
        }
        asm volatile("s_waitcnt vmcnt(0)" ::: "memory");
        __syncthreads();
        if (tid == 0) __hip_atomic_fetch_add(zcnt + i, 1, __ATOMIC_RELAXED, __HIP_MEMORY_SCOPE_AGENT);
        SX_PHASE(3)
        const unsigned ab2 = (unsigned)(x_n1<S>() * 2 + ((w8 * X_KS2) * 2 + rb) * 2 * 1024);
        sx_preload(A, rw, lane16, ab2);
        float prev[16];
        {
            const rsrc_t rp = make_rsrc(rb == 0 ? ((l & 1) ? a.xb : a.xa) + (int64_t)b * XC * T : a.skip + (int64_t)b * XC * T);
#pragma unroll
            for (int r = 0; r < 16; ++r) prev[r] = buf_load(rp, vo4, (unsigned)(ch0 + urow(r)) * T4);
        }
#pragma unroll
        for (int r = 0; r < 16; ++r) {
            const float blo = bo[urow(r)], bhi = bo[urow(r) + 4];
            const float bias = half ? bhi : blo;
            acc[r] = (rb == 0 ? bias + prev[r] : bias) * s2;
        }
        if (tid == 0) *s_ok = sx_wait(zcnt + i, zcnt + i, zcnt + i, 4 * (l + 1), abort_flag, a.err_flag, !nofence) ? 1 : 0;
        __syncthreads();
        if (__builtin_amdgcn_readfirstlane(*s_ok) == 0) return;
        SX_PHASE(4)
        {
            u32x4_t zv[8];
#pragma unroll
            for (int k = 0; k < 8; ++k)
                zv[k] = nofence ? buf_load_u4_sc1(rz, 16u * (unsigned)tid, 4096u * (unsigned)k) : buf_load_u4(rz, 16u * (unsigned)tid, 4096u * (unsigned)k);
#pragma unroll
            for (int k = 0; k < 8; ++k) {
                const int unit = tid + 256 * k;
                const int q = unit >> 10, fr = (unit >> 5) & 31, part = unit & 31;
                *reinterpret_cast<u32x4_t *>(lds + q * piece_bytes + fr * XR + part * 16) = zv[k];
            }
        }
        __syncthreads();
        SX_PHASE(5)
        sx_gemm<X_KS2>(acc, A, rw, lane16, ab2, lds, piece_bytes, [&](int ks) {
            return (unsigned)(l31 * XR + (ks * 16 + half * 8) * 2);
        });
        SX_PHASE(6)
        if (tv && rb == 0) {
#pragma unroll
            for (int r = 0; r < 16; ++r) buf_store_agent((acc[r] * is2) * RSQRT2, rxout, vo4, (unsigned)(ch0 + urow(r)) * T4);
        } else if (tv) {
            const bool first = l == 0;
#pragma unroll
            for (int r = 0; r < 16; ++r)
                buf_store(first ? acc[r] * is2 : acc[r] * is2 + prev[r], rsk, vo4, (unsigned)(ch0 + urow(r)) * T4);
        }
        asm volatile("s_waitcnt vmcnt(0)" ::: "memory");
        __syncthreads();
        if (tid == 0 && !(l == 0 && i == fault_tile && h == 0))
            __hip_atomic_fetch_add(ready + i, 1, __ATOMIC_RELAXED, __HIP_MEMORY_SCOPE_AGENT);
        SX_PHASE(7)
    }
#undef SX_PHASE
}

}

int set_launch_diffnet_stack_split_x2(const SetDiffnetStackArgs &a, int fault_tile, hipStream_t s) {
    static SetDeviceOnce lds_once;
    if (int rc = set_lds_optin(lds_once, 80 * 1024, "set_diffnet_stack(split x2 attr)", diffnet_stack_split_x2_kernel)) return rc;
    const int tiles = (a.T + 31) / 32, nt = a.B * tiles;
    const int max_dil = 1 << (a.dilation_cycle_length - 1);
    const unsigned piece_bytes = (unsigned)((32 + 2 * max_dil) * XR);
    const size_t ldsz = (size_t)2 * piece_bytes + (64 * 32 + XC) * sizeof(float) + 16;
    SET_HIP(set_zero_async(a.sync_ws, (size_t)(4 + 2 * nt) * sizeof(int32_t), s), "set_diffnet_stack(memset)");
    int n_cu = 0;
    (void)set_cu_count(&n_cu);
    const int extra = (4 * nt + 8 <= n_cu && a.L > 1) ? 8 : 0;
    const int nofence = 1;
    hipLaunchKernelGGL(diffnet_stack_split_x2_kernel, dim3(4 * nt + extra), dim3(256), ldsz, s, a, tiles, nt, piece_bytes, fault_tile, nofence);
    return set_check_launch("set_diffnet_stack");
}

extern "C" int set_debug_x3_phase_buffer(uint64_t *buf) {
    SET_HIP(hipMemcpyToSymbol(HIP_SYMBOL(g_x3_phase_buf), &buf, sizeof(buf)), "set_debug_x3_phase_buffer");
    return SET_OK;
}

extern "C" int64_t set_diffnet_layer_x3_image_size(int32_t mode) {
    return mode == 2 ? x_nimg<SplitF16x2>() : (mode == 3 ? x_nimg<SplitBf16x3>() : -1);
}

extern "C" int set_pack_diffnet_layer_x3(const float *w_dil, const float *w_out, void *img, int32_t mode, int32_t k1, int32_t k2,
                                         void *stream) {
    SET_REQUIRE(w_dil && w_out && img && (mode == 2 || mode == 3), "set_pack_diffnet_layer_x3");
    SET_REQUIRE(k1 >= -60 && k1 <= 60 && k2 >= -60 && k2 <= 60, "set_pack_diffnet_layer_x3(scale exponents)");
    const float s1 = ldexpf(1.0f, k1), s2 = ldexpf(1.0f, k2);
    unsigned short *im = reinterpret_cast<unsigned short *>(img);
    if (mode == 2)
        hipLaunchKernelGGL(pack_layer_x3_kernel<SplitF16x2>, dim3(set_blocks((x_nimg<SplitF16x2>() - 16) / 2, 256)), dim3(256), 0,
                           (hipStream_t)stream, w_dil, w_out, im, s1, s2);
    else
        hipLaunchKernelGGL(pack_layer_x3_kernel<SplitBf16x3>, dim3(set_blocks((x_nimg<SplitBf16x3>() - 8) / 3, 256)), dim3(256), 0,
                           (hipStream_t)stream, w_dil, w_out, im, s1, s2);
    return set_check_launch("set_pack_diffnet_layer_x3");
}

int set_x3_winograd_selected(int x3_mode, int B, int T, int dilation_cycle_length, int n_cu) {
    if (x3_mode != 2 || dilation_cycle_length != 1 || T % 2 != 0) return 0;
    const int64_t tiles64 = (int64_t)B * ((T + 63) / 64);
    bool narrow = 5 * tiles64 < 3 * (int64_t)n_cu;
    if (const char *e = getenv("SET_AMD_X3_TILE")) narrow = atoi(e) == 32;
    if (narrow) return 0;
    if (const char *e = getenv("SET_AMD_X3_WINO")) {
        const int v = atoi(e);
        if (v <= 0) return 0;
        if (v == 2 || v == 3) return v;
    }
    const int64_t tiles96 = ((int64_t)B * ((T + 31) / 32) + 2) / 3;
    return tiles96 >= (int64_t)n_cu ? 3 : 2;
}

int set_launch_diffnet_stack_x3(const SetDiffnetStackArgs &a, int n_cu, int fault_tile, hipStream_t s) {
    SET_REQUIRE(a.x3_mode == 2 || a.x3_mode == 3, "set_diffnet_stack(x3_mode must be 2 = f16x2 or 3 = bf16x3)");
    const int64_t tiles64 = (int64_t)a.B * ((a.T + 63) / 64);
    bool narrow = 5 * tiles64 < 3 * (int64_t)n_cu;
    if (const char *e = getenv("SET_AMD_X3_TILE")) narrow = atoi(e) == 32;
    const bool al8 = ((reinterpret_cast<uintptr_t>(a.condproj) | reinterpret_cast<uintptr_t>(a.xa) | reinterpret_cast<uintptr_t>(a.xb)) & 7) == 0 &&
                     ((a.cp_bs | a.cp_ls) & 1) == 0;
    const int wino = al8 ? set_x3_winograd_selected(a.x3_mode, a.B, a.T, a.dilation_cycle_length, n_cu) : 0;
    if (wino == 3) return launch_x3v<3>(a, n_cu, fault_tile, s);
    if (wino == 2) return launch_x3v<2>(a, n_cu, fault_tile, s);
    if (a.x3_mode == 2)
        return narrow ? launch_x3<SplitF16x2, 1, 1>(a, n_cu, fault_tile, s) : launch_x3<SplitF16x2, 1, 2>(a, n_cu, fault_tile, s);
    return narrow ? launch_x3<SplitBf16x3, 1, 1>(a, n_cu, fault_tile, s) : launch_x3<SplitBf16x3, 1, 2>(a, n_cu, fault_tile, s);
}
```

### speech-editing-toolkit_amd/ops.py

```python
import collections
import ctypes as C
import math
import os
import typing

import torch

from . import _lib
from ._lib import (ACT, PRO, IMPL_BF16, IMPL_MFMA, IMPL_MFMA2, IMPL_NAIVE, SetConv1dArgs, SetDiffnetLayerArgs,
                   SetDiffLoopArgs, SetDiffnetStackArgs, check)

_DEFAULT_IMPL = os.environ.get("SET_AMD_CONV_IMPL", "auto")
_WEIGHTS_EPOCH = 0


_COMPUTE_DTYPE = os.environ.get("SET_AMD_DTYPE", "f32")


def set_compute_dtype(dtype):
    global _COMPUTE_DTYPE
    if dtype not in ("f32", "bf16"):
        raise ValueError("compute dtype must be 'f32' or 'bf16', got %r" % (dtype,))
    _COMPUTE_DTYPE = dtype

# ... 629 lines not shown
    return z


def res_skip(x_in, o, skip, first):
    _f(x_in), _f(o), _f(skip)
    B, Cc, T = x_in.shape
    x_out = torch.empty_like(x_in)
    check(_lib.lib().set_res_skip(_p(x_in), _p(o), _p(x_out), _p(skip), B, Cc, T, int(bool(first)), _stream()),
          "set_res_skip")
    return x_out


def pack_diffnet_layer(w_dil, w_out, w1p=None, w2p=None):
    _f(w_dil), _f(w_out)
    L = _lib.lib()
    if w1p is None:
        w1p = torch.empty(L.set_diffnet_w1p_size(), dtype=torch.float32, device=w_dil.device)
        w2p = torch.empty(L.set_diffnet_w2p_size(), dtype=torch.float32, device=w_dil.device)
    check(L.set_pack_diffnet_layer(_p(w_dil), _p(w_out), _p(_f(w1p)), _p(_f(w2p)), _stream()), "set_pack_diffnet_layer")
    return w1p, w2p


def pack_diffnet_layer_wino(w_dil, w_out, w1w, w2w):
    _f(w_dil), _f(w_out), _f(w1w), _f(w2w)
    check(_lib.lib().set_pack_diffnet_layer_wino(_p(w_dil), _p(w_out), _p(w1w), _p(w2w), _stream()),
          "set_pack_diffnet_layer_wino")


def sync_ws_size(B, T):
    return 160 + 2 * B * ((T + 31) // 32)


class SplitRangeError(_lib.SetAmdError):
    """An activation left the range of the fp16 operand splitting (the loop's output is not valid)."""


_SPLIT_MODE_OVERRIDE = [None]


def split_operand_mode():
    if _SPLIT_MODE_OVERRIDE[0] is not None:
        return _SPLIT_MODE_OVERRIDE[0]
    v = os.environ.get("SET_AMD_SPLIT_OPERAND", "f16x2").lower()
    if v not in ("f16x2", "bf16x3"):
        raise ValueError("SET_AMD_SPLIT_OPERAND must be f16x2 or bf16x3, not %r" % v)
    return 2 if v == "f16x2" else 3


class split_operand_mode_as:

    def __init__(self, mode):
        self.mode = mode

    def __enter__(self):
        self.prev, _SPLIT_MODE_OVERRIDE[0] = _SPLIT_MODE_OVERRIDE[0], self.mode

    def __exit__(self, *exc):
        _SPLIT_MODE_OVERRIDE[0] = self.prev


def _images_mask(have_wino, have_split, x3_mode):
    m = split_operand_mode() if x3_mode is None else int(x3_mode)
    return int(bool(have_wino)) | (2 if have_split else 0) | (4 if m == 3 else 0) | (8 if m == 2 else 0)


def stack_variant(B, T, dilation_cycle_length, have_wino=True, have_split=True, x3_mode=None):
    return int(_lib.lib().set_diffnet_stack_variant(int(B), int(T), int(dilation_cycle_length), _images_mask(have_wino, have_split, x3_mode)))


def stack_x3_winograd(B, T, dilation_cycle_length, have_wino=True, have_split=True, x3_mode=None):
    return int(_lib.lib().set_diffnet_stack_x3_winograd(int(B), int(T), int(dilation_cycle_length), _images_mask(have_wino, have_split, x3_mode)))


STACK_VARIANT_NAMES = {0: "diffnet_stack_kernel<2,4,2>", 1: "diffnet_stack_kernel<1,8,2>", 2: "diffnet_stack_wino_kernel",
                       3: "diffnet_stack_split_kernel", 4: "diffnet_stack_x3_kernel<SplitBf16x3>",
                       5: "diffnet_stack_x3_kernel<SplitF16x2>"}


class SplitOperandImages:

    def __init__(self, L, mode, device):
        self.mode = int(mode)
        n = int(_lib.lib().set_diffnet_layer_x3_image_size(self.mode))
        self.data = torch.empty(L, n, dtype=torch.int16, device=device)

    def pack(self, i, w_dil, w_out):
        _f(w_dil), _f(w_out)
        k1 = k2 = 0
        if self.mode == 2:
            import math
            m1, m2 = float(w_dil.abs().max()), float(w_out.abs().max())
            k1 = max(-60, min(60, 3 - math.frexp(m1)[1] + 1)) if m1 > 0 and math.isfinite(m1) else 0
            k2 = max(-60, min(60, 3 - math.frexp(m2)[1] + 1)) if m2 > 0 and math.isfinite(m2) else 0
        check(_lib.lib().set_pack_diffnet_layer_x3(_p(w_dil), _p(w_out), self.data[i].data_ptr(), self.mode, k1, k2, _stream()),
              "set_pack_diffnet_layer_x3")


def split_images(w1p_all, w2p_all):
    L = w1p_all.shape[0]
    return tuple(w.view(L, 4, -1, 64, 4).permute(0, 1, 4, 2, 3).contiguous().view(L, -1) for w in (w1p_all, w2p_all))


class StackImages(typing.NamedTuple):
    w1p: torch.Tensor
    w2p: torch.Tensor
    b_dil: torch.Tensor
    b_out: torch.Tensor
    w1w: typing.Optional[torch.Tensor] = None
    w2w: typing.Optional[torch.Tensor] = None
    w1s: typing.Optional[torch.Tensor] = None
    w2s: typing.Optional[torch.Tensor] = None
    wx3: typing.Optional[SplitOperandImages] = None


def _set_images(a, images, B, T, dcl, dev):
    if not isinstance(images, StackImages):
        raise TypeError("the layer stack takes its weight images as an ops.StackImages (fields by name), not %s: a bare tuple in the "
                        "wrong order would launch on the wrong image" % type(images).__name__)
    a.w1p_all, a.w2p_all = images.w1p.data_ptr(), images.w2p.data_ptr()
    a.b_dil_all, a.b_out_all = images.b_dil.data_ptr(), images.b_out.data_ptr()
    if images.w1w is not None:
        a.w1w_all, a.w2w_all = images.w1w.data_ptr(), images.w2w.data_ptr()
    x3 = images.wx3
    if x3 is not None:
        a.wx3_all, a.x3_mode = x3.data.data_ptr(), x3.mode
    if images.w1s is None or stack_variant(B, T, dcl, x3_mode=x3.mode if x3 is not None else 0) != 3:
        return None
    a.w1s_all, a.w2s_all = images.w1s.data_ptr(), images.w2s.data_ptr()
    z_ws = torch.empty(B * ((T + 31) // 32) * 256 * 32, dtype=torch.float32, device=dev)
    a.z_ws = z_ws.data_ptr()
    return z_ws


def diffnet_stack(xa, xb, skip, condproj, dstep_ptr, d_bs, d_cs, d_ls, images, dilation_cycle_length, sync_ws=None,
                  x_all=None, save_y=None, save_z=None, err_flag=None):
    B, Cc, T = xa.shape
    assert Cc == 256
    a = SetDiffnetStackArgs()
    z_ws = _set_images(a, images, B, T, dilation_cycle_length, xa.device)
    _f(xa), _f(xb), _f(skip), _f(condproj)
    L = images.b_dil.shape[0]
    if sync_ws is None:
        sync_ws = torch.empty(sync_ws_size(B, T), dtype=torch.int32, device=xa.device)
    a.xa, a.xb, a.skip = xa.data_ptr(), xb.data_ptr(), skip.data_ptr()
    a.condproj, a.dstep = condproj.data_ptr(), dstep_ptr
    if x_all is not None:
        a.x_all, a.save_y, a.save_z = _f(x_all).data_ptr(), _f(save_y).data_ptr(), _f(save_z).data_ptr()
    if err_flag is not None:
        a.err_flag = err_flag.data_ptr()
    a.sync_ws = sync_ws.data_ptr()
    a.cp_bs, a.cp_ls = condproj.stride(0), 512 * T
    a.d_bs, a.d_cs, a.d_ls = int(d_bs), int(d_cs), int(d_ls)
    a.B, a.T, a.L, a.dilation_cycle_length = B, T, L, int(dilation_cycle_length)
    check(_lib.lib().set_diffnet_stack(C.byref(a), _stream()), "set_diffnet_stack")
    return sync_ws


def diffnet_layer(x_in, condproj, cp_bs, dstep, d_bs, d_cs, w1p, b_dil, w2p, b_out, x_out, skip, dil, first,
                  dbg_clock=None):
    _f(x_in), _f(x_out), _f(skip)
    B, Cc, T = x_in.shape
    assert Cc == 256
    a = SetDiffnetLayerArgs()
    a.x_in, a.condproj, a.dstep = x_in.data_ptr(), condproj, dstep
    a.w1p, a.b_dil, a.w2p, a.b_out = w1p.data_ptr(), b_dil.data_ptr(), w2p.data_ptr(), b_out.data_ptr()
    a.x_out, a.skip = x_out.data_ptr(), skip.data_ptr()
    a.cp_bs, a.d_bs, a.d_cs = int(cp_bs), int(d_bs), int(d_cs)
    a.B, a.T, a.dil, a.first = B, T, int(dil), int(bool(first))
    a.dbg_clock = dbg_clock.data_ptr() if dbg_clock is not None else None
    check(_lib.lib().set_diffnet_layer(C.byref(a), _stream()), "set_diffnet_layer")


def posterior_step(x0, x_t, coef4, eps=None, out=None, seed=0, offset=0):
    _f(x0), _f(x_t), _f(coef4), _f(eps)
    B = x0.shape[0]
    per_batch = x0.numel() // B
    out = x_t if out is None else out
    assert coef4.shape[0] in (1, B) and coef4.shape[-1] == 4
    coef_bs = 0 if coef4.shape[0] == 1 else 4
    check(_lib.lib().set_posterior_step(_p(x0), _p(x_t), _p(eps), _p(coef4), coef_bs, _p(out), B, per_batch, int(seed),
                                        int(offset), _stream()), "set_posterior_step")
    return out


def q_sample(x_start, eps, ab2, nonpad=None):
    _f(x_start), _f(eps), _f(ab2), _f(nonpad)
    B, M, T = x_start.shape[0], x_start.shape[-2], x_start.shape[-1]
    out = torch.empty_like(x_start)
    check(_lib.lib().set_q_sample(_p(x_start), _p(eps), _p(ab2), _p(nonpad), _p(out), B, M, T, _stream()),
          "set_q_sample")
    return out


def randn(shape, device, seed=0, offset=0):
    out = torch.empty(shape, dtype=torch.float32, device=device)
    check(_lib.lib().set_randn(_p(out), out.numel(), int(seed), int(offset), _stream()), "set_randn")
    return out


def fanout(x, n):
    return (x,) * n


def grad_scale(x, s):
    return x


def dropout(x, p, seed, offset=0):
    return x


def res_skip_fn(x, o, skip_in):
    first = skip_in is None
    skip = torch.empty_like(x) if first else skip_in
    return res_skip(x, o, skip, first), skip


def selftest_mfma():
    err = C.c_float(-1.0)
    check(_lib.lib().set_selftest_mfma(C.byref(err), _stream()), "set_selftest_mfma")
    return float(err.value)


def diffusion_loop(*, x, noise, seed, condproj, dstep, coef4, w_in, b_in, packs, w_skip, b_skip,
                   w_outp, b_outp, L, steps, dilation_cycle_length, want_layer_spans=False, n_groups=None,
                   persistent=None, bf16=None):
    _f(x), _f(noise), _f(condproj), _f(dstep), _f(coef4)
    B, M, T = x.shape
    dev = x.device
    ws = [torch.empty(B, 256, T, dtype=torch.float32, device=dev) for _ in range(4)]
    ws_x0pred = torch.empty(B, M, T, dtype=torch.float32, device=dev)
    a = SetDiffLoopArgs()
    a.B, a.T, a.M, a.L, a.steps, a.dilation_cycle_length = B, T, M, L, steps, dilation_cycle_length
    a.x = x.data_ptr()
    a.noise = noise.data_ptr() if noise is not None else None
    a.seed = int(seed)
    a.condproj = condproj.data_ptr() if condproj is not None else None
    a.dstep, a.coef4 = dstep.data_ptr(), coef4.data_ptr()
    if bf16 is not None:
        a.cond, a.img16_all, a.b_cond_all = _f(bf16["cond"]).data_ptr(), bf16["imgs"].data_ptr(), _f(bf16["b_cond"]).data_ptr()
        n_ws = max(_lib.lib().set_diffnet_layers_bf16_scratch_floats(B, T, 0, n, dilation_cycle_length) for n in range(2, 17)) \
            if dilation_cycle_length <= 2 else 0
        if n_ws > 0:
            bf16_ws = torch.empty(n_ws, dtype=torch.float32, device=dev)
            a.bf16_ws, a.bf16_ws_floats = bf16_ws.data_ptr(), n_ws
    a.w_in_p, a.b_in = w_in.packed().data_ptr(), b_in.data_ptr()
    z_ws = _set_images(a, packs, B, T, dilation_cycle_length, dev)
    a.persistent = int(default_persistent() if persistent is None else bool(persistent))
    sync_ws = torch.empty(sync_ws_size(B, T), dtype=torch.int32, device=dev)
    a.sync_ws = sync_ws.data_ptr()
    err = torch.zeros(1, dtype=torch.int32, device=dev)
    a.err_flag = err.data_ptr()
    bf16_bx2 = bf16 is not None and split_operand_mode() == 2
    use_bx2 = ((a.wx3_all and a.x3_mode == 2) or bf16_bx2) and M <= 96 and os.environ.get("SET_AMD_BOUNDARY_X2", "1") != "0"
    if use_bx2:
        a.w_skip_x2, a.w_outp_x2, a.w_in_x2 = (w.packed_x2().data_ptr() for w in (w_skip, w_outp, w_in))
    a.w_skip_p, a.b_skip = w_skip.packed().data_ptr(), b_skip.data_ptr()
    a.w_outp_p, a.b_outp = w_outp.packed().data_ptr(), b_outp.data_ptr()
    a.ws_x0, a.ws_x1, a.ws_skip, a.ws_h = (w.data_ptr() for w in ws)
    a.ws_x0pred = ws_x0pred.data_ptr()
    a.n_groups = default_groups(B, T) if n_groups is None else int(n_groups)
    spans, loop_ms = None, None
    if want_layer_spans:
        spans = (C.c_float * steps)()
        a.layer_span_ms = C.cast(spans, C.POINTER(C.c_float))
        loop_ms = C.c_float(0.0)
        a.loop_ms = C.pointer(loop_ms)
    check(_lib.lib().set_diffusion_loop(C.byref(a), _stream()), "set_diffusion_loop")
    if a.persistent or use_bx2:
        code = int(err.item())
        if code == 2:
            raise SplitRangeError("set_diffusion_loop: an activation of magnitude >= 32768 is outside the range of the fp16 "
                                  "operand splitting; set SET_AMD_SPLIT_OPERAND=bf16x3 (fp32 range) or SET_AMD_X3=0")
        if code != 0:
            raise _lib.SetAmdError("set_diffusion_loop: a tile dependency wait of the persistent layer-stack kernel timed out")
    if spans is None:
        return None
    return {"layer_span_ms": list(spans), "loop_ms": float(loop_ms.value), "n_groups": int(a.n_groups),
            "persistent": int(a.persistent)}


def default_persistent():
    return os.environ.get("SET_AMD_PERSISTENT", "1") != "0"


def default_groups(B, T):
    return 1


class MatView:

    def __init__(self, tensor, n_outer, n_inner, rows, cols, bo_s, bi_s, rs, cs, offset=0):
        self.tensor = _f(tensor)
        self.n_outer, self.n_inner, self.rows, self.cols = int(n_outer), int(n_inner), int(rows), int(cols)
        self.bo_s, self.bi_s, self.rs, self.cs, self.offset = int(bo_s), int(bi_s), int(rs), int(cs), int(offset)

    @property
    def t(self):
        return MatView(self.tensor, self.n_outer, self.n_inner, self.cols, self.rows, self.bo_s, self.bi_s, self.cs,
                       self.rs, self.offset)

    @staticmethod
    def heads(x, heads, chan0=0, width=None):
        B, Ctot, T = x.shape
        H = Ctot - chan0 if width is None else width
        d = H // heads
# ... 167 lines not shown
```

Before: 175,100.

## Skip dead last-layer residual output and fold sync reset into boundary kernel

Result: no change. 176,200 (median of 6 runs) (+0.6%).

```diff
diff --git a/include/set_amd.h b/include/set_amd.h
--- a/include/set_amd.h
+++ b/include/set_amd.h
@@ -172,6 +172,7 @@
     float *z_ws;
     const void *wx3_all;
     int32_t x3_mode;
+    int32_t last_x_dead;
 } SetDiffnetStackArgs;
 int set_diffnet_stack(const SetDiffnetStackArgs *args, void *stream);
 int64_t set_sizeof_diffnet_stack_args(void);
diff --git a/speech-editing-toolkit_amd/_lib.py b/speech-editing-toolkit_amd/_lib.py
--- a/speech-editing-toolkit_amd/_lib.py
+++ b/speech-editing-toolkit_amd/_lib.py
@@ -86,7 +86,7 @@
         ("x_all", C.c_void_p), ("save_y", C.c_void_p), ("save_z", C.c_void_p),
         ("err_flag", C.c_void_p),
         ("w1s_all", C.c_void_p), ("w2s_all", C.c_void_p), ("z_ws", C.c_void_p), ("wx3_all", C.c_void_p),
-        ("x3_mode", C.c_int32),
+        ("x3_mode", C.c_int32), ("last_x_dead", C.c_int32),
     ]
 
 
diff --git a/speech-editing-toolkit_amd/csrc/diffnet.hip b/speech-editing-toolkit_amd/csrc/diffnet.hip
--- a/speech-editing-toolkit_amd/csrc/diffnet.hip
+++ b/speech-editing-toolkit_amd/csrc/diffnet.hip
@@ -988,7 +988,7 @@
     return stack_variant(B, T, dilation_cycle_length, (images & 1) != 0, (images & 2) != 0, x3_mode_of_images(images), n_cu);
 }
 
-int set_launch_diffnet_stack_x3(const SetDiffnetStackArgs &a, int n_cu, int fault_tile, hipStream_t s);
+int set_launch_diffnet_stack_x3(const SetDiffnetStackArgs &a, int n_cu, int fault_tile, bool sync_clean, hipStream_t s);
 int set_x3_winograd_selected(int x3_mode, int B, int T, int dilation_cycle_length, int n_cu);
 extern "C" int set_diffnet_stack_x3_winograd(int B, int T, int dilation_cycle_length, int images) {
     int n_cu = 256;
@@ -997,17 +997,16 @@
     if (stack_variant(B, T, dilation_cycle_length, (images & 1) != 0, (images & 2) != 0, x3_mode, n_cu) != 5) return 0;
     return set_x3_winograd_selected(x3_mode, B, T, dilation_cycle_length, n_cu);
 }
-int set_launch_diffnet_stack_split_x2(const SetDiffnetStackArgs &a, int fault_tile, hipStream_t s);
-
-extern "C" int set_diffnet_stack(const SetDiffnetStackArgs *args, void *stream) {
-    SET_REQUIRE(args != nullptr, "set_diffnet_stack");
-    const SetDiffnetStackArgs &a = *args;
+int set_launch_diffnet_stack_split_x2(const SetDiffnetStackArgs &a, int fault_tile, bool sync_clean, hipStream_t s);
+
+static inline int sync_ws_words(int B, int T) { return 16 + 2 * B * ((T + 31) / 32); }
+
+static int diffnet_stack_launch(const SetDiffnetStackArgs &a, bool sync_clean, hipStream_t s) {
     SET_REQUIRE(a.xa && a.xb && a.skip && a.condproj && a.dstep && a.w1p_all && a.w2p_all && a.b_dil_all &&
                     a.b_out_all && a.sync_ws,
                 "set_diffnet_stack");
     SET_REQUIRE(a.B > 0 && a.T > 0 && a.L > 0 && a.dilation_cycle_length >= 1 && a.dilation_cycle_length <= 4,
                 "set_diffnet_stack");
-    hipStream_t s = (hipStream_t)stream;
     static SetDeviceOnce lds_once;
     if (int rc = set_lds_optin(lds_once, 150 * 1024, "set_diffnet_stack(attr)", diffnet_stack_kernel<1, 8, 2>, diffnet_stack_kernel<2, 4, 2>,
                                diffnet_stack_wino_kernel<true>, diffnet_stack_wino_kernel<false>, diffnet_stack_split_kernel))
@@ -1019,12 +1018,12 @@
                                       a.w1s_all && a.w2s_all && a.z_ws && plain, (a.wx3_all && plain) ? a.x3_mode : 0, n_cu);
     int fault_tile = -1;
     if (const char *e = getenv("SET_AMD_FAULT_TILE")) fault_tile = atoi(e);
-    if (variant >= 4) return set_launch_diffnet_stack_x3(a, n_cu, fault_tile, s);
+    if (variant >= 4) return set_launch_diffnet_stack_x3(a, n_cu, fault_tile, sync_clean, s);
     if (variant == 3 && a.wx3_all && a.x3_mode == 2 && !split_f32_pinned())
-        return set_launch_diffnet_stack_split_x2(a, fault_tile, s);
+        return set_launch_diffnet_stack_split_x2(a, fault_tile, sync_clean, s);
     if (variant == 3) {
         const int tiles = (a.T + 31) / 32, nt = a.B * tiles;
-        SET_HIP(set_zero_async(a.sync_ws, (size_t)(4 + 2 * nt) * sizeof(int32_t), s), "set_diffnet_stack(memset)");
+        if (!sync_clean) SET_HIP(set_zero_async(a.sync_ws, (size_t)(4 + 2 * nt) * sizeof(int32_t), s), "set_diffnet_stack(memset)");
         hipLaunchKernelGGL(diffnet_stack_split_kernel, dim3(4 * nt), dim3(256), (size_t)SP_LDS_FLOATS * sizeof(float), s, a,
                            tiles, nt, fault_tile);
         return set_check_launch("set_diffnet_stack");
@@ -1045,8 +1044,8 @@
     const int max_dil = 1 << (a.dilation_cycle_length - 1);
     const int task_slot = DC * (ntt + 2 * max_dil);
     const size_t lds = (size_t)(task_slot + 4) * sizeof(float);
-    SET_HIP(set_zero_async(a.sync_ws, (size_t)(4 + ntiles + (wino ? 12 : 0)) * sizeof(int32_t), s),
-            "set_diffnet_stack(memset)");
+    if (!sync_clean)
+        SET_HIP(set_zero_async(a.sync_ws, (size_t)(4 + ntiles + (wino ? 12 : 0)) * sizeof(int32_t), s), "set_diffnet_stack(memset)");
     const int wps = wino ? 1 : 2;
     int grid = wps * n_cu;
     if (grid > ntiles * 4 / 5) grid = ntiles * 4 / 5;
@@ -1072,6 +1071,11 @@
     return set_check_launch("set_diffnet_stack");
 }
 
+extern "C" int set_diffnet_stack(const SetDiffnetStackArgs *args, void *stream) {
+    SET_REQUIRE(args != nullptr, "set_diffnet_stack");
+    return diffnet_stack_launch(*args, false, (hipStream_t)stream);
+}
+
 namespace {
 __global__ void __launch_bounds__(256) gate_kernel(const float *y, float *z, int B, int C, int T) {
     const int64_t i = (int64_t)blockIdx.x * 256 + threadIdx.x;
@@ -1243,7 +1247,13 @@
     float div;
     uint64_t seed, quad_offset;
     int T, M, MP;
+    int32_t *zero_ws;
+    int32_t zero_words;
 };
+__device__ __forceinline__ void boundary_zero_ws(const BoundaryArgs &a) {
+    if (blockIdx.x == 0 && blockIdx.y == 0)
+        for (int i = threadIdx.x; i < a.zero_words; i += 256) a.zero_ws[i] = 0;
+}
 constexpr int BD_LD = 64;
 
 __global__ void __launch_bounds__(256, 2) diffnet_boundary_kernel(BoundaryArgs a) {
@@ -1252,6 +1262,7 @@
     const int w = __builtin_amdgcn_readfirstlane(tid >> 6);
     const int half = lane >> 5, l31 = lane & 31;
     const int b = blockIdx.y, t0 = blockIdx.x * 64, T = a.T, M = a.M;
+    boundary_zero_ws(a);
     {
         const rsrc_t rs = make_rsrc(a.skip + (int64_t)b * DC * T);
         const unsigned vo = 4u * (unsigned)min(t0 + lane, T - 1);
@@ -1391,6 +1402,7 @@
     const unsigned lane16 = 16u * (unsigned)lane;
     const unsigned T4 = 4u * (unsigned)T;
     float amax = 0.0f;
+    boundary_zero_ws(a);
     {
         const int f = lane, cg = w;
         const rsrc_t rs = make_rsrc(a.skip + (int64_t)b * DC * T);
@@ -1575,7 +1587,7 @@
 }
 
 static int launch_boundary(const SetDiffLoopArgs &a, int Bg, const float *skip, float *x, const float *eps, int sid,
-                           uint64_t quad_offset, float *xin_next, bool x2, hipStream_t s) {
+                           uint64_t quad_offset, float *xin_next, bool x2, int32_t *zero_ws, int zero_words, hipStream_t s) {
     static SetDeviceOnce lds_once;
     if (int rc = set_lds_optin(lds_once, 80 * 1024, "boundary(attr)", diffnet_boundary_kernel, diffnet_boundary_x2_kernel)) return rc;
     BoundaryArgs g = {};
@@ -1584,6 +1596,7 @@
     g.w_in_p = a.w_in_p; g.b_in = a.b_in; g.xin_next = xin_next;
     g.div = sqrtf((float)a.L); g.seed = a.seed; g.quad_offset = quad_offset;
     g.T = a.T; g.M = a.M; g.MP = (a.M + 15) / 16 * 16;
+    g.zero_ws = zero_ws; g.zero_words = zero_ws ? zero_words : 0;
     if (x2) {
         BoundaryX2Args gx = {};
         gx.g = g;
@@ -1642,6 +1655,10 @@
     }
     if (bf16_loop && fused_boundary && a.w_skip_x2 && a.w_outp_x2 && a.w_in_x2 && a.M <= 96) boundary_x2 = true;
     if (const char *e = getenv("SET_AMD_BOUNDARY_X2")) boundary_x2 = boundary_x2 && atoi(e) != 0;
+    bool lean = true;
+    if (const char *e = getenv("SET_AMD_LOOP_LEAN")) lean = atoi(e) != 0;
+    const bool fold_reset = lean && a.persistent && !bf16_loop && fused_boundary && g == 0 && Bg == a.B && a.err_flag != nullptr;
+    bool sync_clean = false;
     for (int k = 0; k < a.steps && rc == SET_OK; ++k) {
         const int sid = a.steps - 1 - k;
         if (!fused_boundary || k == 0) {
@@ -1664,7 +1681,9 @@
             sa.err_flag = a.err_flag;
             sa.sync_ws = sync_ws;
             sa.B = Bg; sa.T = T; sa.L = L; sa.dilation_cycle_length = a.dilation_cycle_length;
-            rc = set_diffnet_stack(&sa, s);
+            sa.last_x_dead = lean ? 1 : 0;
+            rc = diffnet_stack_launch(sa, sync_clean, s);
+            sync_clean = false;
         }
         int fuse = 1;
         if (bf16_loop && a.bf16_ws && a.dilation_cycle_length <= 2) {
@@ -1716,8 +1735,10 @@
         if (rc != SET_OK) break;
         const float *eps = a.noise ? a.noise + (int64_t)k * a.B * per_batch + (int64_t)b0 * per_batch : nullptr;
         if (fused_boundary) {
+            const bool fold = fold_reset && k + 1 < a.steps;
             rc = launch_boundary(a, Bg, ws_skip, x, eps, sid, (uint64_t)(k + 1) * quads_total + quads_before,
-                                 k + 1 < a.steps ? ws_x0 : nullptr, boundary_x2, s);
+                                 k + 1 < a.steps ? ws_x0 : nullptr, boundary_x2, fold ? sync_ws : nullptr, sync_ws_words(Bg, T), s);
+            sync_clean = fold && rc == SET_OK;
             continue;
         }
         SetConv1dArgs cs = conv1x1_args(ws_skip, a.w_skip_p, a.b_skip, ws_h, Bg, DC, DC, T);
diff --git a/speech-editing-toolkit_amd/csrc/diffnet_x3.hip b/speech-editing-toolkit_amd/csrc/diffnet_x3.hip
--- a/speech-editing-toolkit_amd/csrc/diffnet_x3.hip
+++ b/speech-editing-toolkit_amd/csrc/diffnet_x3.hip
@@ -119,18 +119,19 @@
     for (int q = 0; q < S::NP; ++q) base[q * 512] = p[q];
 }
 
-template <typename S, int NKS, int NU, int NCB, int PF, typename BF>
+template <typename S, int NKS, int NU, int NCB, int PF, int NRB = 2, int RB0 = 0, typename BF>
 __device__ __forceinline__ void gemm_x3(f32x16 (&acc)[NU][2][NCB], rsrc_t img, unsigned lane16, unsigned abase, unsigned ustride,
                                         const unsigned char *lds, unsigned piece_bytes, BF bfrag) {
     constexpr int NP = S::NP;
     static_assert(NKS % PF == 0, "k-steps must be a multiple of the prefetch distance");
+    static_assert(RB0 >= 0 && NRB >= 1 && RB0 + NRB <= 2, "row blocks of the image");
     u32x4_t A[PF][NU][2][NP];
 #pragma unroll
     for (int p = 0; p < PF; ++p)
 #pragma unroll
         for (int u = 0; u < NU; ++u)
 #pragma unroll
-            for (int rb = 0; rb < 2; ++rb)
+            for (int rb = RB0; rb < RB0 + NRB; ++rb)
 #pragma unroll
                 for (int q = 0; q < NP; ++q)
                     A[p][u][rb][q] = buf_load_u4(img, lane16, abase + (unsigned)u * ustride + (unsigned)(((p * 2 + rb) * NP + q) * 1024));
@@ -152,7 +153,7 @@
 #pragma unroll
                 for (int u = 0; u < NU; ++u)
 #pragma unroll
-                    for (int rb = 0; rb < 2; ++rb)
+                    for (int rb = RB0; rb < RB0 + NRB; ++rb)
 #pragma unroll
                         for (int cb = 0; cb < NCB; ++cb)
                             acc[u][rb][cb] = S::mma(A[p][u][rb][S::qa(t)], Bv[cb][S::qb(t)], acc[u][rb][cb]);
@@ -161,7 +162,7 @@
 #pragma unroll
             for (int u = 0; u < NU; ++u)
 #pragma unroll
-                for (int rb = 0; rb < 2; ++rb)
+                for (int rb = RB0; rb < RB0 + NRB; ++rb)
 #pragma unroll
                     for (int q = 0; q < NP; ++q)
                         A[p][u][rb][q] = buf_load_u4(img, lane16, abase + (unsigned)u * ustride + (unsigned)(((kn * 2 + rb) * NP + q) * 1024));
@@ -185,6 +186,7 @@
     const float *b_dil, *b_out;
     int32_t *err_flag;
     int T, dil, first;
+    int dead;
     int q0, nbu, Q;
 };
 
@@ -476,6 +478,7 @@
         lt.b_out = a.b_out_all + (int64_t)l * 512;
         lt.err_flag = a.err_flag;
         lt.T = a.T; lt.dil = 1 << (l % a.dilation_cycle_length); lt.first = (l == 0);
+        lt.dead = 0;
         lt.nbu = (a.T + 31) / 32; lt.Q = a.B * lt.nbu; lt.q0 = i * NCB;
         f32x16 acc[NU][2][NCB];
         if constexpr (NU == 1) x3_init<NU, NCB>(lt, acc);
@@ -538,7 +541,7 @@
 }
 
 template <typename S, int NU, int NCB>
-int launch_x3(const SetDiffnetStackArgs &a, int n_cu, int fault_tile, hipStream_t s) {
+int launch_x3(const SetDiffnetStackArgs &a, int n_cu, int fault_tile, bool sync_clean, hipStream_t s) {
     static SetDeviceOnce lds_once;
     if (int rc = set_lds_optin(lds_once, 160 * 1024, "set_diffnet_stack(x3 attr)", diffnet_stack_x3_kernel<S, NU, NCB>)) return rc;
     const int Q = a.B * ((a.T + 31) / 32);
@@ -549,7 +552,7 @@
     const int max_dil = 1 << (a.dilation_cycle_length - 1);
     const unsigned piece_bytes = (unsigned)(NCB * (32 + 2 * max_dil) * XR);
     const size_t ldsz = x3_lds_bytes<S, NCB>(max_dil);
-    SET_HIP(set_zero_async(a.sync_ws, (size_t)(4 + ntiles) * sizeof(int32_t), s), "set_diffnet_stack(memset)");
+    if (!sync_clean) SET_HIP(set_zero_async(a.sync_ws, (size_t)(4 + ntiles) * sizeof(int32_t), s), "set_diffnet_stack(memset)");
     int grid = NU * n_cu;
     if (grid > ntiles * 4 / 5) grid = ntiles * 4 / 5;
     if (const char *e = getenv("SET_AMD_STACK_GRID")) grid = atoi(e) > 0 ? atoi(e) : grid;
@@ -831,12 +834,15 @@
         vo4[cb] = 4u * (unsigned)(4 * half * T + min(t, T - 1));
         ub[cb] = (int64_t)c.b * XC * T;
     }
+    const bool dead = a.dead != 0;
     float xres[NB][16];
-#pragma unroll
-    for (int cb = 0; cb < NB; ++cb) {
-        const rsrc_t rx = make_rsrc(a.xin + ub[cb]);
-#pragma unroll
-        for (int r = 0; r < 16; ++r) xres[cb][r] = buf_load(rx, vo4[cb], (unsigned)(32 * w + urow(r)) * T4);
+    if (!dead) {
+#pragma unroll
+        for (int cb = 0; cb < NB; ++cb) {
+            const rsrc_t rx = make_rsrc(a.xin + ub[cb]);
+#pragma unroll
+            for (int r = 0; r < 16; ++r) xres[cb][r] = buf_load(rx, vo4[cb], (unsigned)(32 * w + urow(r)) * T4);
+        }
     }
     __syncthreads();
     X3V_TS(15)
@@ -872,6 +878,7 @@
     f32x16 acc[1][2][NB];
 #pragma unroll
     for (int rb = 0; rb < 2; ++rb) {
+        if (rb == 0 && dead) continue;
         const float *bo = a.b_out + (rb ? XC : 0) + 32 * w;
 #pragma unroll
         for (int r = 0; r < 16; ++r) {
@@ -884,8 +891,12 @@
     X3V_TS(16)
     __syncthreads();
     X3V_PHASE(8)
-    gemm_x3<S, X_KS2, 1, NB, XV_PF2>(acc, rw, lane16, (unsigned)(x_n1<S>() * 2 + w * X_KS2 * 2 * 2 * 1024), (unsigned)(X_KS2 * 2 * 2 * 1024), lds,
-                                     xv_zpiece<NB>(), [&](int ks, int cb) { return (unsigned)((cb * 32 + l31) * XR + (ks * 16 + half * 8) * 2); });
+    const unsigned a2base = (unsigned)(x_n1<S>() * 2 + w * X_KS2 * 2 * 2 * 1024);
+    auto zfrag = [&](int ks, int cb) { return (unsigned)((cb * 32 + l31) * XR + (ks * 16 + half * 8) * 2); };
+    if (dead)
+        gemm_x3<S, X_KS2, 1, NB, XV_PF2, 1, 1>(acc, rw, lane16, a2base, (unsigned)(X_KS2 * 2 * 2 * 1024), lds, xv_zpiece<NB>(), zfrag);
+    else
+        gemm_x3<S, X_KS2, 1, NB, XV_PF2>(acc, rw, lane16, a2base, (unsigned)(X_KS2 * 2 * 2 * 1024), lds, xv_zpiece<NB>(), zfrag);
     X3V_PHASE(9)
     const bool first = a.first != 0;
     float sk[NB][16];
@@ -899,7 +910,7 @@
     }
 #pragma unroll
     for (int cb = 0; cb < NB; ++cb) {
-        if (tv[cb]) {
+        if (tv[cb] && !dead) {
             const rsrc_t rxo = make_rsrc(a.xout + ub[cb]);
 #pragma unroll
             for (int r = 0; r < 16; ++r) buf_store_agent((acc[0][0][cb][r] * is2) * RSQRT2, rxo, vo4[cb], (unsigned)(32 * w + urow(r)) * T4);
@@ -962,6 +973,7 @@
         lt.b_out = a.b_out_all + (int64_t)l * 512;
         lt.err_flag = a.err_flag;
         lt.T = a.T; lt.dil = 1; lt.first = (l == 0);
+        lt.dead = (a.last_x_dead != 0 && l == a.L - 1);
         lt.nbu = (a.T + 31) / 32; lt.Q = a.B * lt.nbu; lt.q0 = i * NB;
         f32x4 PQ[2][4][NB];
         X3V_KTS(0)
@@ -1055,7 +1067,7 @@
 }
 
 template <int NB>
-int launch_x3v(const SetDiffnetStackArgs &a, int n_cu, int fault_tile, hipStream_t s) {
+int launch_x3v(const SetDiffnetStackArgs &a, int n_cu, int fault_tile, bool sync_clean, hipStream_t s) {
     static SetDeviceOnce lds_once;
     if (int rc = set_lds_optin(lds_once, 160 * 1024, "set_diffnet_stack(x3v attr)", diffnet_stack_x3v_kernel<NB>)) return rc;
     const int Q = a.B * ((a.T + 31) / 32);
@@ -1065,7 +1077,7 @@
     SET_REQUIRE((int64_t)2 * XC * a.T * 4 < ((int64_t)1 << 31), "set_diffnet_stack(split-operand kernel: T too large)");
     SET_REQUIRE(a.dilation_cycle_length == 1 && a.T % 2 == 0, "set_diffnet_stack(x3v: dilation 1 and even T only)");
     const size_t ldsz = (size_t)xv_tile<NB>() + NB * XC * sizeof(float) + 16;
-    SET_HIP(set_zero_async(a.sync_ws, (size_t)(4 + ntiles) * sizeof(int32_t), s), "set_diffnet_stack(memset)");
+    if (!sync_clean) SET_HIP(set_zero_async(a.sync_ws, (size_t)(4 + ntiles) * sizeof(int32_t), s), "set_diffnet_stack(memset)");
     int grid = n_cu;
     if (NB == 2 && grid > ntiles * 4 / 5) grid = ntiles * 4 / 5;
     if (const char *e = getenv("SET_AMD_STACK_GRID")) grid = atoi(e) > 0 ? atoi(e) : grid;
@@ -1359,14 +1371,14 @@
 
 }
 
-int set_launch_diffnet_stack_split_x2(const SetDiffnetStackArgs &a, int fault_tile, hipStream_t s) {
+int set_launch_diffnet_stack_split_x2(const SetDiffnetStackArgs &a, int fault_tile, bool sync_clean, hipStream_t s) {
     static SetDeviceOnce lds_once;
     if (int rc = set_lds_optin(lds_once, 80 * 1024, "set_diffnet_stack(split x2 attr)", diffnet_stack_split_x2_kernel)) return rc;
     const int tiles = (a.T + 31) / 32, nt = a.B * tiles;
     const int max_dil = 1 << (a.dilation_cycle_length - 1);
     const unsigned piece_bytes = (unsigned)((32 + 2 * max_dil) * XR);
     const size_t ldsz = (size_t)2 * piece_bytes + (64 * 32 + XC) * sizeof(float) + 16;
-    SET_HIP(set_zero_async(a.sync_ws, (size_t)(4 + 2 * nt) * sizeof(int32_t), s), "set_diffnet_stack(memset)");
+    if (!sync_clean) SET_HIP(set_zero_async(a.sync_ws, (size_t)(4 + 2 * nt) * sizeof(int32_t), s), "set_diffnet_stack(memset)");
     int n_cu = 0;
     (void)set_cu_count(&n_cu);
     const int extra = (4 * nt + 8 <= n_cu && a.L > 1) ? 8 : 0;
@@ -1414,7 +1426,7 @@
     return tiles96 >= (int64_t)n_cu ? 3 : 2;
 }
 
-int set_launch_diffnet_stack_x3(const SetDiffnetStackArgs &a, int n_cu, int fault_tile, hipStream_t s) {
+int set_launch_diffnet_stack_x3(const SetDiffnetStackArgs &a, int n_cu, int fault_tile, bool sync_clean, hipStream_t s) {
     SET_REQUIRE(a.x3_mode == 2 || a.x3_mode == 3, "set_diffnet_stack(x3_mode must be 2 = f16x2 or 3 = bf16x3)");
     const int64_t tiles64 = (int64_t)a.B * ((a.T + 63) / 64);
     bool narrow = 5 * tiles64 < 3 * (int64_t)n_cu;
@@ -1422,9 +1434,9 @@
     const bool al8 = ((reinterpret_cast<uintptr_t>(a.condproj) | reinterpret_cast<uintptr_t>(a.xa) | reinterpret_cast<uintptr_t>(a.xb)) & 7) == 0 &&
                      ((a.cp_bs | a.cp_ls) & 1) == 0;
     const int wino = al8 ? set_x3_winograd_selected(a.x3_mode, a.B, a.T, a.dilation_cycle_length, n_cu) : 0;
-    if (wino == 3) return launch_x3v<3>(a, n_cu, fault_tile, s);
-    if (wino == 2) return launch_x3v<2>(a, n_cu, fault_tile, s);
+    if (wino == 3) return launch_x3v<3>(a, n_cu, fault_tile, sync_clean, s);
+    if (wino == 2) return launch_x3v<2>(a, n_cu, fault_tile, sync_clean, s);
     if (a.x3_mode == 2)
-        return narrow ? launch_x3<SplitF16x2, 1, 1>(a, n_cu, fault_tile, s) : launch_x3<SplitF16x2, 1, 2>(a, n_cu, fault_tile, s);
-    return narrow ? launch_x3<SplitBf16x3, 1, 1>(a, n_cu, fault_tile, s) : launch_x3<SplitBf16x3, 1, 2>(a, n_cu, fault_tile, s);
-}
+        return narrow ? launch_x3<SplitF16x2, 1, 1>(a, n_cu, fault_tile, sync_clean, s) : launch_x3<SplitF16x2, 1, 2>(a, n_cu, fault_tile, sync_clean, s);
+    return narrow ? launch_x3<SplitBf16x3, 1, 1>(a, n_cu, fault_tile, sync_clean, s) : launch_x3<SplitBf16x3, 1, 2>(a, n_cu, fault_tile, sync_clean, s);
+}
diff --git a/speech-editing-toolkit_amd/ops.py b/speech-editing-toolkit_amd/ops.py
--- a/speech-editing-toolkit_amd/ops.py
+++ b/speech-editing-toolkit_amd/ops.py
@@ -805,6 +805,7 @@
     a.cp_bs, a.cp_ls = condproj.stride(0), 512 * T
     a.d_bs, a.d_cs, a.d_ls = int(d_bs), int(d_cs), int(d_ls)
     a.B, a.T, a.L, a.dilation_cycle_length = B, T, L, int(dilation_cycle_length)
+    a.last_x_dead = 0
     check(_lib.lib().set_diffnet_stack(C.byref(a), _stream()), "set_diffnet_stack")
     return sync_ws
 
```
